# AIRI-Institute/nablaDFT

Hardware: AMD Instinct MI355X
Metric: conformer-steps/sec (fwd+bwd) + MAE(E,F) vs CPU reference (higher is better)
Workload: dtype f32 (dense products >= 192 tiles: f32 values split exactly into 3 bf16 pieces, 6 MFMA piece products, f32 accumulate; non-finite operands give NaN where plain f32 gives inf); 1 GPU; PaiNN-OC (nablaDFT/painn_pyg, config/model/painn-oc.yaml: F=128 L=6 R=100 rc=5A K=100) energy+forces train step incl. neighbour list, L1+L2 loss, grad all-reduce, clip 5.0, AdamW lr 5e-4; synthetic ~42-atom drug-like conformers, 2048 conformers/GPU/step; conformers_per_gpu=2048, edges_last_step=1669592, parallelism=dp1

## Files before the change

### nabladft_amd/csrc/common.h

```cpp
#pragma once
#include <hip/hip_runtime.h>
#include <stdint.h>
#include <stdio.h>

#define NQ_WAVE 64

#define NQ_OK 0
#define NQ_ERR_HIP 1
#define NQ_ERR_ARG 2
#define NQ_ERR_MOL_TOO_LARGE 3
#define NQ_ERR_WORKSPACE 4
#define NQ_ERR_NO_EDGES 5

extern thread_local char nq_err_buf[512];
int nq_fail(int code, const char* fmt, ...);

#define NQ_HIP(call)                                                                            \
  do {                                                                                          \
    hipError_t e__ = (call);                                                                    \
    if (e__ != hipSuccess)                                                                      \
      return nq_fail(NQ_ERR_HIP, "%s:%d %s -> %s", __FILE__, __LINE__, #call, hipGetErrorString(e__)); \
  } while (0)

#define NQ_LAUNCH_CHECK() NQ_HIP(hipGetLastError())
// ... 91 lines not shown
#define NQ_ROWCTR_INTS (8 * 4 * 8 * NQ_ROWCTR_PAD)

struct MsgRevArgs {
  NqGraphView g; int F;
  const float* V; const float* XH; const float* PHI; const float* PSI;
  const float* TV; const float* TXH; const float* TD; const float* TR;
  const float* GX; const float* GV;
  const float* GTX; const float* GTV;
  float* GXH; float* GTXH;
  float* GV_out; float* GTV_out;
  float* GPHI; float* GPSI;
  float4* GEDGE;
  float* GBR;
  int row_filter, mol_cap;
  int lite;
};

struct UpdArgs {
  int N, F;
  const float* XM; const float* VM; const float* U; const float* Y;
  float* S; float* CAT; float* X1; float* V1;
  const float* TXM; const float* TVM; const float* TU; const float* TY;
  float* TS; float* TCAT; float* TX1; float* TV1;
};

struct UpdRevArgs {
  int N, F;
  const float* U; const float* Y; const float* S; const float* CAT;
  const float* TU; const float* TY; const float* TS; const float* TCAT;
  float* GX; float* GV; float* GTX; float* GTV;
  float* GY; float* GTY;
  const float* GCAT; const float* GTCAT;
  float* GU; float* GTU;
  int lite; float* GX_out;
};

struct ReadoutArgs {
  int N, H;
  const float* ZO; const float* TZO; const float* w2; float o2_dummy; const float* o2;
  float* e_atom; float* te_atom;
  const float* ge; const float* gte;
  float* GZO; float* GTZO;
  float* TMPW;
};

int nq_graph_count_impl(const float* pos, const int* mol_ptr, int N, int B, int max_mol_atoms, float cutoff2, int K, int* deg, int* lowdeg,
                        int* row_ptr, int* lowptr, int* E_host, hipStream_t st);
int nq_graph_fill_impl(GraphFillArgs args, int B, int max_mol_atoms, hipStream_t st);

int nq_gemm_nn_epi(hipStream_t st, const float* G, const float* W, float* C, int M, int Nout, int Kin, const float* aux, float ea, float eb, int mode,
                   const char* tag = nullptr);
int nq_gemm_nn_dsilu2(hipStream_t st, const float* G, const float* W, float* C, float* C2, const float* aux, int M, int Nout, int Kin, const char* tag);
int nq_gemm_nt_dsilu(hipStream_t st, const float* A, const float* W, float* C, float* C2, const float* aux, int M, int N, int K, const char* tag = nullptr);
int nq_gemm_nt_act(hipStream_t, const float* A, const float* W, float* C, float* C2, const float* resid, float ea, float eb, int M, int N, int K,
                   const char* tag = nullptr);
int nq_gemm_nt(hipStream_t, const float* A, const float* W, float* C, const float* bias, float* C2_silu, int M, int N, int K, int lda,
               int ldw, int ldc, const char* tag = nullptr);
int nq_gemm_nn(hipStream_t, const float* G, const float* W, float* C, int M, int Nout, int Kin, int ldg, int ldw, int ldc, int accumulate,
               const char* tag = nullptr);
int nq_gemm_nt_res(hipStream_t st, const float* A, const float* W, float* C, const float* aux, float ea, int M, int N, int K);
size_t nq_gemm_tn_scratch_floats(long rows, int Mo, int No);
int nq_gemm_tn(hipStream_t, const float* GY, const float* X, float* out, long rows, int Mo, int No, int ldg, int ldx, float* scratch,
               const char* tag = nullptr, float* bias_out = nullptr, long bias_rows = 0);
size_t nq_colsum_scratch_floats(long rows, int cols);
int nq_colsum(hipStream_t, const float* A, long rows, int cols, int lda, float* out, float* scratch);
int nq_reduce_partials(hipStream_t, const float* part, int nsplit, long stride, long count, float* out);

int nq_rbf(hipStream_t, const float4* geom, int E, int R, double cutoff, int env_p, float coeff, const float* offsets, float* rho,
           float* drho, int type = 0, const float* theta = nullptr);
int nq_rbf_param_grad(hipStream_t, const float4* geom, int E, int R, double cutoff, int env_p, const float* offsets, int type, const float* theta,
                      const float* grho, float* contrib);
int nq_msg_fwd(hipStream_t, const MsgArgs&, bool tangent);
bool nq_filter_fits_lds(int F, int R);
void nq_make_filter_args(FilterArgs* fa, const float* WRT, const float* br, const float* mu, const float* RW, int R, double cutoff, int env_p,
                         float coeff, int mode = 0);
int nq_rbf_window(hipStream_t, const float4* geom, int E, const FilterArgs& fa, float* RW);
int nq_transpose(hipStream_t, const float* in, int rows, int cols, float* out);
size_t nq_k0_sort_scratch_ints(int E, int R);
int nq_k0_sort(hipStream_t, const float* RW, int E, int R, int* order, int* scratch, const int* row_of = nullptr, const int* col = nullptr,
               const int* mol_ptr = nullptr, const int* atom_mol = nullptr, int cap = 0, int* count_out = nullptr);
size_t nq_gwr_scratch_floats(int E, int F, int R, int parts = 3);
int nq_gwr_sorted(hipStream_t, const float* GPHI, const float* GPSI, const float* RW, const int* order, int E, int F, int R, float* gWr,
                  float* scratch, int parts = 3, const int* count_dev = nullptr);
int nq_msgf_fwd(hipStream_t, const MsgArgs&, const FilterArgs&, bool tangent);
int nq_msgf_rev(hipStream_t, const MsgRevArgs&, const FilterArgs&, bool dual, bool pair_rows = true);
int nq_molgw_max_atoms(void);
bool nq_molgw_config_ok(int F, int R);
bool nq_molgw_supported(int F, int R, int max_mol_atoms);
size_t nq_molgw_sched_ints(int E, int B);
size_t nq_molgw_sched_slots(int E, int B);
size_t nq_molgw_rec_floats(int E, int B);
size_t nq_molgw_part_floats(int F, int B);
int nq_molgw_schedule(hipStream_t, const NqGraphView&, const int* dst, const float* RW, int R, int cap, int* sched_ints, float* recs);
int nq_molgw_geometry(hipStream_t, const NqGraphView&, const float* RW, const float* TD, const float* TR, const int* sched_ints, float* recs);
int nq_gwr_mol(hipStream_t, const NqGraphView&, int F, int R, int max_mol_atoms, const float* XH, const float* V, const float* TXH, const float* TV,
               const float* GX, const float* GV, const float* GTX, const float* GTV, const int* sched_ints, const float* recs, float* part, float* gWr,
               float* gbr, bool accumulate = false);
int nq_msg_rev(hipStream_t, const MsgRevArgs&, bool dual);
int nq_geom_tan(hipStream_t, const NqGraphView&, const int* dst, const float* pos_dot, float* TD, float* TR);
int nq_geom_rev(hipStream_t, const NqGraphView&, const float4* GEDGE, int nwaves, float* forces);

bool nq_gemm_exact_f32_requested();
size_t nq_updfuse_frag_floats(int F);
int nq_updfuse_presplit(hipStream_t, const float* U, const float* V1, const float* V2, int F, float* frag);
int nq_upd_fused(hipStream_t, const UpdArgs&, const float* frag, const float* c1, const float* c2, float* ZQ, float* Q);
int nq_upd_a(hipStream_t, const UpdArgs&, bool tan);
int nq_upd_b(hipStream_t, const UpdArgs&, bool tan);
int nq_silu_tan(hipStream_t, const float* Z, const float* TZ, float* TH, long count);
int nq_silu_rev(hipStream_t, const float* Z, const float* TZ, float* G, float* GT, long count, bool dual, bool lite = false);
int nq_upd_rev(hipStream_t, const UpdRevArgs&, int stage, bool dual);
int nq_embed(hipStream_t, const int* z, const float* emb, int N, int F, float* X0);
size_t nq_embed_grad_scratch_floats(int N, int F, int T);
int nq_embed_grad(hipStream_t, const int* z, const float* GX, int N, int F, int T, float* out, float* scratch);
int nq_readout(hipStream_t, const ReadoutArgs&, int mode);
int nq_readout_rev(hipStream_t, const ReadoutArgs&, bool dual);
int nq_mol_sum(hipStream_t, const float* e_atom, const int* mol_ptr, int B, float* out);
int nq_atom_seeds(hipStream_t, const float* gE, const int* atom_mol, int N, float* ge, float* gte);
int nq_negate(hipStream_t, const float* in, float* out, long count);
int nq_axpy(hipStream_t, const float* x, float* y, long count);
int nq_loss_impl(hipStream_t, const float* E, const float* y, int B, const float* Fc, const float* Ft, int N, float ce, float cf, float* loss,
                 float* gE, float* gF, bool mse);
int nq_adamw_impl(hipStream_t, float* p, const float* g, float* m, float* v, long count, float max_norm, float lr, float beta1, float beta2,
                  float eps, float wd, int step, float* scratch);
```

### nabladft_amd/csrc/edge.hip

```cpp
#include "common.h"
#include <type_traits>
#include "lanes.h"

struct RbfArgs {
  const float4* geom; int E; int R; float inv_cutoff; float p, a, b, c; float coeff; const float* mu;
  float* rho; float* drho;
  int type;
  const float* theta;
  float norm_const;
  const float* grho;
  float* contrib;
};

__device__ __forceinline__ void rbf_envelope(const RbfArgs& q, float ds, float& env, float& denv) {
  env = 0.f; denv = 0.f;
  if (ds < 1.0f) {
    if (q.p > 0.f) {
      const float pm1 = powf(ds, q.p - 1.0f);
      const float p0 = pm1 * ds, p1 = p0 * ds, p2 = p1 * ds;
      env = 1.0f + q.a * p0 + q.b * p1 + q.c * p2;
      denv = q.a * q.p * pm1 + q.b * (q.p + 1.0f) * p0 + q.c * (q.p + 2.0f) * p1;
    } else {
      const float om = (1.0f - ds) * (1.0f + ds);
      env = expf(-(ds * ds) / om);
// ... 122 lines not shown
  const float v0 = q.V[o3 + f], v1 = q.V[o3 + F + f], v2 = q.V[o3 + 2 * F + f];
  float txa = 0.f, txb = 0.f, txc = 0.f, tv0 = 0.f, tv1 = 0.f, tv2 = 0.f;
  if (DUAL) {
    txa = q.TXH[o3 + f]; txb = q.TXH[o3 + F + f]; txc = q.TXH[o3 + 2 * F + f];
    tv0 = q.TV[o3 + f]; tv1 = q.TV[o3 + F + f]; tv2 = q.TV[o3 + 2 * F + f];
  }
  float gxa = 0.f, gxb = 0.f, gxc = 0.f, gv0 = 0.f, gv1 = 0.f, gv2 = 0.f;
  float gtxa = 0.f, gtxb = 0.f, gtxc = 0.f, gtv0 = 0.f, gtv1 = 0.f, gtv2 = 0.f;
  float sba = 0.f, sbb = 0.f, sbc = 0.f;
  for (int sp = beg; sp < end; ++sp) {
    const int k = q.g.col[sp];
    const float4 gm = q.g.geom[sp];
    const float r0 = -gm.x, r1 = -gm.y, r2 = -gm.z;
    const float* ph = q.PHI + (long)sp * F3;
    const float pa = ph[f], pb = ph[F + f], pc = ph[2 * F + f];
    const float* A = q.GV + (long)k * F3;
    const float A0 = A[f], A1 = A[F + f], A2 = A[2 * F + f];
    const float gma = q.GX[(long)k * F + f];
    const float mb = xb * pb, mc = xc * pc;
    float gmb = A0 * v0 + A1 * v1 + A2 * v2;
    float gmc = A0 * r0 + A1 * r1 + A2 * r2;
    gv0 += A0 * mb; gv1 += A1 * mb; gv2 += A2 * mb;
    if (DUAL) {
      const float td = q.TD[sp];
      const float tr0 = -q.TR[3 * (long)sp], tr1 = -q.TR[3 * (long)sp + 1], tr2 = -q.TR[3 * (long)sp + 2];
      const float* ps = q.PSI + (long)sp * F3;
      const float tpa = ps[f] * td, tpb = ps[F + f] * td, tpc = ps[2 * F + f] * td;
      const float* T = q.GTV + (long)k * F3;
      const float T0 = T[f], T1 = T[F + f], T2 = T[2 * F + f];
      const float gtma = q.GTX[(long)k * F + f];
      const float tmb = txb * pb + xb * tpb;
      gmb += T0 * tv0 + T1 * tv1 + T2 * tv2;
      const float gtmb = T0 * v0 + T1 * v1 + T2 * v2;
      gmc += T0 * tr0 + T1 * tr1 + T2 * tr2;
      const float gtmc = T0 * r0 + T1 * r1 + T2 * r2;
      gv0 += T0 * tmb; gv1 += T1 * tmb; gv2 += T2 * tmb;
      gtv0 += T0 * mb; gtv1 += T1 * mb; gtv2 += T2 * mb;
      gxa += gma * pa + gtma * tpa; gxb += gmb * pb + gtmb * tpb; gxc += gmc * pc + gtmc * tpc;
      gtxa += gtma * pa; gtxb += gtmb * pb; gtxc += gtmc * pc;
      float* gp = q.GPHI + (long)sp * F3;
      float* gs = q.GPSI + (long)sp * F3;
      const float ga = gma * xa + gtma * txa, gb = gmb * xb + gtmb * txb, gc = gmc * xc + gtmc * txc;
      gp[f] = ga; gp[F + f] = gb; gp[2 * F + f] = gc;
      sba += ga; sbb += gb; sbc += gc;
      gs[f] = gtma * xa * td; gs[F + f] = gtmb * xb * td; gs[2 * F + f] = gtmc * xc * td;
    } else {
      gxa += gma * pa; gxb += gmb * pb; gxc += gmc * pc;
      const float* ps = q.PSI + (long)sp * F3;
      float gd = gma * xa * ps[f] + gmb * xb * ps[F + f] + gmc * xc * ps[2 * F + f];
      float e0 = A0 * mc, e1 = A1 * mc, e2 = A2 * mc;
      gd = nq_wave_sum(gd); e0 = nq_wave_sum(e0); e1 = nq_wave_sum(e1); e2 = nq_wave_sum(e2);
      if (lane == 0) {
        float4* dstp = q.GEDGE + (long)wave * q.g.E + sp;
        float4 acc = *dstp;
        acc.x += gd; acc.y += e0; acc.z += e1; acc.w += e2;
        *dstp = acc;
      }
    }
  }
  q.GXH[o3 + f] = gxa; q.GXH[o3 + F + f] = gxb; q.GXH[o3 + 2 * F + f] = gxc;
  q.GV_out[o3 + f] = q.GV[o3 + f] + gv0;
  q.GV_out[o3 + F + f] = q.GV[o3 + F + f] + gv1;
  q.GV_out[o3 + 2 * F + f] = q.GV[o3 + 2 * F + f] + gv2;
  if (DUAL) {
    q.GTXH[o3 + f] = gtxa; q.GTXH[o3 + F + f] = gtxb; q.GTXH[o3 + 2 * F + f] = gtxc;
    q.GBR[o3 + f] = sba; q.GBR[o3 + F + f] = sbb; q.GBR[o3 + 2 * F + f] = sbc;
    q.GTV_out[o3 + f] = q.GTV[o3 + f] + gtv0;
    q.GTV_out[o3 + F + f] = q.GTV[o3 + F + f] + gtv1;
    q.GTV_out[o3 + 2 * F + f] = q.GTV[o3 + 2 * F + f] + gtv2;
  }
}


#define FUSED_THREADS 1024
#ifndef NQ_DUAL2_THREADS
#define NQ_DUAL2_THREADS 512
#endif
#ifndef NQ_TAN2_THREADS
#define NQ_TAN2_THREADS 768
#endif
#ifndef NQ_DUALNG2_THREADS
#define NQ_DUALNG2_THREADS 768
#endif
__host__ __device__ constexpr int fused_threads(int kind, int ch) {
  return ch >= 4 ? 512
                 : (ch == 2 ? (kind == 3 ? NQ_DUAL2_THREADS : (kind == 4 ? NQ_DUALNG2_THREADS : (kind == 1 ? NQ_TAN2_THREADS : 1024)))
                            : (kind >= 3 ? 768 : 1024));
}
#define FUSED_THREADS_DUAL 1024

__device__ __forceinline__ float bcast_lane(float v, int t) {
  return __int_as_float(__builtin_amdgcn_readlane(__float_as_int(v), t));
}

#define RBFW_THREADS 256
__global__ __launch_bounds__(RBFW_THREADS) void k_rbf_window(const float4* __restrict__ geom, int E, FilterArgs fa, float* __restrict__ RW) {
  __shared__ float tile[RBFW_THREADS][RW_STRIDE + 1];
  const int e0 = blockIdx.x * RBFW_THREADS, e = e0 + threadIdx.x;
  if (e < E) {
    const int R = fa.R;
    const float dist = geom[e].w;
    const float ds = dist * fa.inv_cutoff;
    const int nwin = R < FWIN ? R : FWIN;
    int kc = (int)rintf(ds * (float)(R - 1));
    kc = min(max(kc, 0), R - 1);
    const int k0 = min(max(kc - FWIN / 2, 0), R - nwin);
    float beta = 1.f, dbeta = 0.f, env = 0.f, denv = 0.f;
    if (fa.mode == 0) {
      if (ds < 1.0f) {
        if (fa.p > 0.f) {
          const float pm1 = powf(ds, fa.p - 1.0f);
          const float p0 = pm1 * ds, p1 = p0 * ds, p2 = p1 * ds;
          env = 1.0f + fa.a * p0 + fa.b * p1 + fa.c * p2;
          denv = fa.a * fa.p * pm1 + fa.b * (fa.p + 1.0f) * p0 + fa.c * (fa.p + 2.0f) * p1;
        } else {
          const float om = (1.0f - ds) * (1.0f + ds);
          env = expf(-(ds * ds) / om);
          denv = -env * 2.0f * ds / (om * om);
        }
      }
    } else {
      const float arg = dist * (3.14159265358979323846f / fa.cutoff);
      const bool inside = dist < fa.cutoff;
      beta = inside ? 0.5f * (cosf(arg) + 1.0f) : 0.f;
      dbeta = inside ? -0.5f * (3.14159265358979323846f / fa.cutoff) * sinf(arg) : 0.f;
    }
    float* rw = tile[threadIdx.x];
#pragma unroll
    for (int t = 0; t < 16; ++t) {
      float rl = 0.f, drl = 0.f;
      if (t < nwin) {
        if (fa.mode == 0) {
          const float diff = ds - fa.mu[k0 + t];
          const float g = expf(fa.coeff * (diff * diff));
          rl = env * g;
          drl = fa.inv_cutoff * g * (denv + env * (2.0f * fa.coeff) * diff);
        } else {
          const float diff = dist - fa.mu[k0 + t];
          const float g = expf(fa.coeff * (diff * diff));
          if (fa.mode == 2) {
            rl = g;
            drl = g * (2.0f * fa.coeff) * diff;
          } else {
            rl = beta * g;
            drl = dbeta * g + beta * g * (2.0f * fa.coeff) * diff;
          }
        }
      }
      rw[t] = (t == 13) ? __int_as_float(k0) : (t == 14 ? beta : rl);
      rw[16 + t] = (t == 14) ? dbeta : drl;
    }
  }
  __syncthreads();
  const long base = (long)e0 * RW_STRIDE;
  const long lim = (long)min(RBFW_THREADS, E - e0) * RW_STRIDE;
#pragma unroll 4
  for (int i = threadIdx.x; i < RBFW_THREADS * RW_STRIDE; i += RBFW_THREADS)
    if (i < lim) RW[base + i] = tile[i / RW_STRIDE][i % RW_STRIDE];
}

struct RowRegs { int kk; float gx, gy, gz, td, t0, t1, t2, pf; };
#ifndef NQ_RW_TOUCH
#define NQ_RW_TOUCH 1
#endif
__device__ __forceinline__ void row_touch_done(const RowRegs& r) {
#if NQ_RW_TOUCH
  asm volatile("" ::"v"(r.pf));
#endif
}

template <bool NEED_T>
__device__ __forceinline__ void load_row(RowRegs& r, const NqGraphView& g, const float* __restrict__ TD, const float* __restrict__ TR,
                                         const float* __restrict__ RW, int sp0, int cnt, int lane) {
  r.kk = 0; r.gx = r.gy = r.gz = 0.f; r.td = r.t0 = r.t1 = r.t2 = 0.f; r.pf = 0.f;
  if (lane < cnt) {
    const int sp = sp0 + lane;
#if NQ_RW_TOUCH
    r.pf = RW[(long)sp * RW_STRIDE + 15];
#endif
    r.kk = g.col[sp];
    const float4 gm = g.geom[sp];
    r.gx = gm.x; r.gy = gm.y; r.gz = gm.z;
    if (NEED_T) { r.td = TD[sp]; r.t0 = TR[3 * (long)sp]; r.t1 = TR[3 * (long)sp + 1]; r.t2 = TR[3 * (long)sp + 2]; }
  }
}
template <bool PSI, int CH>
__device__ __forceinline__ void filter_eval(const WinRegs<PSI>& w, const float* wrt, int F, int F3, int fb, const float (&bra)[CH],
                                            const float (&brb)[CH], const float (&brc)[CH], float (&pa)[CH], float (&pb)[CH], float (&pc)[CH],
                                            float (&qa)[CH], float (&qb)[CH], float (&qc)[CH]) {
  typedef VOps<CH> O;
  typedef typename O::V V;
  const V ba = O::from(bra), bb = O::from(brb), bc = O::from(brc);
  V va = ba * O::splat(w.rr[14]), vb = bb * O::splat(w.rr[14]), vc = bc * O::splat(w.rr[14]);
  V ua = O::splat(0.f), ub = ua, uc = ua;
  if (PSI) { ua = ba * O::splat(w.dd[14]); ub = bb * O::splat(w.dd[14]); uc = bc * O::splat(w.dd[14]); }
  const int k0 = __builtin_amdgcn_readfirstlane(__float_as_int(w.rr[13]));
  const float* wk = wrt + k0 * F3 + fb;
#pragma unroll
  for (int t = 0; t < FWIN; ++t) {
    const V wa = lds_tap<CH>(wk + t * F3), wb = lds_tap<CH>(wk + t * F3 + F), wc = lds_tap<CH>(wk + t * F3 + 2 * F);
    const V r = O::splat(w.rr[t]);
    va = O::fma(wa, r, va); vb = O::fma(wb, r, vb); vc = O::fma(wc, r, vc);
    if (PSI) {
      const V d = O::splat(w.dd[t]);
      ua = O::fma(wa, d, ua); ub = O::fma(wb, d, ub); uc = O::fma(wc, d, uc);
    }
  }
  O::to(pa, va); O::to(pb, vb); O::to(pc, vc);
  O::to(qa, ua); O::to(qb, ub); O::to(qc, uc);
}

#ifndef NQ_CLAIM_KINDS
#define NQ_CLAIM_KINDS 15
#endif
#ifndef NQ_CLAIM_ROWS
#define NQ_CLAIM_ROWS 1
#endif
#ifndef NQ_CLAIM_GROUPS_DUAL
#define NQ_CLAIM_GROUPS_DUAL 1
#endif
#ifndef NQ_CLAIM_GROUPS
#define NQ_CLAIM_GROUPS 2
#endif
#define FUSED_ROWS(KIND)                                                                        \
  constexpr bool claim__ = ((NQ_CLAIM_KINDS >> (KIND)) & 1) != 0;                               \
  const bool dyn__ = claim__ && fa.row_ctr != nullptr;    \
  constexpr int crows__ = claim__ ? NQ_CLAIM_ROWS : 1;                                          \
  constexpr int cgmax__ = ((KIND) == 3) ? NQ_CLAIM_GROUPS_DUAL : NQ_CLAIM_GROUPS;               \
  const int cgrp__ = max(1, min(cgmax__, (int)(gridDim.x / nxcd / nslices)));    \
  const int grp__ = wg % cgrp__;                                                                \
  const int sub__ = (n_hi - x_lo + cgrp__ - 1) / cgrp__;                                        \
  const int s_lo__ = dyn__ ? x_lo + grp__ * sub__ : x_lo;                                       \
  const int s_hi__ = dyn__ ? min(n_hi, s_lo__ + sub__) : n_hi;                                  \
  int* const ctr__ = dyn__ ? fa.row_ctr + (((int)(blockIdx.x % nxcd) * nslices + slice) * cgmax__ + grp__) * NQ_ROWCTR_PAD : nullptr; \
  int n_static__ = x_lo + wg * nslots + slot;                                                   \
  auto claim_rows = [&]() __attribute__((always_inline)) -> int {                               \
    if (dyn__) {                                                                                \
      int v__ = 0;                                                                              \
      if (lane == 0) v__ = __hip_atomic_fetch_add(ctr__, crows__, __ATOMIC_RELAXED, __HIP_MEMORY_SCOPE_AGENT); \
      return s_lo__ + __builtin_amdgcn_readfirstlane(v__);                                      \
    }                                                                                           \
    const int v__ = n_static__; n_static__ += n_step; return v__;                               \
  };                                                                                            \
  for (int blk__ = claim_rows(), nxt__ = claim_rows(); blk__ < s_hi__; blk__ = nxt__, nxt__ = claim_rows()) \
    for (int n = blk__; n < min(blk__ + (dyn__ ? crows__ : 1), s_hi__); ++n)

#define FUSED_PROLOGUE                                                                          \
  extern __shared__ __attribute__((aligned(16))) float wrt[];                                  \
  const int F = q.F, F3 = 3 * q.F;                                                             \
  constexpr int FL = 64 * CH;                        \
  const int nslices = F / FL;                                                                  \
   \
  const int nxcd = (gridDim.x % (8 * nslices)) == 0 ? 8 : 1;                                   \
  const int bx = (int)(blockIdx.x / nxcd);                                                     \
  const int slice = bx % nslices, wg = bx / nslices;                                           \
  {                                 \
    const int Rp = fa.R < FWIN ? FWIN : fa.R;                                                  \
    const int per_row4 = (3 * FL) >> 2, fl4 = FL >> 2;                                         \
    float4* dst4 = reinterpret_cast<float4*>(wrt);                                             \
    for (int i = threadIdx.x; i < Rp * per_row4; i += blockDim.x) {                            \
      const int r = i / per_row4, c4 = i % per_row4, part = c4 / fl4, cc = c4 % fl4;           \
      dst4[i] = r < fa.R ? reinterpret_cast<const float4*>(fa.WRT + (long)r * F3 + part * F + slice * FL)[cc] : make_float4(0.f, 0.f, 0.f, 0.f); \
    }                                                                                          \
  }                                                                                            \
  __syncthreads();                                                                             \
  const int nslots = blockDim.x >> 6;                                                          \
  const int slot = __builtin_amdgcn_readfirstlane(threadIdx.x >> 6);                           \
  const int lane = threadIdx.x & 63;                                                           \
  const int lfb = lane * CH;                           \
  const int fb = slice * FL + lfb;                        \
  float bra[CH], brb[CH], brc[CH];                                                             \
  ldv<CH>(bra, fa.br + fb); ldv<CH>(brb, fa.br + F + fb); ldv<CH>(brc, fa.br + 2 * F + fb);    \
                                \
  const int per_x = (q.g.N + nxcd - 1) / nxcd;                                                 \
  const int x_lo = (int)(blockIdx.x % nxcd) * per_x, n_hi = min(q.g.N, x_lo + per_x);          \
  const int n_step = (int)(gridDim.x / nxcd / nslices) * nslots;                               \
                                                          \

template <bool TAN, int CH>
struct FwdOps { float xa[CH], xb[CH], xc[CH], va[CH], vb[CH], vc[CH], txa[CH], txb[CH], txc[CH], tva[CH], tvb[CH], tvc[CH]; };

template <bool TAN>
struct FwdSrc {
  __amdgpu_buffer_rsrc_t xh, v, txh, tv;
  __device__ __forceinline__ FwdSrc(const MsgArgs& q) : xh(row_rsrc(q.XH)), v(row_rsrc(q.V)), txh(row_rsrc(TAN ? q.TXH : q.XH)), tv(row_rsrc(TAN ? q.TV : q.V)) {}
};
template <bool TAN, int CH>
__device__ __forceinline__ void load_fwd(FwdOps<TAN, CH>& o, const FwdSrc<TAN>& src, int k, int F, int F3, int fb) {
  const int ob = fb * 4, r0 = k * F3 * 4, r1 = r0 + F * 4, r2 = r1 + F * 4;
  ldv_buf<CH>(o.xa, src.xh, ob, r0); ldv_buf<CH>(o.xb, src.xh, ob, r1); ldv_buf<CH>(o.xc, src.xh, ob, r2);
  ldv_buf<CH>(o.va, src.v, ob, r0); ldv_buf<CH>(o.vb, src.v, ob, r1); ldv_buf<CH>(o.vc, src.v, ob, r2);
  if (TAN) {
    ldv_buf<CH>(o.txa, src.txh, ob, r0); ldv_buf<CH>(o.txb, src.txh, ob, r1); ldv_buf<CH>(o.txc, src.txh, ob, r2);
    ldv_buf<CH>(o.tva, src.tv, ob, r0); ldv_buf<CH>(o.tvb, src.tv, ob, r1); ldv_buf<CH>(o.tvc, src.tv, ob, r2);
  }
}

template <bool TAN, int CH>
__global__ __launch_bounds__(fused_threads(TAN ? 1 : 0, CH)) void k_msgf_fwd(MsgArgs q, FilterArgs fa, const float* __restrict__ RW) {
  FUSED_PROLOGUE
  const FwdSrc<TAN> src(q);
  FUSED_ROWS(TAN ? 1 : 0) {
    const int beg = __builtin_amdgcn_readfirstlane(q.g.row_ptr[n]), end = __builtin_amdgcn_readfirstlane(q.g.row_ptr[n + 1]);
    float dx[CH], d0[CH], d1[CH], d2[CH];
#pragma unroll
    for (int c = 0; c < CH; ++c) dx[c] = d0[c] = d1[c] = d2[c] = 0.f;
    for (int c0 = beg; c0 < end; c0 += 64) {
      const int cnt = min(64, end - c0);
      RowRegs row;
      load_row<TAN>(row, q.g, q.TD, q.TR, RW, c0, cnt, lane);
      FwdOps<TAN, CH> opA, opB;
      load_fwd<TAN, CH>(opA, src, bl_i(row.kk, 0), F, F3, fb);
      WinRegs<TAN> win;
      load_win<TAN>(win, RW, c0);
      auto step = [&](FwdOps<TAN, CH>& cur, FwdOps<TAN, CH>& nxt, int j, auto prefetch) __attribute__((always_inline)) {
        const int jn = min(j + 1, cnt - 1);
        if (decltype(prefetch)::value) load_fwd<TAN, CH>(nxt, src, bl_i(row.kk, jn), F, F3, fb);
        float pa[CH], pb[CH], pc[CH], qa[CH], qb[CH], qc[CH];
        filter_eval<TAN, CH>(win, wrt, FL, 3 * FL, lfb, bra, brb, brc, pa, pb, pc, qa, qb, qc);
        __builtin_amdgcn_sched_barrier(0);
        if (decltype(prefetch)::value) load_win<TAN>(win, RW, c0 + jn);
        const float gx = bl_f(row.gx, j), gy = bl_f(row.gy, j), gz = bl_f(row.gz, j);
        float td = 0.f, tr0 = 0.f, tr1 = 0.f, tr2 = 0.f;
        if (TAN) { td = bl_f(row.td, j); tr0 = bl_f(row.t0, j); tr1 = bl_f(row.t1, j); tr2 = bl_f(row.t2, j); }
#pragma unroll
        for (int c = 0; c < CH; ++c) {
          const float mb = cur.xb[c] * pb[c], mc = cur.xc[c] * pc[c];
          if (!TAN) {
            dx[c] += cur.xa[c] * pa[c];
            d0[c] += cur.va[c] * mb + mc * gx;
            d1[c] += cur.vb[c] * mb + mc * gy;
            d2[c] += cur.vc[c] * mb + mc * gz;
          } else {
            const float tma = cur.txa[c] * pa[c] + cur.xa[c] * (qa[c] * td);
            const float tmb = cur.txb[c] * pb[c] + cur.xb[c] * (qb[c] * td);
            const float tmc = cur.txc[c] * pc[c] + cur.xc[c] * (qc[c] * td);
            dx[c] += tma;
            d0[c] += cur.tva[c] * mb + cur.va[c] * tmb + tmc * gx + mc * tr0;
            d1[c] += cur.tvb[c] * mb + cur.vb[c] * tmb + tmc * gy + mc * tr1;
            d2[c] += cur.tvc[c] * mb + cur.vc[c] * tmb + tmc * gz + mc * tr2;
          }
        }
      };
      const int pairs = cnt & ~1;
#pragma nounroll
      for (int j = 0; j < pairs; j += 2) {
        step(opA, opB, j, std::true_type());
        step(opB, opA, j + 1, std::true_type());
      }
      if (cnt & 1) step(opA, opB, cnt - 1, std::false_type());
      row_touch_done(row);
    }
    const long o = (long)n * F + fb, o3 = (long)n * F3 + fb;
    float x0[CH], w0[CH], w1[CH], w2[CH];
    if (!TAN) {
      ldv<CH>(x0, q.X + o); ldv<CH>(w0, q.V + o3); ldv<CH>(w1, q.V + o3 + F); ldv<CH>(w2, q.V + o3 + 2 * F);
    } else {
      ldv<CH>(x0, q.TX + o); ldv<CH>(w0, q.TV + o3); ldv<CH>(w1, q.TV + o3 + F); ldv<CH>(w2, q.TV + o3 + 2 * F);
    }
#pragma unroll
    for (int c = 0; c < CH; ++c) { x0[c] += dx[c]; w0[c] += d0[c]; w1[c] += d1[c]; w2[c] += d2[c]; }
    if (!TAN) {
      stv<CH>(q.XM + o, x0); stv<CH>(q.VM + o3, w0); stv<CH>(q.VM + o3 + F, w1); stv<CH>(q.VM + o3 + 2 * F, w2);
    } else {
      stv<CH>(q.TXM + o, x0); stv<CH>(q.TVM + o3, w0); stv<CH>(q.TVM + o3 + F, w1); stv<CH>(q.TVM + o3 + 2 * F, w2);
    }
  }
}

#ifndef NQ_ABLATE
#define NQ_ABLATE 0
#endif
#if NQ_ABLATE == 3
#define ABL_K(j) n
#else
#define ABL_K(j) bl_i(row.kk, j)
#endif
#if NQ_ABLATE == 4
#define ABL_SP(x) 0
#else
#define ABL_SP(x) (x)
#endif
template <bool DUAL, int CH>
struct RevOps { float A0[CH], A1[CH], A2[CH], gma[CH], T0[CH], T1[CH], T2[CH], gtma[CH]; };

template <bool DUAL>
struct RevSrc {
  __amdgpu_buffer_rsrc_t gv, gx, gtv, gtx;
  __device__ __forceinline__ RevSrc(const MsgRevArgs& q) : gv(row_rsrc(q.GV)), gx(row_rsrc(q.GX)), gtv(row_rsrc(DUAL ? q.GTV : q.GV)), gtx(row_rsrc(DUAL ? q.GTX : q.GX)) {}
};
template <bool DUAL, int CH>
__device__ __forceinline__ void load_rev(RevOps<DUAL, CH>& o, const RevSrc<DUAL>& src, int k, int F, int F3, int fb) {
  const int ob = fb * 4, r0 = k * F3 * 4, r1 = r0 + F * 4, r2 = r1 + F * 4, rx = k * F * 4;
  ldv_buf<CH>(o.A0, src.gv, ob, r0); ldv_buf<CH>(o.A1, src.gv, ob, r1); ldv_buf<CH>(o.A2, src.gv, ob, r2);
  ldv_buf<CH>(o.gma, src.gx, ob, rx);
  if (DUAL) {
    ldv_buf<CH>(o.T0, src.gtv, ob, r0); ldv_buf<CH>(o.T1, src.gtv, ob, r1); ldv_buf<CH>(o.T2, src.gtv, ob, r2);
    ldv_buf<CH>(o.gtma, src.gtx, ob, rx);
  }
}

#ifndef NQ_DUAL_NA_RESIDENT
#define NQ_DUAL_NA_RESIDENT 1
#endif
#ifndef NQ_DUAL_MIRROR
#define NQ_DUAL_MIRROR 1
#endif
#ifndef NQ_DUAL_KX_EARLY
#define NQ_DUAL_KX_EARLY 1
#endif
template <bool DUAL, int CH, bool GW, bool LITE = false>
__device__ __forceinline__ void msgf_rev_body(const MsgRevArgs& q, const FilterArgs& fa, const float* __restrict__ RW) {
  FUSED_PROLOGUE
  const RevSrc<DUAL> src(q);
  FUSED_ROWS(DUAL ? 3 : 2) {
    if (DUAL && q.row_filter) {
      const int mm = __builtin_amdgcn_readfirstlane(q.g.atom_mol[n]);
      const bool big = __builtin_amdgcn_readfirstlane(q.g.mol_ptr[mm + 1]) - __builtin_amdgcn_readfirstlane(q.g.mol_ptr[mm]) > q.mol_cap;
      if (big != (q.row_filter == 2)) continue;
    }
    const int beg = __builtin_amdgcn_readfirstlane(q.g.row_ptr[n]), end = __builtin_amdgcn_readfirstlane(q.g.row_ptr[n + 1]);
    const int nlow = (DUAL && GW) ? __builtin_amdgcn_readfirstlane(q.g.lowptr[n + 1]) - __builtin_amdgcn_readfirstlane(q.g.lowptr[n]) : 0;
    const long o3 = (long)n * F3 + fb;
    float xa[CH], xb[CH], xc[CH], v0[CH], v1[CH], v2[CH], txa[CH], txb[CH], txc[CH], tv0[CH], tv1[CH], tv2[CH];
    ldv<CH>(xa, q.XH + o3); ldv<CH>(xb, q.XH + o3 + F); ldv<CH>(xc, q.XH + o3 + 2 * F);
    ldv<CH>(v0, q.V + o3); ldv<CH>(v1, q.V + o3 + F); ldv<CH>(v2, q.V + o3 + 2 * F);
    float nA0[CH], nA1[CH], nA2[CH], ngma[CH], nT0[CH], nT1[CH], nT2[CH], ngtma[CH];
    if (DUAL) {
      ldv<CH>(txa, q.TXH + o3); ldv<CH>(txb, q.TXH + o3 + F); ldv<CH>(txc, q.TXH + o3 + 2 * F);
      ldv<CH>(tv0, q.TV + o3); ldv<CH>(tv1, q.TV + o3 + F); ldv<CH>(tv2, q.TV + o3 + 2 * F);
#if NQ_DUAL_NA_RESIDENT
      if (GW) {
      ldv<CH>(nA0, q.GV + o3); ldv<CH>(nA1, q.GV + o3 + F); ldv<CH>(nA2, q.GV + o3 + 2 * F);
      ldv<CH>(nT0, q.GTV + o3); ldv<CH>(nT1, q.GTV + o3 + F); ldv<CH>(nT2, q.GTV + o3 + 2 * F);
      ldv<CH>(ngma, q.GX + (long)n * F + fb); ldv<CH>(ngtma, q.GTX + (long)n * F + fb);
      }
#endif
    } else {
#pragma unroll
      for (int c = 0; c < CH; ++c) txa[c] = txb[c] = txc[c] = tv0[c] = tv1[c] = tv2[c] = 0.f;
    }
    float gxa[CH], gxb[CH], gxc[CH], gv0[CH], gv1[CH], gv2[CH], gtxa[CH], gtxb[CH], gtxc[CH], gtv0[CH], gtv1[CH], gtv2[CH], sba[CH], sbb[CH], sbc[CH];
#pragma unroll
    for (int c = 0; c < CH; ++c) {
      gxa[c] = gxb[c] = gxc[c] = gv0[c] = gv1[c] = gv2[c] = 0.f;
      gtxa[c] = gtxb[c] = gtxc[c] = gtv0[c] = gtv1[c] = gtv2[c] = 0.f;
      sba[c] = sbb[c] = sbc[c] = 0.f;
    }
    for (int c0 = beg; c0 < end; c0 += 64) {
      const int cnt = min(64, end - c0);
      const int nlo = (DUAL && GW) ? max(0, min(cnt, nlow - (c0 - beg))) : 0;
      RowRegs row;
      load_row<DUAL>(row, q.g, q.TD, q.TR, RW, c0, cnt, lane);
      RevOps<DUAL, CH> opA, opB;
      load_rev<DUAL, CH>(opA, src, ABL_K(0), F, F3, fb);
      WinRegs<true> win;
      load_win<true>(win, RW, ABL_SP(c0));
      float4 eacc = make_float4(0.f, 0.f, 0.f, 0.f);
      auto step = [&](RevOps<DUAL, CH>& cur, RevOps<DUAL, CH>& nxt, int j, auto low_tag) __attribute__((always_inline)) {
        constexpr bool LOW = decltype(low_tag)::value;
        const int sp = c0 + j;
        const int jn = min(j + 1, cnt - 1);
        load_rev<DUAL, CH>(nxt, src, ABL_K(jn), F, F3, fb);
        float kxa[CH], kxb[CH], kxc[CH], kv0[CH], kv1[CH], kv2[CH], ktxa[CH], ktxb[CH], ktxc[CH], ktv0[CH], ktv1[CH], ktv2[CH];
        if (DUAL && GW && LOW && NQ_DUAL_KX_EARLY) {
          const long k3 = (long)ABL_K(j) * F3 + fb;
          ldv<CH>(kxa, q.XH + k3); ldv<CH>(kxb, q.XH + k3 + F); ldv<CH>(kxc, q.XH + k3 + 2 * F);
          ldv<CH>(kv0, q.V + k3); ldv<CH>(kv1, q.V + k3 + F); ldv<CH>(kv2, q.V + k3 + 2 * F);
          ldv<CH>(ktxa, q.TXH + k3); ldv<CH>(ktxb, q.TXH + k3 + F); ldv<CH>(ktxc, q.TXH + k3 + 2 * F);
          ldv<CH>(ktv0, q.TV + k3); ldv<CH>(ktv1, q.TV + k3 + F); ldv<CH>(ktv2, q.TV + k3 + 2 * F);
        }
        float pa[CH], pb[CH], pc[CH], qa[CH], qb[CH], qc[CH];
#if NQ_ABLATE == 2
#pragma unroll
        for (int c = 0; c < CH; ++c) { pa[c] = bra[c] * win.rr[0]; pb[c] = brb[c] * win.rr[1]; pc[c] = brc[c] * win.rr[2]; qa[c] = bra[c] * win.dd[0]; qb[c] = brb[c] * win.dd[1]; qc[c] = brc[c] * win.dd[2]; }
#else
        filter_eval<true, CH>(win, wrt, FL, 3 * FL, lfb, bra, brb, brc, pa, pb, pc, qa, qb, qc);
#endif
        const float beta = win.rr[14], dbeta = win.dd[14];
        __builtin_amdgcn_sched_barrier(0);
        load_win<true>(win, RW, ABL_SP(c0 + jn));
        if (DUAL && GW && LOW && !NQ_DUAL_KX_EARLY) {
          const long k3 = (long)ABL_K(j) * F3 + fb;
          ldv<CH>(kxa, q.XH + k3); ldv<CH>(kxb, q.XH + k3 + F); ldv<CH>(kxc, q.XH + k3 + 2 * F);
          ldv<CH>(kv0, q.V + k3); ldv<CH>(kv1, q.V + k3 + F); ldv<CH>(kv2, q.V + k3 + 2 * F);
          ldv<CH>(ktxa, q.TXH + k3); ldv<CH>(ktxb, q.TXH + k3 + F); ldv<CH>(ktxc, q.TXH + k3 + 2 * F);
          ldv<CH>(ktv0, q.TV + k3); ldv<CH>(ktv1, q.TV + k3 + F); ldv<CH>(ktv2, q.TV + k3 + 2 * F);
        }
        const float r0 = -bl_f(row.gx, j), r1 = -bl_f(row.gy, j), r2 = -bl_f(row.gz, j);
        float td = 0.f, tr0 = 0.f, tr1 = 0.f, tr2 = 0.f;
        if (DUAL) { td = bl_f(row.td, j); tr0 = -bl_f(row.t0, j); tr1 = -bl_f(row.t1, j); tr2 = -bl_f(row.t2, j); }
        float gd = 0.f, e0 = 0.f, e1 = 0.f, e2 = 0.f;
        float ga[CH], gb[CH], gc[CH], ha[CH], hb[CH], hc[CH];
#pragma unroll
        for (int c = 0; c < CH; ++c) {
          const float A0 = cur.A0[c], A1 = cur.A1[c], A2 = cur.A2[c], gma = cur.gma[c];
          const float mb = xb[c] * pb[c], mc = xc[c] * pc[c];
          float gmb = A0 * v0[c] + A1 * v1[c] + A2 * v2[c];
          float gmc = A0 * r0 + A1 * r1 + A2 * r2;
          gv0[c] += A0 * mb; gv1[c] += A1 * mb; gv2[c] += A2 * mb;
          if (DUAL) {
            const float tpa = qa[c] * td, tpb = qb[c] * td, tpc = qc[c] * td;
            const float T0 = cur.T0[c], T1 = cur.T1[c], T2 = cur.T2[c], gtma = cur.gtma[c];
            const float tmb = txb[c] * pb[c] + xb[c] * tpb;
            gmb += T0 * tv0[c] + T1 * tv1[c] + T2 * tv2[c];
            const float gtmb = T0 * v0[c] + T1 * v1[c] + T2 * v2[c];
            gmc += T0 * tr0 + T1 * tr1 + T2 * tr2;
            const float gtmc = T0 * r0 + T1 * r1 + T2 * r2;
            gv0[c] += T0 * tmb; gv1[c] += T1 * tmb; gv2[c] += T2 * tmb;
            if (!LITE) { gtv0[c] += T0 * mb; gtv1[c] += T1 * mb; gtv2[c] += T2 * mb; }
            gxa[c] += gma * pa[c] + gtma * tpa; gxb[c] += gmb * pb[c] + gtmb * tpb; gxc[c] += gmc * pc[c] + gtmc * tpc;
            if (!LITE) { gtxa[c] += gtma * pa[c]; gtxb[c] += gtmb * pb[c]; gtxc[c] += gtmc * pc[c]; }
            if (GW) {
              ga[c] = gma * xa[c] + gtma * txa[c]; gb[c] = gmb * xb[c] + gtmb * txb[c]; gc[c] = gmc * xc[c] + gtmc * txc[c];
              ha[c] = gtma * xa[c] * td; hb[c] = gtmb * xb[c] * td; hc[c] = gtmc * xc[c] * td;
              sba[c] += ga[c] * beta + ha[c] * dbeta;
              sbb[c] += gb[c] * beta + hb[c] * dbeta;
              sbc[c] += gc[c] * beta + hc[c] * dbeta;
            }
          } else {
            gxa[c] += gma * pa[c]; gxb[c] += gmb * pb[c]; gxc[c] += gmc * pc[c];
            gd += gma * xa[c] * qa[c] + gmb * xb[c] * qb[c] + gmc * xc[c] * qc[c];
            e0 += A0 * mc; e1 += A1 * mc; e2 += A2 * mc;
          }
        }
        if (DUAL && GW && LOW && NQ_ABLATE != 1) {
#if !NQ_DUAL_NA_RESIDENT
          __builtin_amdgcn_sched_barrier(0);
          ldv<CH>(nA0, q.GV + o3); ldv<CH>(nA1, q.GV + o3 + F); ldv<CH>(nA2, q.GV + o3 + 2 * F);
          ldv<CH>(nT0, q.GTV + o3); ldv<CH>(nT1, q.GTV + o3 + F); ldv<CH>(nT2, q.GTV + o3 + 2 * F);
          ldv<CH>(ngma, q.GX + (long)n * F + fb); ldv<CH>(ngtma, q.GTX + (long)n * F + fb);
#endif
#pragma unroll
          for (int c = 0; c < CH; ++c) {
            const float rgmb = nA0[c] * kv0[c] + nA1[c] * kv1[c] + nA2[c] * kv2[c] + (nT0[c] * ktv0[c] + nT1[c] * ktv1[c] + nT2[c] * ktv2[c]);
            const float rgtmb = nT0[c] * kv0[c] + nT1[c] * kv1[c] + nT2[c] * kv2[c];
            const float rgmc = -(nA0[c] * r0 + nA1[c] * r1 + nA2[c] * r2) - (nT0[c] * tr0 + nT1[c] * tr1 + nT2[c] * tr2);
            const float rgtmc = -(nT0[c] * r0 + nT1[c] * r1 + nT2[c] * r2);
            ga[c] += ngma[c] * kxa[c] + ngtma[c] * ktxa[c]; gb[c] += rgmb * kxb[c] + rgtmb * ktxb[c]; gc[c] += rgmc * kxc[c] + rgtmc * ktxc[c];
            ha[c] += ngtma[c] * kxa[c] * td; hb[c] += rgtmb * kxb[c] * td; hc[c] += rgtmc * kxc[c] * td;
          }
          float* gp = q.GPHI + (long)sp * F3 + fb;
          float* gs = q.GPSI + (long)sp * F3 + fb;
          stv_stream<CH>(gp, ga); stv_stream<CH>(gp + F, gb); stv_stream<CH>(gp + 2 * F, gc);
          stv_stream<CH>(gs, ha); stv_stream<CH>(gs + F, hb); stv_stream<CH>(gs + 2 * F, hc);
        } else if (!DUAL) {
          gd = nq_wave_sum(gd); e0 = nq_wave_sum(e0); e1 = nq_wave_sum(e1); e2 = nq_wave_sum(e2);
          const bool mine = lane == j;
          eacc.x = mine ? gd : eacc.x; eacc.y = mine ? e0 : eacc.y; eacc.z = mine ? e1 : eacc.z; eacc.w = mine ? e2 : eacc.w;
        }
      };
      int j = 0;
#pragma nounroll
      for (; j + 1 < nlo; j += 2) {
        step(opA, opB, j, std::true_type());
        step(opB, opA, j + 1, std::true_type());
      }
#if NQ_DUAL_MIRROR
      if (j < nlo) {
        step(opA, opB, j, std::true_type());
        ++j;
#pragma nounroll
        for (; j + 1 < cnt; j += 2) {
          step(opB, opA, j, std::false_type());
          step(opA, opB, j + 1, std::false_type());
        }
        if (j < cnt) step(opB, opA, j, std::false_type());
      } else {
#pragma nounroll
        for (; j + 1 < cnt; j += 2) {
          step(opA, opB, j, std::false_type());
          step(opB, opA, j + 1, std::false_type());
        }
        if (j < cnt) step(opA, opB, j, std::false_type());
      }
#else
      if (j < nlo) {
        step(opA, opB, j, std::true_type());
        ++j;
        opA = opB;
      }
#pragma nounroll
      for (; j + 1 < cnt; j += 2) {
        step(opA, opB, j, std::false_type());
        step(opB, opA, j + 1, std::false_type());
      }
      if (j < cnt) step(opA, opB, j, std::false_type());
#endif
      row_touch_done(row);
      if (!DUAL && lane < cnt) {
        float4* dstp = q.GEDGE + (long)slice * q.g.E + c0 + lane;
        float4 acc = *dstp;
        acc.x += eacc.x; acc.y += eacc.y; acc.z += eacc.z; acc.w += eacc.w;
        *dstp = acc;
      }
    }
    float g0[CH], g1[CH], g2[CH];
    stv<CH>(q.GXH + o3, gxa); stv<CH>(q.GXH + o3 + F, gxb); stv<CH>(q.GXH + o3 + 2 * F, gxc);
    ldv<CH>(g0, q.GV + o3); ldv<CH>(g1, q.GV + o3 + F); ldv<CH>(g2, q.GV + o3 + 2 * F);
#pragma unroll
    for (int c = 0; c < CH; ++c) { g0[c] += gv0[c]; g1[c] += gv1[c]; g2[c] += gv2[c]; }
    stv<CH>(q.GV_out + o3, g0); stv<CH>(q.GV_out + o3 + F, g1); stv<CH>(q.GV_out + o3 + 2 * F, g2);
    if (DUAL) {
      if (GW) { stv<CH>(q.GBR + o3, sba); stv<CH>(q.GBR + o3 + F, sbb); stv<CH>(q.GBR + o3 + 2 * F, sbc); }
      if (!LITE && !q.lite) {
        stv<CH>(q.GTXH + o3, gtxa); stv<CH>(q.GTXH + o3 + F, gtxb); stv<CH>(q.GTXH + o3 + 2 * F, gtxc);
        ldv<CH>(g0, q.GTV + o3); ldv<CH>(g1, q.GTV + o3 + F); ldv<CH>(g2, q.GTV + o3 + 2 * F);
#pragma unroll
        for (int c = 0; c < CH; ++c) { g0[c] += gtv0[c]; g1[c] += gtv1[c]; g2[c] += gtv2[c]; }
        stv<CH>(q.GTV_out + o3, g0); stv<CH>(q.GTV_out + o3 + F, g1); stv<CH>(q.GTV_out + o3 + 2 * F, g2);
      }
    }
  }
}


template <bool DUAL, int CH>
__global__ __launch_bounds__(fused_threads(DUAL ? 3 : 2, CH)) void k_msgf_rev(MsgRevArgs q, FilterArgs fa, const float* __restrict__ RW) {
  msgf_rev_body<DUAL, CH, DUAL>(q, fa, RW);
}
template <bool LITE, int CH>
__global__ __launch_bounds__(fused_threads(4, CH)) void k_msgf_rev_nopair(MsgRevArgs q, FilterArgs fa, const float* __restrict__ RW) {
  msgf_rev_body<true, CH, false, LITE>(q, fa, RW);
}

#define SORT_CHUNK 256
struct K0Filter { const int* row_of; const int* col; const int* mol_ptr; const int* atom_mol; int cap; };
__device__ __forceinline__ int k0_key(const float* __restrict__ RW, int e, int E, const K0Filter& f) {
  if (e >= E) return -1;
  if (f.row_of && f.col[e] >= f.row_of[e]) return -1;
  if (f.cap > 0) { const int m = f.atom_mol[f.row_of[e]]; if (f.mol_ptr[m + 1] - f.mol_ptr[m] <= f.cap) return -1; }
  return __float_as_int(RW[(long)e * RW_STRIDE + 13]);
}
__global__ __launch_bounds__(SORT_CHUNK) void k_k0_hist(const float* __restrict__ RW, int E, int nbins, int* __restrict__ chunk_hist,
                                                        int* __restrict__ local_rank, K0Filter flt) {
  __shared__ int keys[SORT_CHUNK];
  __shared__ int hist[256];
  const int e = blockIdx.x * SORT_CHUNK + threadIdx.x;
  const int key = k0_key(RW, e, E, flt);
  keys[threadIdx.x] = key;
  if (threadIdx.x < nbins) hist[threadIdx.x] = 0;
  __syncthreads();
  if (key >= 0) {
    int r = 0;
    for (int i = 0; i < (int)threadIdx.x; ++i) r += (keys[i] == key);
    local_rank[e] = r;
    atomicAdd(&hist[key], 1);
  }
  __syncthreads();
  if (threadIdx.x < nbins) chunk_hist[(long)threadIdx.x * gridDim.x + blockIdx.x] = hist[threadIdx.x];
}
__global__ __launch_bounds__(256) void k_k0_scan(int* __restrict__ hist, int nchunks, int nbins, int* __restrict__ bin_total) {
  const int lane = threadIdx.x & 63;
  const int b = blockIdx.x * 4 + (threadIdx.x >> 6);
  if (b >= nbins) return;
  int* row = hist + (long)b * nchunks;
  int carry = 0;
  for (int c0 = 0; c0 < nchunks; c0 += 64) {
    const int c = c0 + lane;
    const int v = c < nchunks ? row[c] : 0;
    int sc = v;
#pragma unroll
    for (int off = 1; off < 64; off <<= 1) {
      const int t = __shfl_up(sc, off, 64);
      if (lane >= off) sc += t;
    }
    if (c < nchunks) row[c] = carry + sc - v;
    carry += __shfl(sc, 63, 64);
  }
  if (lane == 0) bin_total[b] = carry;
}
__global__ __launch_bounds__(SORT_CHUNK) void k_k0_scatter(const float* __restrict__ RW, int E, int nbins, const int* __restrict__ hist,
                                                           const int* __restrict__ bin_total, const int* __restrict__ local_rank,
                                                           int* __restrict__ order, K0Filter flt, int* __restrict__ count_out) {
  __shared__ int base[256];
  if (threadIdx.x == 0) {
    int run = 0;
    for (int i = 0; i < nbins; ++i) { base[i] = run; run += bin_total[i]; }
    if (count_out && blockIdx.x == 0) *count_out = run;
  }
  __syncthreads();
  const int e = blockIdx.x * SORT_CHUNK + threadIdx.x;
  const int key = k0_key(RW, e, E, flt);
  if (key < 0) return;
  order[base[key] + hist[(long)key * gridDim.x + blockIdx.x] + local_rank[e]] = e;
}

#ifndef GWR_WAVES
#define GWR_WAVES 4
#endif
#ifndef GWR_DEPTH
#define GWR_DEPTH 6
#endif
#ifndef GWR_CHUNKS
#define GWR_CHUNKS 1360
#endif
template <int CH>
__global__ __launch_bounds__(GWR_WAVES * 64) void k_gwr_sorted(const float* __restrict__ GPHI, const float* __restrict__ GPSI, const float* __restrict__ RW,
                                                               const int* __restrict__ order, int E_, int F, int F3, int R, int chunk_len,
                                                               float* __restrict__ part, int* __restrict__ chunk_range, const int* __restrict__ count_dev) {
  const int wave = __builtin_amdgcn_readfirstlane(threadIdx.x >> 6), lane = threadIdx.x & 63;
  const int chunk = blockIdx.x * GWR_WAVES + wave;
// ... 178 lines not shown
  else hipLaunchKernelGGL((k_msg_rev<false>), dim3(q.g.N), dim3(q.F), 0, st, q);
  NQ_LAUNCH_CHECK();
  return NQ_OK;
}

int nq_geom_tan(hipStream_t st, const NqGraphView& g, const int* dst, const float* pos_dot, float* TD, float* TR) {
  NQ_PROF(st, "geom_tan");
  if (g.E <= 0) return NQ_OK;
  hipLaunchKernelGGL(k_geom_tan, dim3(nq_cdiv(g.E, 256)), dim3(256), 0, st, g, dst, pos_dot, TD, TR);
  NQ_LAUNCH_CHECK();
  return NQ_OK;
}

int nq_geom_rev(hipStream_t st, const NqGraphView& g, const float4* GEDGE, int nwaves, float* forces) {
  NQ_PROF(st, "geom_rev");
  hipLaunchKernelGGL(k_geom_rev, dim3(nq_cdiv(g.N, 128)), dim3(128), 0, st, g, GEDGE, nwaves, forces);
  NQ_LAUNCH_CHECK();
  return NQ_OK;
}

bool nq_filter_fits_lds(int F, int R) {
  return (size_t)(R < FWIN ? FWIN : R) * 3 * F * sizeof(float) <= 156 * 1024 && (F == 64 || F == 128 || F == 256);
}

void nq_make_filter_args(FilterArgs* fa, const float* WRT, const float* br, const float* mu, const float* RW, int R, double cutoff, int env_p,
                         float coeff, int mode) {
  const double p = env_p;
  fa->WRT = WRT; fa->br = br; fa->mu = mu; fa->RW = RW; fa->R = R; fa->inv_cutoff = (float)(1.0 / cutoff);
  fa->p = (float)p; fa->a = (float)(-(p + 1) * (p + 2) / 2); fa->b = (float)(p * (p + 2)); fa->c = (float)(-p * (p + 1) / 2);
  fa->coeff = coeff; fa->mode = mode; fa->cutoff = (float)cutoff; fa->row_ctr = nullptr;
}

int nq_rbf_window(hipStream_t st, const float4* geom, int E, const FilterArgs& fa, float* RW) {
  NQ_PROF(st, "rbf_window");
  if (E <= 0) return NQ_OK;
  hipLaunchKernelGGL(k_rbf_window, dim3(nq_cdiv(E, RBFW_THREADS)), dim3(RBFW_THREADS), 0, st, geom, E, fa, RW);
  NQ_LAUNCH_CHECK();
  return NQ_OK;
}

int nq_transpose(hipStream_t st, const float* in, int rows, int cols, float* out) {
  NQ_PROF(st, "transpose");
  hipLaunchKernelGGL(k_transpose, dim3(nq_cdiv(cols, 32), nq_cdiv(rows, 32)), dim3(32, 8), 0, st, in, rows, cols, out);
  NQ_LAUNCH_CHECK();
  return NQ_OK;
}

#ifndef NQ_CH_FWD
#define NQ_CH_FWD 0
#endif
#ifndef NQ_CH_TAN
#define NQ_CH_TAN 0
#endif
#ifndef NQ_CH_FORCE
#define NQ_CH_FORCE 0
#endif
#ifndef NQ_CH_DUAL
#define NQ_CH_DUAL 0
#endif
#ifndef NQ_SMALL_SLICE_ATOMS
#define NQ_SMALL_SLICE_ATOMS 2048
#endif
static int fused_ch(int kind, int F, int N) {
  const int forced = kind == 0 ? NQ_CH_FWD : (kind == 1 ? NQ_CH_TAN : (kind == 2 ? NQ_CH_FORCE : NQ_CH_DUAL));
  const int full = F / 64;
  if (forced > 0 && forced <= full && full % forced == 0) return forced;
  if (N < NQ_SMALL_SLICE_ATOMS && full >= 2) return full / 2;
  return full;
}
static int fused_grid(int N, int F, int ch, int* threads, size_t* lds, int R, int max_threads = FUSED_THREADS) {
  const int nslots = max_threads / 64;
  const int nslices = F / (64 * ch);
  *threads = nslots * 64;
  *lds = (size_t)(R < FWIN ? FWIN : R) * 3 * 64 * ch * sizeof(float);
  int per_cu = (int)((156 * 1024) / *lds);
  per_cu = per_cu < 1 ? 1 : (per_cu > 2 ? 2 : per_cu);
  int groups = 256 * per_cu / nslices;
  groups = groups < 8 ? 8 : (groups / 8) * 8;
  const int need = nq_cdiv(N, nslots);
  if (need < groups) groups = need;
  return groups * nslices;
}

#define FUSED_LAUNCH(KERN, FLAG, CHV, Q)                                                                          \
  do {                                                                                                            \
    NQ_DYN_LDS((KERN<FLAG, CHV>), lds);                                                                           \
    hipLaunchKernelGGL((KERN<FLAG, CHV>), dim3(grid), dim3(threads), lds, st, Q, fa, fa.RW);                      \
  } while (0)
#define FUSED_DISPATCH(KERN, FLAG, Q)                                   \
  do {                                                                  \
    switch (ch) {                                                       \
      case 1: FUSED_LAUNCH(KERN, FLAG, 1, Q); break;                    \
      case 2: FUSED_LAUNCH(KERN, FLAG, 2, Q); break;                    \
      case 4: FUSED_LAUNCH(KERN, FLAG, 4, Q); break;                    \
      default: return nq_fail(NQ_ERR_ARG, "fused message kernels need hidden_channels in {64,128,256}"); \
    }                                                                   \
  } while (0)

int nq_msgf_fwd(hipStream_t st, const MsgArgs& q, const FilterArgs& fa, bool tangent) {
  NQ_PROF(st, tangent ? "msgf_tan" : "msgf_fwd");
  if (q.g.N <= 0) return NQ_OK;
  if ((size_t)q.g.N * 3 * q.F * 4 >= 0xfffff000ull) return nq_fail(NQ_ERR_ARG, "fused message kernels: a node array of %d atoms x %d channels exceeds the 4 GB a buffer descriptor's scalar offset reaches", q.g.N, 3 * q.F);
  int threads; size_t lds;
  const int ch = fused_ch(tangent ? 1 : 0, q.F, q.g.N);
  const int grid = fused_grid(q.g.N, q.F, ch, &threads, &lds, fa.R, fused_threads(tangent ? 1 : 0, ch));
  if (tangent) FUSED_DISPATCH(k_msgf_fwd, true, q);
  else FUSED_DISPATCH(k_msgf_fwd, false, q);
  NQ_LAUNCH_CHECK();
  return NQ_OK;
}

int nq_msgf_rev(hipStream_t st, const MsgRevArgs& q, const FilterArgs& fa, bool dual, bool pair_rows) {
  NQ_PROF(st, dual ? (pair_rows ? "msgf_rev_dual" : "msgf_rev_dual_ng") : "msgf_rev_force");
  if (q.g.N <= 0) return NQ_OK;
  if ((size_t)q.g.N * 3 * q.F * 4 >= 0xfffff000ull) return nq_fail(NQ_ERR_ARG, "fused message kernels: a node array of %d atoms x %d channels exceeds the 4 GB a buffer descriptor's scalar offset reaches", q.g.N, 3 * q.F);
  int threads; size_t lds;
  const int kind = dual ? (pair_rows ? 3 : 4) : 2;
  const int ch = fused_ch(dual ? 3 : 2, q.F, q.g.N);
  const int grid = fused_grid(q.g.N, q.F, ch, &threads, &lds, fa.R, fused_threads(kind, ch));
  if (dual && !pair_rows && q.lite) FUSED_DISPATCH(k_msgf_rev_nopair, true, q);
  else if (dual && !pair_rows) FUSED_DISPATCH(k_msgf_rev_nopair, false, q);
  else if (dual) FUSED_DISPATCH(k_msgf_rev, true, q);
  else FUSED_DISPATCH(k_msgf_rev, false, q);
  NQ_LAUNCH_CHECK();
  return NQ_OK;
}

static int gwr_nbins(int R) { return R - (R < FWIN ? R : FWIN) + 1; }
static int gwr_chunks(int E) {
  int chunk_len = nq_cdiv(E, GWR_CHUNKS);
  if (chunk_len < 64) chunk_len = 64;
  return nq_cdiv(E, chunk_len);
}
size_t nq_k0_sort_scratch_ints(int E, int R) { return (size_t)nq_cdiv(E, SORT_CHUNK) * gwr_nbins(R) + (size_t)E + 256; }
int nq_k0_sort(hipStream_t st, const float* RW, int E, int R, int* order, int* scratch, const int* row_of, const int* col, const int* mol_ptr,
               const int* atom_mol, int cap, int* count_out) {
  NQ_PROF(st, "k0_sort");
  K0Filter flt{row_of, col, mol_ptr, atom_mol, (row_of && mol_ptr && atom_mol) ? cap : 0};
  const int nbins = gwr_nbins(R), nchunks = nq_cdiv(E, SORT_CHUNK);
  if (nbins > 256) return nq_fail(NQ_ERR_ARG, "k0 sort supports at most 256 bins (num_rbf <= 268)");
  int* chunk_hist = scratch; int* local_rank = scratch + (size_t)nchunks * nbins; int* bin_total = local_rank + E;
  hipLaunchKernelGGL(k_k0_hist, dim3(nchunks), dim3(SORT_CHUNK), 0, st, RW, E, nbins, chunk_hist, local_rank, flt);
  NQ_LAUNCH_CHECK();
  hipLaunchKernelGGL(k_k0_scan, dim3(nq_cdiv(nbins, 4)), dim3(256), 0, st, chunk_hist, nchunks, nbins, bin_total);
  NQ_LAUNCH_CHECK();
  hipLaunchKernelGGL(k_k0_scatter, dim3(nchunks), dim3(SORT_CHUNK), 0, st, RW, E, nbins, chunk_hist, bin_total, local_rank, order, flt, count_out);
  NQ_LAUNCH_CHECK();
  return NQ_OK;
}

size_t nq_gwr_scratch_floats(int E, int F, int R, int parts) { const size_t nc = gwr_chunks(E); return nc * R * parts * F + 2 * nc + 16; }

int nq_gwr_sorted(hipStream_t st, const float* GPHI, const float* GPSI, const float* RW, const int* order, int E, int F, int R, float* gWr,
                  float* scratch, int parts, const int* count_dev) {
  NQ_PROF(st, "gwr_sorted");
  const int nchunks = gwr_chunks(E), chunk_len = nq_cdiv(E, nchunks);
  float* part = scratch;
  const int F3 = parts * F;
  int* chunk_range = reinterpret_cast<int*>(scratch + (size_t)nchunks * R * F3);
  dim3 grid(nq_cdiv(nchunks, GWR_WAVES), parts);
  switch (F / 64) {
    case 1: hipLaunchKernelGGL((k_gwr_sorted<1>), grid, dim3(GWR_WAVES * 64), 0, st, GPHI, GPSI, RW, order, E, F, F3, R, chunk_len, part, chunk_range, count_dev); break;
    case 2: hipLaunchKernelGGL((k_gwr_sorted<2>), grid, dim3(GWR_WAVES * 64), 0, st, GPHI, GPSI, RW, order, E, F, F3, R, chunk_len, part, chunk_range, count_dev); break;
    case 4: hipLaunchKernelGGL((k_gwr_sorted<4>), grid, dim3(GWR_WAVES * 64), 0, st, GPHI, GPSI, RW, order, E, F, F3, R, chunk_len, part, chunk_range, count_dev); break;
    default: return nq_fail(NQ_ERR_ARG, "gwr_sorted needs hidden_channels in {64,128,256}");
  }
  NQ_LAUNCH_CHECK();
  hipLaunchKernelGGL(k_gwr_reduce, dim3(nq_cdiv((long)R * F3, 256)), dim3(256), 0, st, part, chunk_range, nq_cdiv(E, chunk_len), R, F3, gWr);
  NQ_LAUNCH_CHECK();
  return NQ_OK;
}
```

### nabladft_amd/csrc/engine.hip

```cpp
#include <stdarg.h>
#include <stdlib.h>
#include <string.h>

#include "../../include/nablaq.h"
#include "common.h"

thread_local char nq_err_buf[512] = "";
int nq_fail(int code, const char* fmt, ...) {
  va_list ap;
  va_start(ap, fmt);
  vsnprintf(nq_err_buf, sizeof(nq_err_buf), fmt, ap);
  va_end(ap);
  return code;
}

#include <map>
#include <mutex>
#include <utility>
static std::mutex g_lds_mu;
static std::map<std::pair<int, const void*>, size_t> g_lds_granted;
int nq_dyn_lds(const void* kernel, size_t bytes) {
  int dev = 0;
  NQ_HIP(hipGetDevice(&dev));
  std::lock_guard<std::mutex> lock(g_lds_mu);
// ... 58 lines not shown
  for (int l = 0; l < c->num_layers; ++l) {
    UpdP& u = P->upd[l];
    u.U = o; o += 2 * F * F; u.V1 = o; o += F * 2 * F; u.c1 = o; o += F; u.V2 = o; o += 3 * F * F; u.c2 = o; o += 3 * F;
  }
  P->O1 = o; o += H * F; P->o1 = o; o += H; P->w2 = o; o += H; P->o2 = o; o += 1;
  P->total = o;
  return NQ_OK;
}

struct WsLayer {
  size_t Z1, Hh, XH, PHI, PSI, XM, VM, UU, S, CAT, ZQ, Q, Y;
  size_t WRT;
  size_t UFRAG;
  size_t LGY, LGCAT, LGU, LGXH, LGXA, LGXB, LGVA, LGVB;
  size_t LGQ, LGH, LGQP, LGHP;
};
struct WsLayout {
  size_t X[65], V[65];
  WsLayer lay[64];
  size_t RHO2, RW, ORDER, ZO, e_atom, te_atom, TD, TR, pos_dot, ge, gte;
  size_t GX, GVa, GVb, GY, GQ, GCAT, GU, GXH, GH, GBR, GPHI2, GEDGE, GZO, TMPW, GRHO, BCON, ROWCTR, SCHED, GWREC, GWPART, scratch;
  size_t scratch_floats, total_floats;
  bool fused;
};
static size_t a4(size_t x) { return (x + 3) & ~(size_t)3; }

static void make_ws_layout(const nq_painn_cfg* c, size_t N, size_t E, size_t B, bool fused, WsLayout* W) {
  const size_t F = c->hidden_channels, R = c->num_rbf, H = F / 2, L = c->num_layers, T = c->num_elements;
  W->fused = fused;
  const size_t EP = W->fused ? 0 : E;
  size_t o = 0;
  auto take = [&](size_t n) { size_t r = o; o += a4(n); return r; };
  for (size_t l = 0; l <= L; ++l) { W->X[l] = take(2 * N * F); W->V[l] = take(2 * N * 3 * F); }
  for (size_t l = 0; l < L; ++l) {
    WsLayer& y = W->lay[l];
    y.Z1 = take(2 * N * F); y.Hh = take(2 * N * F); y.XH = take(2 * N * 3 * F);
    y.PHI = take(EP * 3 * F); y.PSI = take(EP * 3 * F); y.WRT = take(R * 3 * F);
    y.XM = take(2 * N * F); y.VM = take(2 * N * 3 * F); y.UU = take(2 * N * 6 * F);
    y.S = take(2 * N * F); y.CAT = take(2 * N * 2 * F); y.ZQ = take(2 * N * F); y.Q = take(2 * N * F); y.Y = take(2 * N * 3 * F);
    y.UFRAG = take(nq_updfuse_frag_floats((int)F));
    const size_t st_ = W->fused ? 1 : 0;
    y.LGY = take(st_ * 2 * N * 3 * F); y.LGCAT = take(st_ * 2 * N * 2 * F); y.LGU = take(st_ * 2 * N * 6 * F); y.LGXH = take(st_ * 2 * N * 3 * F);
    y.LGXA = take(st_ * N * F); y.LGXB = take(st_ * N * F); y.LGVA = take(st_ * N * 3 * F); y.LGVB = take(st_ * N * 3 * F);
    y.LGQ = take(st_ * 2 * N * F); y.LGH = take(st_ * 2 * N * F); y.LGQP = take(st_ * N * F); y.LGHP = take(st_ * N * F);
  }
  W->RHO2 = take(2 * EP * R);
  W->ORDER = take(W->fused ? E : 0);
  W->RW = take(W->fused ? E * 32 : 0);
  W->ZO = take(2 * N * H); W->e_atom = take(N); W->te_atom = take(N);
  W->TD = take(E); W->TR = take(3 * E); W->pos_dot = take(3 * N); W->ge = take(N); W->gte = take(N);
  W->GX = take(2 * N * F); W->GVa = take(2 * N * 3 * F); W->GVb = take(2 * N * 3 * F);
  W->GY = take(2 * N * 3 * F); W->GQ = take(2 * N * F); W->GCAT = take(2 * N * 2 * F); W->GU = take(2 * N * 6 * F);
  W->GXH = take(2 * N * 3 * F); W->GH = take(2 * N * F);
  W->GBR = take(N * 3 * F);
  W->GPHI2 = take(2 * E * 3 * F);
  W->GEDGE = take((F / 64) * E * 4);
  W->GZO = take(2 * N * H); W->TMPW = take(N * H);
  W->GRHO = take(c->rbf_type ? 2 * E * R : 0); W->BCON = take(c->rbf_type ? E * R : 0);
  W->ROWCTR = take(5 * L * NQ_ROWCTR_INTS);
  W->SCHED = take(W->fused ? nq_molgw_sched_ints((int)E, (int)B) : 0);
  W->GWREC = take(W->fused ? nq_molgw_rec_floats((int)E, (int)B) : 0);
  W->GWPART = take(W->fused ? nq_molgw_part_floats((int)F, (int)B) : 0);
  size_t s = 0;
  auto mx = [&](size_t v) { if (v > s) s = v; };
  mx(nq_gemm_tn_scratch_floats(2 * N, 3 * F, F)); mx(nq_gemm_tn_scratch_floats(2 * N, F, 2 * F)); mx(nq_gemm_tn_scratch_floats(6 * N, 2 * F, F));
  mx(W->fused ? nq_gwr_scratch_floats((int)E, (int)F, (int)R) : nq_gemm_tn_scratch_floats(2 * E, 3 * F, R));
  if (W->fused) mx(nq_k0_sort_scratch_ints((int)E, (int)R));
  mx(nq_gemm_tn_scratch_floats(2 * N, F, F)); mx(nq_gemm_tn_scratch_floats(2 * N, H, F));
  mx(nq_colsum_scratch_floats(N > E ? N : E, 3 * F));
  if (c->rbf_type) { mx(nq_colsum_scratch_floats(E, R)); mx(nq_colsum_scratch_floats(E * R, 1)); }
  mx(nq_embed_grad_scratch_floats((int)N, (int)F, (int)T));
  W->scratch_floats = s;
  W->scratch = take(s);
  W->total_floats = o;
  (void)B;
}

enum { GW_PAIR_ROWS = 0, GW_MOLECULE = 1, GW_MIXED = 2 };
struct StepPlan {
  bool fused;
  int gw_mode, gw_cap;
  bool lite;
  bool fused_update;
};
static StepPlan plan_step(const nq_painn_cfg* c, const nq_graph* g, bool want_forces) {
  auto env_on = [](const char* name) { const char* v = getenv(name); return v && v[0] == '1'; };
  StepPlan p{};
  p.fused = c->rbf_type == 0 && nq_filter_fits_lds(c->hidden_channels, c->num_rbf) && !env_on("NQ_NO_FUSED_FILTER");
  const char* cap = getenv("NQ_MOLGW_CAP");
  const int hw = nq_molgw_max_atoms();
  p.gw_cap = cap && atoi(cap) > 0 && atoi(cap) < hw ? atoi(cap) : hw;
  p.gw_mode = GW_PAIR_ROWS;
  if (p.fused && !env_on("NQ_NO_MOLGW") && nq_molgw_config_ok(c->hidden_channels, c->num_rbf) && g->max_mol_atoms > 0 && (env_on("NQ_MOLGW") || g->N >= 4096))
    p.gw_mode = g->max_mol_atoms <= p.gw_cap ? GW_MOLECULE : GW_MIXED;
  p.lite = p.fused && want_forces && !env_on("NQ_NO_LITE");
  p.fused_update = nq_updfuse_frag_floats(c->hidden_channels) > 0 && !env_on("NQ_NO_FUSED_UPDATE") && !nq_gemm_exact_f32_requested();
  return p;
}
static bool plan_fused(const nq_painn_cfg* c, int32_t N, int32_t E, int32_t B) {
  nq_graph g{};
  g.N = N; g.E = E; g.B = B;
  return plan_step(c, &g, false).fused;
}

struct StepRecord { nq_painn_cfg cfg; int32_t N, E, B, max_mol_atoms; StepPlan plan; };
static std::mutex g_plan_mu;
static std::map<const void*, StepRecord> g_plans;
static void record_plan(const void* ws, const nq_painn_cfg* c, const nq_graph* g, const StepPlan& p) {
  std::lock_guard<std::mutex> lock(g_plan_mu);
  g_plans[ws] = StepRecord{*c, g->N, g->E, g->B, g->max_mol_atoms, p};
}
static int recall_plan(const void* ws, const nq_painn_cfg* c, const nq_graph* g, StepPlan* p) {
  std::lock_guard<std::mutex> lock(g_plan_mu);
  auto it = g_plans.find(ws);
  if (it == g_plans.end()) return nq_fail(NQ_ERR_ARG, "nq_painn_backward: no forward call has prepared this workspace");
  const StepRecord& r = it->second;
  if (memcmp(&r.cfg, c, sizeof(nq_painn_cfg)) != 0 || r.N != g->N || r.E != g->E || r.B != g->B || r.max_mol_atoms != g->max_mol_atoms)
    return nq_fail(NQ_ERR_ARG, "nq_painn_backward: the last forward call on this workspace was made for a different model or batch");
  *p = r.plan;
  return NQ_OK;
}

static NqGraphView view_of(const nq_graph* g) {
  NqGraphView v;
  v.N = g->N; v.B = g->B; v.E = g->E;
  v.mol_ptr = g->mol_ptr; v.row_ptr = g->row_ptr; v.col = g->col; v.rev = g->rev;
  v.geom = reinterpret_cast<const float4*>(g->geom); v.z = g->z; v.atom_mol = g->atom_mol; v.lowptr = g->lowptr;
  return v;
}

static int check_common(const nq_painn_cfg* cfg, const nq_graph* g, const void* ws, size_t ws_bytes, bool fused, WsLayout* W, ParamLayout* P) {
  if (!cfg || !g || !ws) return nq_fail(NQ_ERR_ARG, "null argument");
  NQ_TRY(make_param_layout(cfg, P));
  if (g->N <= 0 || g->B <= 0) return nq_fail(NQ_ERR_ARG, "empty batch");
  if (g->E <= 0) return nq_fail(NQ_ERR_NO_EDGES, "batch has no edges within the cutoff");
  if ((reinterpret_cast<uintptr_t>(ws) & 15) != 0) return nq_fail(NQ_ERR_ARG, "workspace must be 16-byte aligned");
  make_ws_layout(cfg, g->N, g->E, g->B, fused, W);
  if (cfg->filter_mode != 0 && cfg->filter_mode != 1) return nq_fail(NQ_ERR_ARG, "filter_mode must be 0 (painn_pyg) or 1 (schnetpack)");
  if (cfg->filter_mode == 1 && !W->fused)
    return nq_fail(NQ_ERR_ARG, "filter_mode 1 (schnetpack) needs the fused-filter path: hidden_channels in {64,128,256} and WrT fitting the LDS");
  if (ws_bytes < W->total_floats * sizeof(float))
    return nq_fail(NQ_ERR_WORKSPACE, "workspace too small: %zu < %zu bytes", ws_bytes, W->total_floats * sizeof(float));
  return NQ_OK;
}

extern "C" {

int nq_abi_version(void) { return NQ_ABI_VERSION; }
int32_t nq_painn_molecule_lds_atoms(void) { return nq_molgw_max_atoms(); }

void nq_profile_enable(int32_t on) { nq_profile_on = on; }
int nq_profile_read2(char* names, int32_t name_stride, double* total_ms, int64_t* counts, double* flops, int32_t cap) {
  (void)hipDeviceSynchronize();
  std::vector<double> tot(g_prof_names.size(), 0.0), fl(g_prof_names.size(), 0.0);
  std::vector<long long> cnt(g_prof_names.size(), 0);
  for (auto& r : g_prof_recs) {
    float ms = 0.f;
    if (hipEventElapsedTime(&ms, r.a, r.b) == hipSuccess) { tot[r.name_id] += ms; cnt[r.name_id] += 1; fl[r.name_id] += r.flops; }
    (void)hipEventDestroy(r.a); (void)hipEventDestroy(r.b);
  }
  g_prof_recs.clear();
  int n = (int)g_prof_names.size();
  for (int i = 0; i < n && i < cap; ++i) {
    snprintf(names + (size_t)i * name_stride, name_stride, "%s", g_prof_names[i].c_str());
    total_ms[i] = tot[i]; counts[i] = cnt[i];
    if (flops) flops[i] = fl[i];
  }
  return n;
}
int nq_profile_read(char* names, int32_t name_stride, double* total_ms, int64_t* counts, int32_t cap) {
  return nq_profile_read2(names, name_stride, total_ms, counts, nullptr, cap);
}
const char* nq_last_error(void) { return nq_err_buf; }

int nq_graph_count(const float* pos, const int32_t* mol_ptr, int32_t N, int32_t B, int32_t max_mol_atoms, double cutoff,
                   int32_t max_neighbors, int32_t* deg, int32_t* lowdeg, int32_t* row_ptr, int32_t* lowptr, int32_t* E_host, void* stream) {
  if (!pos || !mol_ptr || !deg || !lowdeg || !row_ptr || !lowptr || !E_host) return nq_fail(NQ_ERR_ARG, "null argument");
  if (max_neighbors < 1) return nq_fail(NQ_ERR_ARG, "max_neighbors must be >= 1");
  return nq_graph_count_impl(pos, mol_ptr, N, B, max_mol_atoms, (float)(cutoff * cutoff), max_neighbors, deg, lowdeg, row_ptr, lowptr,
                             E_host, (hipStream_t)stream);
}

int nq_graph_fill(const float* pos, const int32_t* mol_ptr, int32_t N, int32_t B, int32_t E, int32_t max_mol_atoms, double cutoff,
                  int32_t max_neighbors, const int32_t* row_ptr, const int32_t* lowptr, int32_t* col, int32_t* dst, int32_t* rev, float* geom,
                  int32_t* slot2canon, int32_t* atom_mol, int64_t* edge_index, float* edge_dist, float* edge_vector, int64_t* id_swap,
                  int64_t* neighbors, void* stream) {
  if (!pos || !mol_ptr || !row_ptr || !lowptr || !col || !dst || !rev || !geom || !slot2canon || !atom_mol)
    return nq_fail(NQ_ERR_ARG, "null argument");
  if (edge_index && (!edge_dist || !edge_vector || !id_swap)) return nq_fail(NQ_ERR_ARG, "canonical outputs must be all set or all NULL");
  if ((reinterpret_cast<uintptr_t>(geom) & 15) != 0) return nq_fail(NQ_ERR_ARG, "geom must be 16-byte aligned");
  GraphFillArgs a;
  a.pos = pos; a.mol_ptr = mol_ptr; a.row_ptr = row_ptr; a.lowptr = lowptr;
  a.r2 = (float)(cutoff * cutoff); a.K = max_neighbors;
  a.col = col; a.dst = dst; a.rev = rev; a.geom = reinterpret_cast<float4*>(geom); a.slot2canon = slot2canon;
  a.c_src = (long long*)edge_index; a.c_dst = edge_index ? (long long*)edge_index + E : nullptr;
  a.c_dist = edge_dist; a.c_vec = edge_vector; a.id_swap = (long long*)id_swap; a.neighbors = (long long*)neighbors;
  a.atom_mol = atom_mol;
  (void)N;
  return nq_graph_fill_impl(a, B, max_mol_atoms, (hipStream_t)stream);
}

size_t nq_painn_num_params(const nq_painn_cfg* cfg) {
  ParamLayout P;
  if (!cfg || make_param_layout(cfg, &P) != NQ_OK) return 0;
  return P.total;
}

size_t nq_painn_workspace_bytes(const nq_painn_cfg* cfg, int32_t N, int32_t E, int32_t B) {
  ParamLayout P;
  if (!cfg || make_param_layout(cfg, &P) != NQ_OK || N <= 0 || E < 0) return 0;
  WsLayout W;
  make_ws_layout(cfg, N, E, B, plan_fused(cfg, N, E, B), &W);
  return W.total_floats * sizeof(float);
}

int nq_painn_ws_lookup(const nq_painn_cfg* cfg, int32_t N, int32_t E, int32_t B, const char* name, int32_t l, int32_t tangent,
                       size_t* off, size_t* count) {
  ParamLayout P;
  if (!cfg || !name || !off || !count) return nq_fail(NQ_ERR_ARG, "null argument");
  NQ_TRY(make_param_layout(cfg, &P));
  WsLayout W;
  make_ws_layout(cfg, N, E, B, plan_fused(cfg, N, E, B), &W);
  const size_t F = cfg->hidden_channels, R = cfg->num_rbf, H = F / 2, n = N, e = E;
  const int L = cfg->num_layers;
  size_t base = 0, rows = 0, w = 0;
  bool dual = true;
#define LAYER_OK(maxl) if (l < 0 || l > (maxl)) return nq_fail(NQ_ERR_ARG, "layer %d out of range", l)
  if (!strcmp(name, "x_in")) { LAYER_OK(L); base = W.X[l]; rows = n; w = F; }
  else if (!strcmp(name, "vec_in")) { LAYER_OK(L); base = W.V[l]; rows = n; w = 3 * F; }
  else if (!strcmp(name, "z1")) { LAYER_OK(L - 1); base = W.lay[l].Z1; rows = n; w = F; }
  else if (!strcmp(name, "h")) { LAYER_OK(L - 1); base = W.lay[l].Hh; rows = n; w = F; }
  else if (!strcmp(name, "xh")) { LAYER_OK(L - 1); base = W.lay[l].XH; rows = n; w = 3 * F; }
  else if (!strcmp(name, "phi") || !strcmp(name, "psi")) {
    LAYER_OK(L - 1);
    if (W.fused) return nq_fail(NQ_ERR_ARG, "buffer '%s' is not materialised (filter is fused into the message kernels)", name);
    base = name[1] == 'h' ? W.lay[l].PHI : W.lay[l].PSI; rows = e; w = 3 * F; dual = false;
  }
  else if (!strcmp(name, "x_msg")) { LAYER_OK(L - 1); base = W.lay[l].XM; rows = n; w = F; }
  else if (!strcmp(name, "vec_msg")) { LAYER_OK(L - 1); base = W.lay[l].VM; rows = n; w = 3 * F; }
  else if (!strcmp(name, "u")) { LAYER_OK(L - 1); base = W.lay[l].UU; rows = n; w = 6 * F; }
  else if (!strcmp(name, "s")) { LAYER_OK(L - 1); base = W.lay[l].S; rows = n; w = F; }
  else if (!strcmp(name, "cat")) { LAYER_OK(L - 1); base = W.lay[l].CAT; rows = n; w = 2 * F; }
  else if (!strcmp(name, "zq")) { LAYER_OK(L - 1); base = W.lay[l].ZQ; rows = n; w = F; }
  else if (!strcmp(name, "q")) { LAYER_OK(L - 1); base = W.lay[l].Q; rows = n; w = F; }
  else if (!strcmp(name, "y")) { LAYER_OK(L - 1); base = W.lay[l].Y; rows = n; w = 3 * F; }
  else if (!strcmp(name, "rho")) {
    if (W.fused) return nq_fail(NQ_ERR_ARG, "buffer 'rho' is not materialised (filter is fused into the message kernels)");
    base = W.RHO2; rows = e; w = R;
  }
  else if (!strcmp(name, "order")) {
    if (!W.fused) return nq_fail(NQ_ERR_ARG, "buffer 'order' exists only with the fused filter");
    base = W.ORDER; rows = e; w = 1; dual = false;
  }
  else if (!strcmp(name, "pair_sched")) {
    if (!W.fused) return nq_fail(NQ_ERR_ARG, "buffer 'pair_sched' exists only with the fused filter");
    base = W.SCHED; rows = 2 * nq_molgw_sched_slots((int)e, B); w = 1; dual = false;
  }
  else if (!strcmp(name, "pair_sched_meta")) {
    if (!W.fused) return nq_fail(NQ_ERR_ARG, "buffer 'pair_sched_meta' exists only with the fused filter");
    base = W.SCHED + 2 * nq_molgw_sched_slots((int)e, B); rows = nq_molgw_sched_ints((int)e, B) - 2 * nq_molgw_sched_slots((int)e, B); w = 1; dual = false;
  }
  else if (!strcmp(name, "rw")) {
    if (!W.fused) return nq_fail(NQ_ERR_ARG, "buffer 'rw' exists only with the fused filter");
    base = W.RW; rows = e; w = 32; dual = false;
  }
  else if (!strcmp(name, "zo")) { base = W.ZO; rows = n; w = H; }
  else if (!strcmp(name, "e_atom")) { base = tangent ? W.te_atom : W.e_atom; rows = n; w = 1; dual = false; tangent = 0; }
  else if (!strcmp(name, "t_d")) { base = W.TD; rows = e; w = 1; dual = false; }
  else if (!strcmp(name, "t_r")) { base = W.TR; rows = e; w = 3; dual = false; }
  else if (!strcmp(name, "gedge")) { base = W.GEDGE; rows = (F / 64) * e; w = 4; dual = false; }
  else return nq_fail(NQ_ERR_ARG, "unknown workspace buffer '%s'", name);
#undef LAYER_OK
  if (tangent && !dual) return nq_fail(NQ_ERR_ARG, "buffer '%s' has no tangent half", name);
  *off = base + (tangent ? rows * w : 0);
  *count = rows * w;
  return NQ_OK;
}

int nq_painn_forward(const nq_painn_cfg* cfg, const float* params, const float* rbf_offsets, const nq_graph* graph, void* workspace,
                     size_t workspace_bytes, float* energy, float* forces, void* stream) {
  if (!cfg || !graph) return nq_fail(NQ_ERR_ARG, "null argument");
  const StepPlan plan = plan_step(cfg, graph, forces != nullptr);
  WsLayout W; ParamLayout P;
  NQ_TRY(check_common(cfg, graph, workspace, workspace_bytes, plan.fused, &W, &P));
  if (!params || !rbf_offsets || !energy) return nq_fail(NQ_ERR_ARG, "null argument");
  record_plan(workspace, cfg, graph, plan);
  hipStream_t st = (hipStream_t)stream;
  float* ws = (float*)workspace;
  const NqGraphView g = view_of(graph);
  const int N = g.N, E = g.E, F = cfg->hidden_channels, R = cfg->num_rbf, H = F / 2, L = cfg->num_layers;
  const size_t NF = (size_t)N * F;
  int* const rowctr0 = reinterpret_cast<int*>(ws + W.ROWCTR);
  NQ_HIP(hipMemsetAsync(rowctr0, 0, (size_t)2 * L * NQ_ROWCTR_INTS * sizeof(int), st));
  auto row_ctr = [&](int kind, int l) { return N >= 4096 ? rowctr0 + ((size_t)kind * L + l) * NQ_ROWCTR_INTS : (int*)nullptr; };

  NQ_TRY(nq_embed(st, g.z, params + P.emb, N, F, ws + W.X[0]));
  NQ_HIP(hipMemsetAsync(ws + W.X[0] + NF, 0, NF * sizeof(float), st));
  NQ_HIP(hipMemsetAsync(ws + W.V[0], 0, 6 * NF * sizeof(float), st));
  float* rho = ws + W.RHO2; float* drho = rho + (size_t)E * R;
  const bool lite_store = plan.lite;
  if (W.fused) {
    FilterArgs fa0;
    nq_make_filter_args(&fa0, nullptr, nullptr, rbf_offsets, ws + W.RW, R, cfg->cutoff, cfg->envelope_exponent, cfg->rbf_coeff, cfg->filter_mode);
    NQ_TRY(nq_rbf_window(st, g.geom, E, fa0, ws + W.RW));
    int* const sched = reinterpret_cast<int*>(ws + W.SCHED);
    if (plan.gw_mode != GW_PAIR_ROWS) NQ_TRY(nq_molgw_schedule(st, g, graph->dst, ws + W.RW, R, plan.gw_cap, sched, ws + W.GWREC));
    if (plan.gw_mode == GW_PAIR_ROWS) NQ_TRY(nq_k0_sort(st, ws + W.RW, E, R, reinterpret_cast<int*>(ws + W.ORDER), reinterpret_cast<int*>(ws + W.scratch), graph->dst, g.col));
    else if (plan.gw_mode == GW_MIXED)
      NQ_TRY(nq_k0_sort(st, ws + W.RW, E, R, reinterpret_cast<int*>(ws + W.ORDER), reinterpret_cast<int*>(ws + W.scratch), graph->dst, g.col, g.mol_ptr, g.atom_mol,
                        plan.gw_cap, sched + nq_molgw_sched_ints(E, g.B) - 1));
  } else {
    NQ_TRY(nq_rbf(st, g.geom, E, R, cfg->cutoff, cfg->envelope_exponent, cfg->rbf_coeff, rbf_offsets, rho, drho, cfg->rbf_type, params + P.basis));
  }

  for (int l = 0; l < L; ++l) {
    const WsLayer& y = W.lay[l]; const MsgP& mp = P.msg[l]; const UpdP& up = P.upd[l];
    NQ_TRY(nq_gemm_nt(st, ws + W.X[l], params + mp.W1, ws + y.Z1, params + mp.b1, ws + y.Hh, N, F, F, F, F, F, "W1"));
    NQ_TRY(nq_gemm_nt(st, ws + y.Hh, params + mp.W2, ws + y.XH, params + mp.b2, nullptr, N, 3 * F, F, F, F, 3 * F, "W2"));
    MsgArgs m{};
    m.g = g; m.F = F; m.X = ws + W.X[l]; m.V = ws + W.V[l]; m.XH = ws + y.XH; m.PHI = ws + y.PHI; m.PSI = ws + y.PSI;
    m.XM = ws + y.XM; m.VM = ws + y.VM;
    if (W.fused) {
      FilterArgs fa;
      NQ_TRY(nq_transpose(st, params + mp.Wr, 3 * F, R, ws + y.WRT));
      nq_make_filter_args(&fa, ws + y.WRT, params + mp.br, rbf_offsets, ws + W.RW, R, cfg->cutoff, cfg->envelope_exponent, cfg->rbf_coeff, cfg->filter_mode);
      fa.row_ctr = row_ctr(0, l);
      NQ_TRY(nq_msgf_fwd(st, m, fa, false));
    } else {
      NQ_TRY(nq_gemm_nt(st, rho, params + mp.Wr, ws + y.PHI, params + mp.br, nullptr, E, 3 * F, R, R, R, 3 * F, "Wr"));
      NQ_TRY(nq_gemm_nt(st, drho, params + mp.Wr, ws + y.PSI, nullptr, nullptr, E, 3 * F, R, R, R, 3 * F, "Wr"));
      NQ_TRY(nq_msg_fwd(st, m, false));
    }
    UpdArgs u{};
    u.N = N; u.F = F; u.XM = ws + y.XM; u.VM = ws + y.VM; u.U = ws + y.UU; u.Y = ws + y.Y; u.S = ws + y.S; u.CAT = ws + y.CAT;
    u.X1 = ws + W.X[l + 1]; u.V1 = ws + W.V[l + 1];
    if (plan.fused_update) {
      NQ_TRY(nq_updfuse_presplit(st, params + up.U, params + up.V1, params + up.V2, F, ws + y.UFRAG));
      NQ_TRY(nq_upd_fused(st, u, ws + y.UFRAG, params + up.c1, params + up.c2, ws + y.ZQ, ws + y.Q));
      continue;
    }
    NQ_TRY(nq_gemm_nt(st, ws + y.VM, params + up.U, ws + y.UU, nullptr, nullptr, 3 * N, 2 * F, F, F, F, 2 * F, "U"));
    NQ_TRY(nq_upd_a(st, u, false));
    NQ_TRY(nq_gemm_nt(st, ws + y.CAT, params + up.V1, ws + y.ZQ, params + up.c1, ws + y.Q, N, F, 2 * F, 2 * F, 2 * F, F, "V1"));
    NQ_TRY(nq_gemm_nt(st, ws + y.Q, params + up.V2, ws + y.Y, params + up.c2, nullptr, N, 3 * F, F, F, F, 3 * F, "V2"));
    NQ_TRY(nq_upd_b(st, u, false));
  }
  NQ_TRY(nq_gemm_nt(st, ws + W.X[L], params + P.O1, ws + W.ZO, params + P.o1, nullptr, N, H, F, F, F, H, "O1"));
  ReadoutArgs r{};
  r.N = N; r.H = H; r.ZO = ws + W.ZO; r.w2 = params + P.w2; r.o2 = params + P.o2; r.e_atom = ws + W.e_atom;
  NQ_TRY(nq_readout(st, r, 0));
  NQ_TRY(nq_mol_sum(st, ws + W.e_atom, g.mol_ptr, g.B, energy));
  if (!forces) return NQ_OK;

  NQ_TRY(nq_atom_seeds(st, nullptr, g.atom_mol, N, ws + W.ge, nullptr));
  r.ge = ws + W.ge; r.GZO = ws + W.GZO;
  NQ_TRY(nq_readout_rev(st, r, false));
  float* gx_cur = lite_store ? ws + W.lay[L - 1].LGXA : ws + W.GX;
  NQ_TRY(nq_gemm_nn(st, ws + W.GZO, params + P.O1, gx_cur, N, H, F, H, F, F, 0, "O1"));
  float* gv_cur = lite_store ? ws + W.lay[L - 1].LGVA : ws + W.GVa; float* gv_oth = ws + W.GVb;
  NQ_HIP(hipMemsetAsync(gv_cur, 0, 3 * NF * sizeof(float), st));
  const int nwaves = F / 64;
  NQ_HIP(hipMemsetAsync(ws + W.GEDGE, 0, (size_t)nwaves * E * 4 * sizeof(float), st));
  for (int l = L - 1; l >= 0; --l) {
    const WsLayer& y = W.lay[l]; const MsgP& mp = P.msg[l]; const UpdP& up = P.upd[l];
    float* const GY = lite_store ? ws + y.LGY + 3 * NF : ws + W.GY;
    float* const GCAT = lite_store ? ws + y.LGCAT + 2 * NF : ws + W.GCAT;
    float* const GU = lite_store ? ws + y.LGU + 6 * NF : ws + W.GU;
    float* const GXH = lite_store ? ws + y.LGXH + 3 * NF : ws + W.GXH;
    float* const gx_msg = lite_store ? ws + y.LGXB : gx_cur;
    float* const gv_msg = lite_store ? ws + y.LGVB : gv_cur;
    float* const gx_next = lite_store ? (l > 0 ? ws + W.lay[l - 1].LGXA : ws + W.GX) : gx_cur;
    float* const gv_next = lite_store ? (l > 0 ? ws + W.lay[l - 1].LGVA : ws + W.GVb) : gv_oth;
    UpdRevArgs u{};
    u.N = N; u.F = F; u.U = ws + y.UU; u.Y = ws + y.Y; u.S = ws + y.S; u.CAT = ws + y.CAT;
    u.GX = gx_cur; u.GV = gv_cur; u.GY = GY; u.GCAT = GCAT; u.GU = GU;
    u.GX_out = lite_store ? gx_msg : nullptr;
    NQ_TRY(nq_upd_rev(st, u, 1, false));
    float* const GQ = lite_store ? ws + y.LGQ + NF : ws + W.GQ;
    if (lite_store) NQ_TRY(nq_gemm_nn_dsilu2(st, GY, params + up.V2, ws + y.LGQP, GQ, ws + y.ZQ, N, 3 * F, F, "V2"));
    else NQ_TRY(nq_gemm_nn_epi(st, GY, params + up.V2, GQ, N, 3 * F, F, ws + y.ZQ, 0.f, 1.f, 1, "V2"));
    NQ_TRY(nq_gemm_nn(st, GQ, params + up.V1, GCAT, N, F, 2 * F, F, 2 * F, 2 * F, 0, "V1"));
    NQ_TRY(nq_upd_rev(st, u, 2, false));
    if (lite_store) NQ_TRY(nq_gemm_nn_epi(st, GU, params + up.U, gv_msg, 3 * N, 2 * F, F, gv_cur, 1.f, 0.f, 0, "U"));
    else NQ_TRY(nq_gemm_nn(st, GU, params + up.U, gv_cur, 3 * N, 2 * F, F, 2 * F, F, F, 1, "U"));
    MsgRevArgs m{};
    m.g = g; m.F = F; m.V = ws + W.V[l]; m.XH = ws + y.XH; m.PHI = ws + y.PHI; m.PSI = ws + y.PSI;
    m.GX = gx_msg; m.GV = gv_msg; m.GXH = GXH; m.GV_out = gv_next; m.GEDGE = reinterpret_cast<float4*>(ws + W.GEDGE);
    if (W.fused) {
      FilterArgs fa;
      nq_make_filter_args(&fa, ws + y.WRT, params + mp.br, rbf_offsets, ws + W.RW, R, cfg->cutoff, cfg->envelope_exponent, cfg->rbf_coeff, cfg->filter_mode);
      fa.row_ctr = row_ctr(1, l);
      NQ_TRY(nq_msgf_rev(st, m, fa, false));
    } else {
      NQ_TRY(nq_msg_rev(st, m, false));
    }
    float* const GH = lite_store ? ws + y.LGH + NF : ws + W.GH;
    if (lite_store) NQ_TRY(nq_gemm_nn_dsilu2(st, GXH, params + mp.W2, ws + y.LGHP, GH, ws + y.Z1, N, 3 * F, F, "W2"));
    else NQ_TRY(nq_gemm_nn_epi(st, GXH, params + mp.W2, GH, N, 3 * F, F, ws + y.Z1, 0.f, 1.f, 1, "W2"));
    if (lite_store) {
      NQ_TRY(nq_gemm_nn_epi(st, GH, params + mp.W1, gx_next, N, F, F, gx_msg, 1.f, 0.f, 0, "W1"));
      gx_cur = gx_next; gv_cur = gv_next;
    } else {
      { float* t = gv_cur; gv_cur = gv_oth; gv_oth = t; }
      NQ_TRY(nq_gemm_nn(st, GH, params + mp.W1, gx_cur, N, F, F, F, F, F, 1, "W1"));
    }
  }
  NQ_TRY(nq_geom_rev(st, g, reinterpret_cast<const float4*>(ws + W.GEDGE), nwaves, forces));
  return NQ_OK;
}

struct SideStream {
  hipStream_t main = nullptr, side = nullptr;
  bool on = false;
  std::vector<hipEvent_t>* pool = nullptr;
  size_t used = 0;
  bool forked = false, joined = false;
  hipEvent_t last_read[8] = {};
  SideStream() = default;
  SideStream(const SideStream&) = delete;
  SideStream& operator=(const SideStream&) = delete;
  ~SideStream() { if (on && forked && !joined) join(); }
  hipEvent_t next() {
    if (used == pool->size()) { hipEvent_t e; if (hipEventCreateWithFlags(&e, hipEventDisableTiming) != hipSuccess) return nullptr; pool->push_back(e); }
    return (*pool)[used++];
  }
  hipStream_t fork() {
    if (!on) return main;
    hipEvent_t e = next();
    (void)hipEventRecord(e, main); (void)hipStreamWaitEvent(side, e, 0);
    forked = true; joined = false;
    return side;
  }
  void read_by_side(int buf) { if (on) { hipEvent_t e = next(); (void)hipEventRecord(e, side); last_read[buf] = e; } }
  void before_main_writes(int buf) { if (on && last_read[buf]) { (void)hipStreamWaitEvent(main, last_read[buf], 0); last_read[buf] = nullptr; } }
  void join() { if (on) { hipEvent_t e = next(); (void)hipEventRecord(e, side); (void)hipStreamWaitEvent(main, e, 0); joined = true; } }
};
enum { SB_GY = 0, SB_GQ, SB_GU, SB_GXH, SB_GH, SB_GPHI, SB_GBR };
struct SidePool { hipStream_t side = nullptr; std::vector<hipEvent_t> events; };
static std::mutex g_side_mu;
static std::map<std::pair<int, hipStream_t>, SidePool*> g_side_pools;
static void side_stream_init(SideStream& s, hipStream_t main, int n_atoms) {
  s.main = main;
  const char* env = getenv("NQ_SIDE_STREAM");
  const bool want = env && (env[0] == '0' || env[0] == '1') ? env[0] == '1' : n_atoms <= 16384;
  if (!want) return;
  int dev = 0;
  if (hipGetDevice(&dev) != hipSuccess) return;
  std::lock_guard<std::mutex> lock(g_side_mu);
  SidePool*& pool = g_side_pools[std::make_pair(dev, main)];
  if (!pool) {
    SidePool* p = new SidePool();
    if (hipStreamCreateWithFlags(&p->side, hipStreamNonBlocking) != hipSuccess) { delete p; return; }
    pool = p;
  }
  s.side = pool->side; s.pool = &pool->events; s.on = true;
}

static int painn_backward_impl(const nq_painn_cfg* cfg, const float* params, const float* rbf_offsets, const nq_graph* graph, void* workspace,
                               size_t workspace_bytes, const float* grad_energy, const float* grad_forces, float* grad_params, void* stream,
                               bool seeded, const float* seed_x, const float* seed_vec, void* const* layer_events = nullptr) {
  if (!cfg || !graph || !workspace) return nq_fail(NQ_ERR_ARG, "null argument");
  StepPlan plan;
  NQ_TRY(recall_plan(workspace, cfg, graph, &plan));
  WsLayout W; ParamLayout P;
  NQ_TRY(check_common(cfg, graph, workspace, workspace_bytes, plan.fused, &W, &P));
  if (!params || !grad_params || !rbf_offsets) return nq_fail(NQ_ERR_ARG, "null argument");
  hipStream_t st = (hipStream_t)stream;
  float* ws = (float*)workspace;
  float* gp = grad_params;
  float* scr = ws + W.scratch;
  const NqGraphView g = view_of(graph);
  const int N = g.N, E = g.E, F = cfg->hidden_channels, R = cfg->num_rbf, H = F / 2, L = cfg->num_layers, T = cfg->num_elements;
  const size_t NF = (size_t)N * F;
  int* const rowctr0 = reinterpret_cast<int*>(ws + W.ROWCTR);
  NQ_HIP(hipMemsetAsync(rowctr0 + (size_t)2 * L * NQ_ROWCTR_INTS, 0, (size_t)3 * L * NQ_ROWCTR_INTS * sizeof(int), st));
  auto row_ctr = [&](int kind, int l) { return N >= 4096 ? rowctr0 + ((size_t)kind * L + l) * NQ_ROWCTR_INTS : (int*)nullptr; };

  const size_t NH = (size_t)N * H;
  ReadoutArgs r{};
  r.N = N; r.H = H; r.ZO = ws + W.ZO; r.TZO = ws + W.ZO + NH; r.w2 = params + P.w2; r.o2 = params + P.o2;
  r.e_atom = ws + W.e_atom; r.te_atom = ws + W.te_atom;
  if (seeded) {
    auto zero = [&](size_t off, size_t n) { return hipMemsetAsync(ws + off, 0, n * sizeof(float), st); };
    for (int l = 0; l <= L; ++l) { NQ_HIP(zero(W.X[l] + NF, NF)); NQ_HIP(zero(W.V[l] + 3 * NF, 3 * NF)); }
    for (int l = 0; l < L; ++l) {
      const WsLayer& y = W.lay[l];
      NQ_HIP(zero(y.Z1 + NF, NF)); NQ_HIP(zero(y.Hh + NF, NF)); NQ_HIP(zero(y.XH + 3 * NF, 3 * NF)); NQ_HIP(zero(y.XM + NF, NF));
      NQ_HIP(zero(y.VM + 3 * NF, 3 * NF)); NQ_HIP(zero(y.UU + 6 * NF, 6 * NF)); NQ_HIP(zero(y.S + NF, NF)); NQ_HIP(zero(y.CAT + 2 * NF, 2 * NF));
      NQ_HIP(zero(y.ZQ + NF, NF)); NQ_HIP(zero(y.Q + NF, NF)); NQ_HIP(zero(y.Y + 3 * NF, 3 * NF));
    }
    NQ_HIP(zero(W.TD, E)); NQ_HIP(zero(W.TR, 3 * (size_t)E)); NQ_HIP(zero(W.ZO + (size_t)N * H, (size_t)N * H)); NQ_HIP(zero(W.te_atom, N));
  } else {
  if (grad_forces) NQ_TRY(nq_negate(st, grad_forces, ws + W.pos_dot, 3L * N));
  else NQ_HIP(hipMemsetAsync(ws + W.pos_dot, 0, 3 * (size_t)N * sizeof(float), st));
  NQ_TRY(nq_geom_tan(st, g, graph->dst, ws + W.pos_dot, ws + W.TD, ws + W.TR));
  for (int l = 0; l < L; ++l) {
    const WsLayer& y = W.lay[l]; const MsgP& mp = P.msg[l]; const UpdP& up = P.upd[l];
    float* TZ1 = ws + y.Z1 + NF; float* TH = ws + y.Hh + NF; float* TXH = ws + y.XH + 3 * NF;
    NQ_TRY(nq_gemm_nt_dsilu(st, ws + W.X[l] + NF, params + mp.W1, TZ1, TH, ws + y.Z1, N, F, F, "W1"));
    NQ_TRY(nq_gemm_nt(st, TH, params + mp.W2, TXH, nullptr, nullptr, N, 3 * F, F, F, F, 3 * F, "W2"));
    MsgArgs m{};
    m.g = g; m.F = F; m.X = ws + W.X[l]; m.V = ws + W.V[l]; m.XH = ws + y.XH; m.PHI = ws + y.PHI; m.PSI = ws + y.PSI;
    m.TX = ws + W.X[l] + NF; m.TV = ws + W.V[l] + 3 * NF; m.TXH = TXH; m.TD = ws + W.TD; m.TR = ws + W.TR;
    m.TXM = ws + y.XM + NF; m.TVM = ws + y.VM + 3 * NF;
    if (W.fused) {
      FilterArgs fa;
      nq_make_filter_args(&fa, ws + y.WRT, params + mp.br, rbf_offsets, ws + W.RW, R, cfg->cutoff, cfg->envelope_exponent, cfg->rbf_coeff, cfg->filter_mode);
      fa.row_ctr = row_ctr(2, l);
      NQ_TRY(nq_msgf_fwd(st, m, fa, true));
    } else {
      NQ_TRY(nq_msg_fwd(st, m, true));
    }
    UpdArgs u{};
    u.N = N; u.F = F; u.XM = ws + y.XM; u.VM = ws + y.VM; u.U = ws + y.UU; u.Y = ws + y.Y; u.S = ws + y.S; u.CAT = ws + y.CAT;
    u.TXM = ws + y.XM + NF; u.TVM = ws + y.VM + 3 * NF; u.TU = ws + y.UU + 6 * NF; u.TY = ws + y.Y + 3 * NF;
    u.TS = ws + y.S + NF; u.TCAT = ws + y.CAT + 2 * NF; u.TX1 = ws + W.X[l + 1] + NF; u.TV1 = ws + W.V[l + 1] + 3 * NF;
    float* TZQ = ws + y.ZQ + NF; float* TQ = ws + y.Q + NF;
    NQ_TRY(nq_gemm_nt(st, ws + y.VM + 3 * NF, params + up.U, ws + y.UU + 6 * NF, nullptr, nullptr, 3 * N, 2 * F, F, F, F, 2 * F, "U"));
    NQ_TRY(nq_upd_a(st, u, true));
    NQ_TRY(nq_gemm_nt_dsilu(st, ws + y.CAT + 2 * NF, params + up.V1, TZQ, TQ, ws + y.ZQ, N, F, 2 * F, "V1"));
    NQ_TRY(nq_gemm_nt(st, TQ, params + up.V2, ws + y.Y + 3 * NF, nullptr, nullptr, N, 3 * F, F, F, F, 3 * F, "V2"));
    NQ_TRY(nq_upd_b(st, u, true));
  }
  NQ_TRY(nq_gemm_nt(st, ws + W.X[L] + NF, params + P.O1, ws + W.ZO + NH, nullptr, nullptr, N, H, F, F, F, H, "O1"));
  r.N = N; r.H = H; r.ZO = ws + W.ZO; r.TZO = ws + W.ZO + NH; r.w2 = params + P.w2; r.o2 = params + P.o2;
  r.e_atom = ws + W.e_atom; r.te_atom = ws + W.te_atom;
  NQ_TRY(nq_readout(st, r, 1));

  }
  if (grad_energy) NQ_TRY(nq_atom_seeds(st, grad_energy, g.atom_mol, N, ws + W.ge, ws + W.gte));
  else {
    NQ_HIP(hipMemsetAsync(ws + W.ge, 0, (size_t)N * sizeof(float), st));
    NQ_TRY(nq_atom_seeds(st, nullptr, g.atom_mol, N, ws + W.gte, nullptr));
  }
  if (seeded) NQ_HIP(hipMemsetAsync(ws + W.gte, 0, (size_t)N * sizeof(float), st));
  r.ge = ws + W.ge; r.gte = ws + W.gte; r.GZO = ws + W.GZO; r.GTZO = ws + W.GZO + NH; r.TMPW = ws + W.TMPW;
  NQ_TRY(nq_readout_rev(st, r, true));
  const bool lite = plan.lite && !seeded;
  SideStream ss;
  if (plan.gw_mode != GW_MIXED) side_stream_init(ss, st, N);
  hipStream_t sd = ss.fork();
  NQ_TRY(nq_colsum(sd, ws + W.TMPW, N, H, H, gp + P.w2, scr));
  NQ_TRY(nq_colsum(sd, ws + W.ge, N, 1, 1, gp + P.o2, scr));
  NQ_TRY(nq_gemm_tn(sd, ws + W.GZO, ws + W.X[L], gp + P.O1, 2L * N, H, F, H, F, scr, "O1", gp + P.o1, N));
  NQ_TRY(nq_gemm_nn(st, ws + W.GZO, params + P.O1, ws + W.GX, lite ? N : 2 * N, H, F, H, F, F, 0, "O1"));
  float* gv_cur = ws + W.GVa; float* gv_oth = ws + W.GVb;
  NQ_HIP(hipMemsetAsync(gv_cur, 0, (lite ? 3 : 6) * NF * sizeof(float), st));
  if (seeded) {
    if (seed_x) NQ_TRY(nq_axpy(st, seed_x, ws + W.GX, (long)NF));
    if (seed_vec) NQ_HIP(hipMemcpyAsync(gv_cur, seed_vec, 3 * NF * sizeof(float), hipMemcpyDeviceToDevice, st));
  }
  float* gphi = ws + W.GPHI2; float* gpsi = gphi + (size_t)E * 3 * F;
  const bool molgw = plan.gw_mode != GW_PAIR_ROWS, mixed = plan.gw_mode == GW_MIXED;
  const int* const sched = reinterpret_cast<const int*>(ws + W.SCHED);
  const int* const n_big_pairs = sched + nq_molgw_sched_ints(E, g.B) - 1;
  if (molgw) NQ_TRY(nq_molgw_geometry(st, g, ws + W.RW, ws + W.TD, ws + W.TR, sched, ws + W.GWREC));
  if (mixed) NQ_HIP(hipMemsetAsync(ws + W.GBR, 0, 3 * NF * sizeof(float), st));
  for (int l = L - 1; l >= 0; --l) {
    const WsLayer& y = W.lay[l]; const MsgP& mp = P.msg[l]; const UpdP& up = P.upd[l];
    float* const GYs = lite ? ws + y.LGY : ws + W.GY;
    float* const GCATs = lite ? ws + y.LGCAT : ws + W.GCAT;
    float* const GUs = lite ? ws + y.LGU : ws + W.GU;
    float* const GXHs = lite ? ws + y.LGXH : ws + W.GXH;
    float* const GQs = lite ? ws + y.LGQ : ws + W.GQ;
    float* const GHs = lite ? ws + y.LGH : ws + W.GH;
    UpdRevArgs u{};
    u.N = N; u.F = F; u.U = ws + y.UU; u.Y = ws + y.Y; u.S = ws + y.S; u.CAT = ws + y.CAT;
    u.TU = ws + y.UU + 6 * NF; u.TY = ws + y.Y + 3 * NF; u.TS = ws + y.S + NF; u.TCAT = ws + y.CAT + 2 * NF;
    u.GX = ws + W.GX; u.GTX = lite ? ws + y.LGXA : ws + W.GX + NF; u.GV = gv_cur; u.GTV = lite ? ws + y.LGVA : gv_cur + 3 * NF;
    u.GY = GYs; u.GTY = GYs + 3 * NF; u.GCAT = GCATs; u.GTCAT = GCATs + 2 * NF;
    u.GU = GUs; u.GTU = GUs + 6 * NF;
    u.lite = lite ? 1 : 0;
    ss.before_main_writes(SB_GY);
    NQ_TRY(nq_upd_rev(st, u, 1, true));
    sd = ss.fork();
    NQ_TRY(nq_gemm_tn(sd, GYs, ws + y.Q, gp + up.V2, 2L * N, 3 * F, F, 3 * F, F, scr, "V2", gp + up.c2, N));
    ss.read_by_side(SB_GY);
    ss.before_main_writes(SB_GQ);
    NQ_TRY(nq_gemm_nn(st, GYs, params + up.V2, GQs, lite ? N : 2 * N, 3 * F, F, 3 * F, F, F, 0, "V2"));
    NQ_TRY(nq_silu_rev(st, ws + y.ZQ, ws + y.ZQ + NF, GQs, lite ? ws + y.LGQP : GQs + NF, (long)NF, true, lite));
    sd = ss.fork();
    NQ_TRY(nq_gemm_tn(sd, GQs, ws + y.CAT, gp + up.V1, 2L * N, F, 2 * F, F, 2 * F, scr, "V1", gp + up.c1, N));
    ss.read_by_side(SB_GQ);
    NQ_TRY(nq_gemm_nn(st, GQs, params + up.V1, GCATs, lite ? N : 2 * N, F, 2 * F, F, 2 * F, 2 * F, 0, "V1"));
    ss.before_main_writes(SB_GU);
    NQ_TRY(nq_upd_rev(st, u, 2, true));
    sd = ss.fork();
    NQ_TRY(nq_gemm_tn(sd, GUs, ws + y.VM, gp + up.U, 6L * N, 2 * F, F, 2 * F, F, scr, "U"));
    ss.read_by_side(SB_GU);
    NQ_TRY(nq_gemm_nn(st, GUs, params + up.U, gv_cur, lite ? 3 * N : 6 * N, 2 * F, F, 2 * F, F, F, 1, "U"));
    MsgRevArgs m{};
    m.g = g; m.F = F; m.V = ws + W.V[l]; m.XH = ws + y.XH; m.PHI = ws + y.PHI; m.PSI = ws + y.PSI;
    m.TV = ws + W.V[l] + 3 * NF; m.TXH = ws + y.XH + 3 * NF; m.TD = ws + W.TD; m.TR = ws + W.TR;
    m.GX = ws + W.GX; m.GV = gv_cur; m.GTX = lite ? ws + y.LGXB : ws + W.GX + NF; m.GTV = lite ? ws + y.LGVB : gv_cur + 3 * NF;
    m.GXH = GXHs; m.GTXH = GXHs + 3 * NF; m.GV_out = gv_oth; m.GTV_out = gv_oth + 3 * NF;
    m.lite = lite ? 1 : 0;
    m.GPHI = gphi; m.GPSI = gpsi; m.GBR = ws + W.GBR;
    ss.before_main_writes(SB_GXH); ss.before_main_writes(SB_GPHI); ss.before_main_writes(SB_GBR);
    if (W.fused) {
      FilterArgs fa;
      nq_make_filter_args(&fa, ws + y.WRT, params + mp.br, rbf_offsets, ws + W.RW, R, cfg->cutoff, cfg->envelope_exponent, cfg->rbf_coeff, cfg->filter_mode);
      fa.row_ctr = row_ctr(3, l);
      m.mol_cap = plan.gw_cap;
      m.row_filter = mixed ? 1 : 0;
      NQ_TRY(nq_msgf_rev(st, m, fa, true, !molgw));
      if (mixed) {
        m.row_filter = 2;
        fa.row_ctr = row_ctr(4, l);
        NQ_TRY(nq_msgf_rev(st, m, fa, true, true));
        NQ_TRY(nq_gwr_sorted(st, gphi, gpsi, ws + W.RW, reinterpret_cast<const int*>(ws + W.ORDER), E / 2, F, R, gp + mp.Wr, scr, 3, n_big_pairs));
        NQ_TRY(nq_colsum(st, ws + W.GBR, N, 3 * F, 3 * F, gp + mp.br, scr));
      }
      if (molgw)
        NQ_TRY(nq_gwr_mol(st, g, F, R, plan.gw_cap, m.XH, m.V, m.TXH, m.TV, m.GX, m.GV, m.GTX, m.GTV, sched, ws + W.GWREC, ws + W.GWPART, gp + mp.Wr, gp + mp.br, mixed));
    } else {
      NQ_TRY(nq_msg_rev(st, m, true));
    }
    { float* t = gv_cur; gv_cur = gv_oth; gv_oth = t; }
    sd = ss.fork();
    if (W.fused && !molgw) NQ_TRY(nq_gwr_sorted(sd, gphi, gpsi, ws + W.RW, reinterpret_cast<const int*>(ws + W.ORDER), E / 2, F, R, gp + mp.Wr, scr));
    else if (!W.fused) NQ_TRY(nq_gemm_tn(sd, gphi, ws + W.RHO2, gp + mp.Wr, 2L * E, 3 * F, R, 3 * F, R, scr, "Wr"));
    if (cfg->rbf_type)
      NQ_TRY(nq_gemm_nn(st, gphi, params + mp.Wr, ws + W.GRHO, 2 * E, 3 * F, R, 3 * F, R, R, l == L - 1 ? 0 : 1, "Wr"));
    if (!molgw) NQ_TRY(nq_colsum(sd, ws + W.GBR, N, 3 * F, 3 * F, gp + mp.br, scr));
    NQ_TRY(nq_gemm_tn(sd, GXHs, ws + y.Hh, gp + mp.W2, 2L * N, 3 * F, F, 3 * F, F, scr, "W2", gp + mp.b2, N));
    ss.read_by_side(SB_GPHI); ss.read_by_side(SB_GBR); ss.read_by_side(SB_GXH);
    ss.before_main_writes(SB_GH);
    NQ_TRY(nq_gemm_nn(st, GXHs, params + mp.W2, GHs, lite ? N : 2 * N, 3 * F, F, 3 * F, F, F, 0, "W2"));
    NQ_TRY(nq_silu_rev(st, ws + y.Z1, ws + y.Z1 + NF, GHs, lite ? ws + y.LGHP : GHs + NF, (long)NF, true, lite));
    sd = ss.fork();
    NQ_TRY(nq_gemm_tn(sd, GHs, ws + W.X[l], gp + mp.W1, 2L * N, F, F, F, F, scr, "W1", gp + mp.b1, N));
    ss.read_by_side(SB_GH);
    NQ_TRY(nq_gemm_nn(st, GHs, params + mp.W1, ws + W.GX, lite ? N : 2 * N, F, F, F, F, F, 1, "W1"));
    if (layer_events && layer_events[L - 1 - l]) NQ_HIP(hipEventRecord((hipEvent_t)layer_events[L - 1 - l], ss.on ? ss.side : st));
  }
  ss.join();
  NQ_TRY(nq_embed_grad(st, g.z, ws + W.GX, N, F, T, gp + P.emb, scr));
  if (cfg->rbf_type) {
    NQ_TRY(nq_rbf_param_grad(st, g.geom, E, R, cfg->cutoff, cfg->envelope_exponent, rbf_offsets, cfg->rbf_type, params + P.basis, ws + W.GRHO, ws + W.BCON));
    if (cfg->rbf_type == 1) NQ_TRY(nq_colsum(st, ws + W.BCON, E, R, R, gp + P.basis, scr));
    else NQ_TRY(nq_colsum(st, ws + W.BCON, (long)E * R, 1, 1, gp + P.basis, scr));
  }
  return NQ_OK;
}

int nq_painn_backward(const nq_painn_cfg* cfg, const float* params, const float* rbf_offsets, const nq_graph* graph, void* workspace,
                      size_t workspace_bytes, const float* grad_energy, const float* grad_forces, float* grad_params, void* stream) {
  return painn_backward_impl(cfg, params, rbf_offsets, graph, workspace, workspace_bytes, grad_energy, grad_forces, grad_params, stream, false, nullptr,
                             nullptr);
}
int nq_painn_backward_events(const nq_painn_cfg* cfg, const float* params, const float* rbf_offsets, const nq_graph* graph, void* workspace,
                             size_t workspace_bytes, const float* grad_energy, const float* grad_forces, float* grad_params, void* const* layer_events_host,
                             void* stream) {
  return painn_backward_impl(cfg, params, rbf_offsets, graph, workspace, workspace_bytes, grad_energy, grad_forces, grad_params, stream, false, nullptr,
                             nullptr, layer_events_host);
}
int nq_painn_layer_param_ranges(const nq_painn_cfg* cfg, int64_t* ranges_host) {
  ParamLayout P;
  if (!cfg || !ranges_host) return nq_fail(NQ_ERR_ARG, "null argument");
  NQ_TRY(make_param_layout(cfg, &P));
  const int L = cfg->num_layers;
  for (int l = 0; l < L; ++l) {
    const size_t m0 = P.msg[l].W1, m1 = l + 1 < L ? P.msg[l + 1].W1 : P.upd[0].U;
    const size_t u0 = P.upd[l].U, u1 = l + 1 < L ? P.upd[l + 1].U : P.O1;
    ranges_host[4 * l + 0] = (int64_t)m0; ranges_host[4 * l + 1] = (int64_t)(m1 - m0);
    ranges_host[4 * l + 2] = (int64_t)u0; ranges_host[4 * l + 3] = (int64_t)(u1 - u0);
  }
  ranges_host[4 * L + 0] = (int64_t)P.O1; ranges_host[4 * L + 1] = (int64_t)(P.total - P.O1);
  ranges_host[4 * L + 2] = 0; ranges_host[4 * L + 3] = (int64_t)P.msg[0].W1;
  return NQ_OK;
}
int nq_painn_backward_seeded(const nq_painn_cfg* cfg, const float* params, const float* rbf_offsets, const nq_graph* graph, void* workspace,
                             size_t workspace_bytes, const float* grad_energy, const float* grad_x, const float* grad_vec, float* grad_params,
                             void* stream) {
  return painn_backward_impl(cfg, params, rbf_offsets, graph, workspace, workspace_bytes, grad_energy, nullptr, grad_params, stream, true, grad_x,
                             grad_vec);
}

int nq_loss_l1_l2(const float* energy, const float* y, int32_t B, const float* forces, const float* f_target, int32_t N, float coef_e,
                  float coef_f, float* loss, float* grad_energy, float* grad_forces, void* stream) {
  if (!energy || !y || !forces || !f_target || !loss || !grad_energy || !grad_forces) return nq_fail(NQ_ERR_ARG, "null argument");
  return nq_loss_impl((hipStream_t)stream, energy, y, B, forces, f_target, N, coef_e, coef_f, loss, grad_energy, grad_forces, false);
}
int nq_loss_mse(const float* energy, const float* y, int32_t B, const float* forces, const float* f_target, int32_t N, float coef_e,
                  float coef_f, float* loss, float* grad_energy, float* grad_forces, void* stream) {
  if (!energy || !y || !forces || !f_target || !loss || !grad_energy || !grad_forces) return nq_fail(NQ_ERR_ARG, "null argument");
  return nq_loss_impl((hipStream_t)stream, energy, y, B, forces, f_target, N, coef_e, coef_f, loss, grad_energy, grad_forces, true);
}

int nq_adamw_step(float* params, const float* grads, float* exp_avg, float* exp_avg_sq, size_t count, float max_norm, float lr, float beta1,
                  float beta2, float eps, float weight_decay, int32_t step, float* scratch, void* stream) {
  if (!params || !grads || !exp_avg || !exp_avg_sq || !scratch || step < 1) return nq_fail(NQ_ERR_ARG, "bad argument");
  return nq_adamw_impl((hipStream_t)stream, params, grads, exp_avg, exp_avg_sq, (long)count, max_norm, lr, beta1, beta2, eps, weight_decay,
                       step, scratch);
}

int nq_linear_forward(const float* A, const float* Wt, const float* bias, float* C, float* C_silu, int32_t M, int32_t N, int32_t K, void* stream) {
  return nq_gemm_nt((hipStream_t)stream, A, Wt, C, bias, C_silu, M, N, K, K, K, N);
}
int nq_linear_forward_act(const float* A, const float* Wt, float* C, float* C_act, const float* resid, float alpha, float beta, int32_t M, int32_t N, int32_t K,
                          void* stream) {
  if (!A || !Wt || !C || !C_act) return nq_fail(NQ_ERR_ARG, "null argument");
  return nq_gemm_nt_act((hipStream_t)stream, A, Wt, C, C_act, resid, alpha, beta, M, N, K);
}
int nq_linear_forward_res(const float* A, const float* Wt, const float* aux, float alpha, float* C, int32_t M, int32_t N, int32_t K, void* stream) {
  if (!A || !Wt || !C || !aux) return nq_fail(NQ_ERR_ARG, "null argument");
  if (aux == C) return nq_fail(NQ_ERR_ARG, "nq_linear_forward_res: aux must not alias C");
  return nq_gemm_nt_res((hipStream_t)stream, A, Wt, C, aux, alpha, M, N, K);
}
int nq_linear_input_grad(const float* G, const float* Wt, float* C, int32_t M, int32_t N, int32_t K, int32_t accumulate, void* stream) {
  return nq_gemm_nn((hipStream_t)stream, G, Wt, C, M, N, K, N, K, K, accumulate);
}
int nq_linear_input_grad_epi(const float* G, const float* Wt, float* C, int32_t M, int32_t N, int32_t K, const float* aux, float alpha, float beta, int32_t mode,
                             void* stream) {
// ... 19 lines not shown
```

### nabladft_amd/csrc/molpair.hip

```cpp
#include "common.h"
#include "lanes.h"
#include <type_traits>

#ifndef GM_THREADS
#define GM_THREADS 512
#endif
#define GM_STAGE_THREADS 512
#define GM_NW (GM_THREADS / 64)
#define GM_ROWS 32
#define GM_WMAX (GM_ROWS - 1 - (FWIN - 1))
#define GM_CH 32
#define GM_BATCH 8
#ifndef GM_ATOM_PAD
#define GM_ATOM_PAD 4
#endif
#define GM_ATOM_FLOATS (20 * GM_CH + GM_ATOM_PAD)
#define GM_ATOM_BYTES (GM_ATOM_FLOATS * 4)
#define GM_RING_BYTES 512
#define GM_MAX_ATOMS ((160 * 1024 - GM_NW * GM_RING_BYTES) / GM_ATOM_BYTES)
#define GM_PART_FLOATS (GM_ROWS * 3 * GM_CH)
#define GM_MAX_BINS 128
#define GM_PA_DWORDS (2 * 64 * 4)
#define GM_PG_DWORDS 64
#ifndef GM_STAGE_EARLY
// ... 125 lines not shown
      const int forced_end = w == GM_NW - 1 ? np : cnt[min(GM_MAX_BINS, wlo[w + 1])];
      const int optional_end = min(cur + target, cnt[min(GM_MAX_BINS, wlo[w] + GM_WMAX)]);
      const int end = max(cur, max(forced_end, optional_end));
      nb += (end - cur + GM_BATCH - 1) / GM_BATCH;
      cur = end;
    }
    cut[GM_NW] = np; bst[GM_NW] = nb;
  }
  __syncthreads();
  if (lane <= GM_NW) sched_ptr[(long)m * (GM_NW + 1) + lane] = cut[lane];
  if (lane < GM_NW) {
    const int len = cut[lane + 1] - cut[lane];
    seg[(long)m * GM_NW + lane] = make_int2(b0 + bst[lane], len);
    for (int i = len; i < (bst[lane + 1] - bst[lane]) * GM_BATCH; ++i) sched[(long)GM_BATCH * (b0 + bst[lane]) + i] = make_int2(-1, 0);
  }
  pair_sched_pass<true>(g, dst, RW, wlo, cut, bst, b0, a0, s0, s1, lane, cnt, sched);
}

__global__ __launch_bounds__(256) void k_pair_arec(const int2* __restrict__ sched, const int2* __restrict__ seg, const float* __restrict__ RW,
                                                    const float* __restrict__ TD, int nseg, u4* __restrict__ PA) {
  const int wid = blockIdx.x * 4 + (threadIdx.x >> 6), sg = wid >> 2, lane = threadIdx.x & 63;
  if (sg >= nseg) return;
  const int2 se = seg[sg];
  const int nb = (se.y + GM_BATCH - 1) / GM_BATCH, j = lane & 31, sub = lane >> 5;
  const int half = TD != nullptr ? 1 : 0, olane = half * 32 + j;
  for (int b = (wid & 3) * 2 + sub; b < nb; b += 8) {
    const long batch = se.x + b;
    float v[GM_BATCH];
#pragma unroll
    for (int i = 0; i < GM_BATCH; ++i) {
      const int2 en = sched[batch * GM_BATCH + i];
      const int off = (int)((unsigned)en.y >> 26);
      const int t = j - off;
      const bool valid = en.x >= 0 && (((unsigned)t < (unsigned)FWIN) | (j == 31));
      const int tap = j == 31 ? 14 : min(max(t, 0), FWIN - 1);
      v[i] = valid ? RW[(long)max(en.x, 0) * RW_STRIDE + half * 16 + tap] * (TD ? TD[max(en.x, 0)] : 1.0f) : 0.f;
    }
    unsigned hi[4], lo[4];
#pragma unroll
    for (int i = 0; i < 4; ++i) gm_split2(v[2 * i], v[2 * i + 1], hi[i], lo[i]);
    PA[(batch * 2 + 0) * 64 + olane] = u4{hi[0], hi[1], hi[2], hi[3]};
    PA[(batch * 2 + 1) * 64 + olane] = u4{lo[0], lo[1], lo[2], lo[3]};
  }
}
__global__ __launch_bounds__(256) void k_pair_grec(const int2* __restrict__ sched, const int2* __restrict__ seg, const float4* __restrict__ geom,
                                                    const float* __restrict__ TR, int nseg, float* __restrict__ PG) {
  const int wid = blockIdx.x * 4 + (threadIdx.x >> 6), sg = wid >> 2, lane = threadIdx.x & 63;
  if (sg >= nseg) return;
  const int2 se = seg[sg];
  const int nb = (se.y + GM_BATCH - 1) / GM_BATCH, i = lane >> 3, f = lane & 7;
  for (int b = wid & 3; b < nb; b += 4) {
    const long batch = se.x + b;
    const int2 en = sched[batch * GM_BATCH + i];
    float v = 0.f;
    if (en.x >= 0) {
      if (f < 3) v = reinterpret_cast<const float*>(geom)[4 * (long)en.x + f];
      else if (f == 3) v = 0.f;
      else if (f < 7) v = TR[3 * (long)en.x + (f - 4)];
      else v = __int_as_float((((en.y >> 13) & 0x1fff) << 16) | (en.y & 0x1fff));
    }
    PG[batch * GM_PG_DWORDS + lane] = v;
  }
}

struct GwrMolArgs {
  NqGraphView g; int F; int nslices; int groups; int max_atoms;
  const float* XH; const float* V; const float* TXH; const float* TV;
  const float* GX; const float* GV; const float* GTX; const float* GTV;
  const int2* seg;
  const int* order;
  float* part;
};

template <bool DIFF>
__device__ __forceinline__ float gm_pair_sum(float x, float y) {
  if (GM_ABLATE & 16) return DIFF ? y - x : x + y;
  const auto r = __builtin_amdgcn_permlane32_swap(__float_as_uint(x), __float_as_uint(y), false, false);
  return DIFF ? __uint_as_float(r[1]) - __uint_as_float(r[0]) : __uint_as_float(r[0]) + __uint_as_float(r[1]);
}

struct GmOps { f4 P0, P1, P2, A, T; };
struct GmRec { u4 hi, lo; };

__global__ __launch_bounds__(GM_THREADS) void k_gwr_mol(GwrMolArgs q, const u4* __restrict__ PA, const unsigned* __restrict__ PG) {
  extern __shared__ __attribute__((aligned(16))) float rows[];
  const int F = q.F, F3 = 3 * q.F;
  int slice = blockIdx.x % q.nslices, group = blockIdx.x / q.nslices;
  if (q.groups % 8 == 0) { const int x = blockIdx.x & 7, r = blockIdx.x >> 3; slice = r % q.nslices; group = (r / q.nslices) * 8 + x; }
  const int wave = __builtin_amdgcn_readfirstlane(threadIdx.x >> 6), lane = threadIdx.x & 63;
  const int half = lane >> 5, c = lane & 31;
  const int cb = slice * GM_CH;
  f16v acc0, acc1, acc2;
#pragma unroll
  for (int r = 0; r < 16; ++r) acc0[r] = acc1[r] = acc2[r] = 0.f;
  const unsigned hmask = half ? 0xffffffffu : 0u;
  const unsigned lbase = (unsigned)(c * 16);
  char* const ring = reinterpret_cast<char*>(rows) + (size_t)q.max_atoms * GM_ATOM_BYTES + wave * GM_RING_BYTES;

  const int st_at = threadIdx.x >> 3, st_qd = threadIdx.x & 7;
  const bool stager = threadIdx.x < GM_STAGE_THREADS;
  auto blk_load = [&](int blk, int a0, int na, f4 (&r)[4]) __attribute__((always_inline)) {
    const float* s0; const float* s1; const float* s2; const float* s3;
    int st3 = F3;
    switch (blk) {
      case 0: s0 = q.XH; s1 = q.XH + F; s2 = q.XH + 2 * F; s3 = q.TXH; break;
      case 1: s0 = q.TXH + F; s1 = q.TXH + 2 * F; s2 = q.V; s3 = q.V + F; break;
      case 2: s0 = q.V + 2 * F; s1 = q.TV; s2 = q.TV + F; s3 = q.TV + 2 * F; break;
      case 3: s0 = q.GV; s1 = q.GV + F; s2 = q.GV + 2 * F; s3 = q.GX; st3 = F; break;
      default: s0 = q.GTV; s1 = q.GTV + F; s2 = q.GTV + 2 * F; s3 = q.GTX; st3 = F; break;
    }
    const long n = a0 + min(st_at, na - 1), o = n * F3 + cb + 4 * st_qd;
    r[0] = *reinterpret_cast<const f4*>(s0 + o); r[1] = *reinterpret_cast<const f4*>(s1 + o); r[2] = *reinterpret_cast<const f4*>(s2 + o);
    r[3] = *reinterpret_cast<const f4*>(s3 + n * st3 + cb + 4 * st_qd);
  };
  auto blk_store = [&](int blk, int na, const f4 (&r)[4]) __attribute__((always_inline)) {
    if (st_at < na) {
      float* d = rows + st_at * GM_ATOM_FLOATS + blk * (GM_CH * 4) + (4 * st_qd) * 4;
#pragma unroll
      for (int i = 0; i < 4; ++i) *reinterpret_cast<f4*>(d + i * 4) = f4{r[0][i], r[1][i], r[2][i], r[3][i]};
    }
  };
  auto ops_load = [&](GmOps& o, unsigned nk) __attribute__((always_inline)) {
    const unsigned no = (nk >> 16) * GM_ATOM_BYTES, ko = (nk & 0xffffu) * GM_ATOM_BYTES;
    const unsigned x = (no ^ ko) & hmask;
    const char* ps = reinterpret_cast<const char*>(rows) + ((no ^ x) + lbase);
    const char* pt = reinterpret_cast<const char*>(rows) + ((ko ^ x) + lbase);
    if (GM_ABLATE & 8) { const float z = __uint_as_float((no ^ x) + lbase); o.P0 = o.P1 = o.P2 = f4{z, z, 1.f, 2.f}; o.A = o.T = f4{1.f, z, __uint_as_float((ko ^ x) + lbase), 3.f}; return; }
    o.P0 = *reinterpret_cast<const f4*>(ps);
    o.P1 = *reinterpret_cast<const f4*>(ps + GM_CH * 16);
    o.P2 = *reinterpret_cast<const f4*>(ps + 2 * GM_CH * 16);
    o.A = *reinterpret_cast<const f4*>(pt + 3 * GM_CH * 16);
    o.T = *reinterpret_cast<const f4*>(pt + 4 * GM_CH * 16);
  };
  auto rec_load = [&](GmRec& r, long batch) __attribute__((always_inline)) {
    r.hi = PA[(batch * 2 + 0) * 64 + lane];
    r.lo = PA[(batch * 2 + 1) * 64 + lane];
  };
  auto geo_load = [&](long batch) __attribute__((always_inline)) -> unsigned { return PG[batch * GM_PG_DWORDS + lane]; };
  auto ring_put = [&](int slot, unsigned g) __attribute__((always_inline)) { *reinterpret_cast<unsigned*>(ring + slot * 256 + lane * 4) = g; };
  auto ring_lo = [&](int slot, int i) __attribute__((always_inline)) -> f4 { return *reinterpret_cast<const f4*>(ring + slot * 256 + i * 32); };
  auto ring_hi = [&](int slot, int i) __attribute__((always_inline)) -> f4 { return *reinterpret_cast<const f4*>(ring + slot * 256 + i * 32 + 16); };
  unsigned bh[3][4], bl[3][4];
#pragma unroll
  for (int p_ = 0; p_ < 3; ++p_)
#pragma unroll
    for (int j = 0; j < 4; ++j) bh[p_][j] = bl[p_][j] = 0u;
  auto batch = [&](const GmRec& rc, int slot, int live, bool more, GmOps& L0, GmOps& L1, f4& gc) __attribute__((always_inline)) {
    auto step = [&](int i, GmOps& cur, GmOps& nxt, float& ba, float& bb, float& bc) __attribute__((always_inline)) {
      const f4 gn = ring_hi(i < GM_BATCH - 1 ? slot : slot ^ 1, (i + 1) & 7);
      const f4 g0 = ring_lo(slot, i);
      unsigned nkn = (unsigned)__builtin_amdgcn_readfirstlane(__float_as_int(gn[3]));
      if (i == GM_BATCH - 1 && !more) nkn = 0;
      ops_load(nxt, nkn);
      const float gx = g0[0], gy = g0[1], gz = g0[2], t0 = gc[0], t1 = gc[1], t2 = gc[2];
      const f4 P0 = cur.P0, P1 = cur.P1, P2 = cur.P2, A = cur.A, T = cur.T;
      const float xa = P0[0], xb = P0[1], xc = P0[2], txa = P0[3], txb = P1[0], txc = P1[1], v0 = P1[2], v1 = P1[3], v2 = P2[0], tv0 = P2[1],
                  tv1 = P2[2], tv2 = P2[3];
      float ga, gb, gcc, ha, hb, hc;
      if (GM_ABLATE & 4) { ga = xa + gx; gb = xb + txa; gcc = xc + A[0]; ha = txb + T[0]; hb = v2 + gy + t0; hc = tv2 + v1 + t1 + t2 + gz + txc + v0 + tv0 + tv1; }
      else {
        const float gmb = A[0] * v0 + A[1] * v1 + A[2] * v2 + (T[0] * tv0 + T[1] * tv1 + T[2] * tv2);
        const float gtmb = T[0] * v0 + T[1] * v1 + T[2] * v2;
        const float gmc = (A[0] * gx + A[1] * gy + A[2] * gz) + (T[0] * t0 + T[1] * t1 + T[2] * t2);
        const float gtmc = T[0] * gx + T[1] * gy + T[2] * gz;
        const float gma = A[3], gtma = T[3];
        ga = gma * xa + gtma * txa; gb = gmb * xb + gtmb * txb; gcc = gmc * xc + gtmc * txc;
        ha = gtma * xa; hb = gtmb * xb; hc = gtmc * xc;
      }
      ba = gm_pair_sum<false>(ga, ha); bb = gm_pair_sum<false>(gb, hb); bc = gm_pair_sum<true>(gcc, hc);
      gc = gn;
    };
    if (!(GM_ABLATE & 1)) {
#pragma unroll
      for (int j = 0; j < GM_BATCH / 2; ++j) {
        if (!(GM_ABLATE & 256) && 2 * j >= live) break;
        float a0_, b0_, c0_, a1_, b1_, c1_;
        step(2 * j, L0, L1, a0_, b0_, c0_);
        step(2 * j + 1, L1, L0, a1_, b1_, c1_);
        gm_split2(a0_, a1_, bh[0][j], bl[0][j]);
        gm_split2(b0_, b1_, bh[1][j], bl[1][j]);
        gm_split2(c0_, c1_, bh[2][j], bl[2][j]);
      }
    }
    if (!(GM_ABLATE & 2)) {
      const gm_bf8 ah = __builtin_bit_cast(gm_bf8, rc.hi), al = __builtin_bit_cast(gm_bf8, rc.lo);
      const gm_bf8 h0 = __builtin_bit_cast(gm_bf8, (u4{bh[0][0], bh[0][1], bh[0][2], bh[0][3]})), l0 = __builtin_bit_cast(gm_bf8, (u4{bl[0][0], bl[0][1], bl[0][2], bl[0][3]}));
      const gm_bf8 h1 = __builtin_bit_cast(gm_bf8, (u4{bh[1][0], bh[1][1], bh[1][2], bh[1][3]})), l1 = __builtin_bit_cast(gm_bf8, (u4{bl[1][0], bl[1][1], bl[1][2], bl[1][3]}));
      const gm_bf8 h2 = __builtin_bit_cast(gm_bf8, (u4{bh[2][0], bh[2][1], bh[2][2], bh[2][3]})), l2 = __builtin_bit_cast(gm_bf8, (u4{bl[2][0], bl[2][1], bl[2][2], bl[2][3]}));
      acc0 = __builtin_amdgcn_mfma_f32_32x32x16_bf16(al, h0, acc0, 0, 0, 0);
      acc1 = __builtin_amdgcn_mfma_f32_32x32x16_bf16(al, h1, acc1, 0, 0, 0);
      acc2 = __builtin_amdgcn_mfma_f32_32x32x16_bf16(al, h2, acc2, 0, 0, 0);
      acc0 = __builtin_amdgcn_mfma_f32_32x32x16_bf16(ah, l0, acc0, 0, 0, 0);
      acc1 = __builtin_amdgcn_mfma_f32_32x32x16_bf16(ah, l1, acc1, 0, 0, 0);
      acc2 = __builtin_amdgcn_mfma_f32_32x32x16_bf16(ah, l2, acc2, 0, 0, 0);
      acc0 = __builtin_amdgcn_mfma_f32_32x32x16_bf16(ah, h0, acc0, 0, 0, 0);
      acc1 = __builtin_amdgcn_mfma_f32_32x32x16_bf16(ah, h1, acc1, 0, 0, 0);
      acc2 = __builtin_amdgcn_mfma_f32_32x32x16_bf16(ah, h2, acc2, 0, 0, 0);
    } else { acc0[0] += __uint_as_float(bh[0][0] ^ bl[1][1] ^ bh[2][2] ^ bl[0][3] ^ bh[1][0] ^ bl[2][1] ^ bh[0][1] ^ bl[0][0] ^ bh[1][2] ^ bl[1][3] ^ bh[2][0] ^ bl[2][3] ^ rc.hi[0] ^ rc.lo[1]); }
  };

  int rpos = -1;
  auto next_mol = [&]() __attribute__((always_inline)) -> int {
    for (++rpos;; ++rpos) {
      const long idx = (long)rpos * q.groups + ((rpos & 1) ? q.groups - 1 - group : group);
      if (idx >= q.g.B) return q.g.B;
      const int mm = q.order ? q.order[idx] : (int)idx;
      if (q.g.mol_ptr[mm + 1] - q.g.mol_ptr[mm] <= q.max_atoms) return mm;
    }
  };
  int m = next_mol();
  if (m < q.g.B && stager) {
    const int a0 = __builtin_amdgcn_readfirstlane(q.g.mol_ptr[m]), na = __builtin_amdgcn_readfirstlane(q.g.mol_ptr[m + 1]) - a0;
#pragma unroll
    for (int blk = 0; blk < 5; ++blk) { f4 r[4]; blk_load(blk, a0, na, r); blk_store(blk, na, r); }
  }
  GmRec RX, RY;
  unsigned gq0 = 0, gq1 = 0;
  int2 sg = make_int2(0, 0);
  if (m < q.g.B) {
    sg = q.seg[(long)m * GM_NW + wave];
    sg.x = __builtin_amdgcn_readfirstlane(sg.x); sg.y = __builtin_amdgcn_readfirstlane(sg.y);
    rec_load(RX, sg.x); gq0 = geo_load(sg.x); gq1 = geo_load(sg.x + 1);
  }
  while (m < q.g.B) {
    const int mn = next_mol();
    int a0n = 0, nan = 1;
    int2 sgn_ = make_int2(0, 0);
    if (mn < q.g.B) {
      a0n = __builtin_amdgcn_readfirstlane(q.g.mol_ptr[mn]); nan = __builtin_amdgcn_readfirstlane(q.g.mol_ptr[mn + 1]) - a0n;
      sgn_ = q.seg[(long)mn * GM_NW + wave];
      sgn_.x = __builtin_amdgcn_readfirstlane(sgn_.x); sgn_.y = __builtin_amdgcn_readfirstlane(sgn_.y);
    }
    if (!(GM_ABLATE & 128)) __syncthreads();
    const int nb = (sg.y + GM_BATCH - 1) / GM_BATCH;
    if (nb > 0) {
      const long b0 = sg.x, last = b0 + nb - 1;
      GmOps L0, L1;
      ring_put(0, gq0);
      f4 gc = ring_hi(0, 0);
      ops_load(L0, (unsigned)__builtin_amdgcn_readfirstlane(__float_as_int(gc[3])));
      int left = sg.y;
#pragma nounroll
      for (long b = b0; b <= last; b += 2) {
        ring_put(1, gq1);
        rec_load(RY, min(b + 1, last));
        gq0 = geo_load(min(b + 2, last));
        __builtin_amdgcn_sched_barrier(0);
        batch(RX, 0, min(left, GM_BATCH), b < last, L0, L1, gc);
        if (b + 1 > last) break;
        ring_put(0, gq0);
        rec_load(RX, min(b + 2, last));
        gq1 = geo_load(min(b + 3, last));
        __builtin_amdgcn_sched_barrier(0);
        batch(RY, 1, min(left - GM_BATCH, GM_BATCH), b + 1 < last, L0, L1, gc);
        left -= 2 * GM_BATCH;
      }
    }
    f4 stg[5][4];
    if (GM_STAGE_EARLY && mn < q.g.B && stager) {
#pragma unroll
      for (int blk = 0; blk < 5; ++blk) blk_load(blk, a0n, nan, stg[blk]);
    }
    if (mn < q.g.B) { rec_load(RX, sgn_.x); gq0 = geo_load(sgn_.x); gq1 = geo_load(sgn_.x + 1); }
    if (!(GM_ABLATE & 128)) __syncthreads();
    if (mn < q.g.B && stager) {
#pragma unroll
      for (int blk = 0; blk < 5; ++blk) {
        if (!GM_STAGE_EARLY) blk_load(blk, a0n, nan, stg[blk]);
        blk_store(blk, nan, stg[blk]);
      }
    }
    m = mn; sg = sgn_;
  }
  float* out = q.part + ((long)(group * q.nslices + slice) * GM_NW + wave) * GM_PART_FLOATS;
#pragma unroll
  for (int r = 0; r < 16; ++r) {
    const int row = (r & 3) + 8 * (r >> 2) + 4 * half;
    out[(row * 3 + 0) * GM_CH + c] = acc0[r];
    out[(row * 3 + 1) * GM_CH + c] = acc1[r];
    out[(row * 3 + 2) * GM_CH + c] = acc2[r];
  }
}

#define GMR_Q 4
__global__ __launch_bounds__(256) void k_gwr_mol_reduce(const float* __restrict__ part, const int* __restrict__ wlo, int groups, int nslices, int R, int F,
                                                        float* __restrict__ gWr, float* __restrict__ gbr, int acc) {
  __shared__ float red[GMR_Q][256 / GMR_Q];
  const int e = threadIdx.x & (256 / GMR_Q - 1), qd = threadIdx.x / (256 / GMR_Q);
  const int idx = blockIdx.x * (256 / GMR_Q) + e;
  const int F3 = 3 * F;
  const bool live = idx < (R + 1) * F3;
  const int k = live ? idx / F3 : 0, col = live ? idx % F3 : 0;
  const int p = col / F, ch = col % F, slice = ch / GM_CH, c = ch % GM_CH;
  const int gper = (groups + GMR_Q - 1) / GMR_Q, g0 = min(groups, qd * gper), g1 = min(groups, g0 + gper);
  float s = 0.f;
  if (live)
    for (int w = 0; w < GM_NW; ++w) {
      int row = GM_ROWS - 1;
      if (k < R) {
        row = k - wlo[w];
        if (row < 0 || row >= GM_ROWS - 1) continue;
      }
      const int o = (row * 3 + p) * GM_CH + c;
#pragma unroll 8
      for (int g = g0; g < g1; ++g) s += part[((long)(g * nslices + slice) * GM_NW + w) * GM_PART_FLOATS + o];
    }
  red[qd][e] = s;
  __syncthreads();
  if (qd != 0 || !live) return;
  s = (red[0][e] + red[1][e]) + (red[2][e] + red[3][e]);
  if (k < R) gWr[(long)col * R + k] = acc ? gWr[(long)col * R + k] + s : s;
  else gbr[col] = acc ? gbr[col] + s : s;
}

#define GM_ORDER_MAX 32768
__global__ __launch_bounds__(1024) void k_mol_order(NqGraphView g, int cap, int n2, int* __restrict__ order) {
  extern __shared__ unsigned okeys[];
  for (int i = threadIdx.x; i < n2; i += 1024) {
    unsigned key = 0;
    if (i < g.B) {
      const int a0 = g.mol_ptr[i], a1 = g.mol_ptr[i + 1];
      const int pairs = a1 - a0 <= cap ? g.lowptr[a1] - g.lowptr[a0] : 0;
      key = ((unsigned)min(pairs, 2047) << 20) | (0xFFFFFu - (unsigned)i);
    }
    okeys[i] = key;
  }
  __syncthreads();
  for (int k = 2; k <= n2; k <<= 1)
    for (int j = k >> 1; j > 0; j >>= 1) {
      for (int i = threadIdx.x; i < n2; i += 1024) {
        const int x = i ^ j;
        if (x > i) {
          const unsigned a = okeys[i], b = okeys[x];
          const bool desc = (i & k) == 0;
          if ((a < b) == desc) { okeys[i] = b; okeys[x] = a; }
        }
      }
      __syncthreads();
    }
  for (int i = threadIdx.x; i < g.B; i += 1024) order[i] = (int)(0xFFFFFu - (okeys[i] & 0xFFFFFu));
}

int nq_molgw_max_atoms(void) { return GM_MAX_ATOMS; }
bool nq_molgw_config_ok(int F, int R) {
  return F % GM_CH == 0 && R >= FWIN && R - FWIN + 1 <= GM_NW * GM_WMAX && R - FWIN + 1 <= GM_MAX_BINS;
}
bool nq_molgw_supported(int F, int R, int max_mol_atoms) {
  return nq_molgw_config_ok(F, R) && max_mol_atoms > 0 && max_mol_atoms <= GM_MAX_ATOMS;
}
static int molgw_groups(int B, int nslices) {
  int groups = 256 / nslices;
  if (groups < 1) groups = 1;
  if (groups > B) groups = B;
  return groups;
}
size_t nq_molgw_sched_ints(int E, int B) {
  return 2 * GM_BATCH * gm_max_batches(E, B) + 2 * (size_t)B * GM_NW + (size_t)B * (GM_NW + 1) + GM_MAX_BINS + GM_NW + 1 + (size_t)B + 16;
}
size_t nq_molgw_sched_slots(int E, int B) { return GM_BATCH * gm_max_batches(E, B); }
size_t nq_molgw_rec_floats(int E, int B) { return gm_max_batches(E, B) * (GM_PA_DWORDS + GM_PG_DWORDS) + 16; }
size_t nq_molgw_part_floats(int F, int B) { const int ns = F / GM_CH; return (size_t)molgw_groups(B, ns) * ns * GM_NW * GM_PART_FLOATS; }

struct MolGwBufs { int2* sched; int2* seg; int* sched_ptr; int* hist; int* wlo; int* order; };
static MolGwBufs molgw_bufs(int* base, int E, int B) {
  MolGwBufs b;
  b.sched = reinterpret_cast<int2*>(base);
  b.seg = b.sched + GM_BATCH * gm_max_batches(E, B);
  b.sched_ptr = reinterpret_cast<int*>(b.seg + (size_t)B * GM_NW);
  b.hist = b.sched_ptr + (size_t)B * (GM_NW + 1);
  b.wlo = b.hist + GM_MAX_BINS;
  b.order = B <= GM_ORDER_MAX ? b.wlo + GM_NW + 1 : nullptr;
  return b;
}

int nq_molgw_schedule(hipStream_t st, const NqGraphView& g, const int* dst, const float* RW, int R, int cap, int* sched_ints, float* recs) {
  NQ_PROF(st, "pair_schedule");
  const MolGwBufs b = molgw_bufs(sched_ints, g.E, g.B);
  NQ_HIP(hipMemsetAsync(b.hist, 0, GM_MAX_BINS * sizeof(int), st));
  int blocks = nq_cdiv(g.E, 256 * 8);
  blocks = blocks < 1 ? 1 : (blocks > 1024 ? 1024 : blocks);
  hipLaunchKernelGGL(k_pair_hist, dim3(blocks), dim3(256), 0, st, RW, dst, g.col, g.E, b.hist);
  NQ_LAUNCH_CHECK();
  hipLaunchKernelGGL(k_pair_windows, dim3(1), dim3(64), 0, st, b.hist, R - FWIN + 1, b.wlo);
  NQ_LAUNCH_CHECK();
  hipLaunchKernelGGL(k_pair_sched, dim3(g.B), dim3(64), 0, st, g, dst, RW, b.wlo, cap < GM_MAX_ATOMS ? cap : GM_MAX_ATOMS, b.sched, b.sched_ptr, b.seg);
  NQ_LAUNCH_CHECK();
  if (b.order) {
    int n2 = 1;
    while (n2 < g.B) n2 <<= 1;
    const size_t lds = (size_t)n2 * sizeof(unsigned);
    NQ_DYN_LDS(k_mol_order, lds);
    hipLaunchKernelGGL(k_mol_order, dim3(1), dim3(1024), lds, st, g, cap < GM_MAX_ATOMS ? cap : GM_MAX_ATOMS, n2, b.order);
    NQ_LAUNCH_CHECK();
  }
  const int nseg = g.B * GM_NW;
  hipLaunchKernelGGL(k_pair_arec, dim3(nseg), dim3(256), 0, st, b.sched, b.seg, RW, (const float*)nullptr, nseg, reinterpret_cast<u4*>(recs));
  NQ_LAUNCH_CHECK();
  return NQ_OK;
}
int nq_molgw_geometry(hipStream_t st, const NqGraphView& g, const float* RW, const float* TD, const float* TR, const int* sched_ints, float* recs) {
  NQ_PROF(st, "pair_geometry");
  const MolGwBufs b = molgw_bufs(const_cast<int*>(sched_ints), g.E, g.B);
  float* PG = recs + gm_max_batches(g.E, g.B) * GM_PA_DWORDS;
  const int nseg = g.B * GM_NW;
  hipLaunchKernelGGL(k_pair_grec, dim3(nseg), dim3(256), 0, st, b.sched, b.seg, g.geom, TR, nseg, PG);
  NQ_LAUNCH_CHECK();
  hipLaunchKernelGGL(k_pair_arec, dim3(nseg), dim3(256), 0, st, b.sched, b.seg, RW, TD, nseg, reinterpret_cast<u4*>(recs));
  NQ_LAUNCH_CHECK();
  return NQ_OK;
}

int nq_gwr_mol(hipStream_t st, const NqGraphView& g, int F, int R, int max_mol_atoms, const float* XH, const float* V, const float* TXH, const float* TV,
               const float* GX, const float* GV, const float* GTX, const float* GTV, const int* sched_ints, const float* recs, float* part, float* gWr,
               float* gbr, bool accumulate) {
  NQ_PROF(st, "gwr_mol");
  const MolGwBufs b = molgw_bufs(const_cast<int*>(sched_ints), g.E, g.B);
  GwrMolArgs q;
  q.g = g; q.F = F; q.nslices = F / GM_CH; q.groups = molgw_groups(g.B, q.nslices);
  q.max_atoms = max_mol_atoms < GM_MAX_ATOMS ? max_mol_atoms : GM_MAX_ATOMS;
  q.XH = XH; q.V = V; q.TXH = TXH; q.TV = TV; q.GX = GX; q.GV = GV; q.GTX = GTX; q.GTV = GTV;
  q.seg = b.seg; q.order = b.order; q.part = part;
  const u4* PA = reinterpret_cast<const u4*>(recs);
  const unsigned* PG = reinterpret_cast<const unsigned*>(recs + gm_max_batches(g.E, g.B) * GM_PA_DWORDS);
  const size_t lds = (size_t)q.max_atoms * GM_ATOM_BYTES + GM_NW * GM_RING_BYTES;
  NQ_DYN_LDS(k_gwr_mol, lds);
  hipLaunchKernelGGL(k_gwr_mol, dim3(q.groups * q.nslices), dim3(GM_THREADS), lds, st, q, PA, PG);
  NQ_LAUNCH_CHECK();
  hipLaunchKernelGGL(k_gwr_mol_reduce, dim3(nq_cdiv((long)(R + 1) * 3 * F, 256 / GMR_Q)), dim3(256), 0, st, part, b.wlo, q.groups, q.nslices, R, F, gWr, gbr, accumulate ? 1 : 0);
  NQ_LAUNCH_CHECK();
  return NQ_OK;
}
```

Before: 47210 conformer-steps/s.

## Specialise layer-0 message kernels to skip terms zeroed by empty vector features

Adds layer-0 template variants of the fused message forward, reverse and per-molecule filter-gradient kernels. At layer 0 the vector features V (and their tangents) are zero, so the b-channel filter, the V loads, and the corresponding MFMA accumulations and LDS staging blocks are dropped. The aim is less memory traffic and arithmetic in the first interaction layer of forward, tangent and backward passes. It adds more kernel instantiations and relies on the caller passing layer0 only when V is truly zero.

Result: faster. 48840 conformer-steps/s, median of 6 (+3.5%).

```diff
diff --git a/nabladft_amd/csrc/common.h b/nabladft_amd/csrc/common.h
--- a/nabladft_amd/csrc/common.h
+++ b/nabladft_amd/csrc/common.h
@@ -197,8 +197,8 @@
 size_t nq_gwr_scratch_floats(int E, int F, int R, int parts = 3);
 int nq_gwr_sorted(hipStream_t, const float* GPHI, const float* GPSI, const float* RW, const int* order, int E, int F, int R, float* gWr,
                   float* scratch, int parts = 3, const int* count_dev = nullptr);
-int nq_msgf_fwd(hipStream_t, const MsgArgs&, const FilterArgs&, bool tangent);
-int nq_msgf_rev(hipStream_t, const MsgRevArgs&, const FilterArgs&, bool dual, bool pair_rows = true);
+int nq_msgf_fwd(hipStream_t, const MsgArgs&, const FilterArgs&, bool tangent, bool layer0 = false);
+int nq_msgf_rev(hipStream_t, const MsgRevArgs&, const FilterArgs&, bool dual, bool pair_rows = true, bool layer0 = false);
 int nq_molgw_max_atoms(void);
 bool nq_molgw_config_ok(int F, int R);
 bool nq_molgw_supported(int F, int R, int max_mol_atoms);
@@ -210,7 +210,7 @@
 int nq_molgw_geometry(hipStream_t, const NqGraphView&, const float* RW, const float* TD, const float* TR, const int* sched_ints, float* recs);
 int nq_gwr_mol(hipStream_t, const NqGraphView&, int F, int R, int max_mol_atoms, const float* XH, const float* V, const float* TXH, const float* TV,
                const float* GX, const float* GV, const float* GTX, const float* GTV, const int* sched_ints, const float* recs, float* part, float* gWr,
-               float* gbr, bool accumulate = false);
+               float* gbr, bool accumulate = false, bool layer0 = false);
 int nq_msg_rev(hipStream_t, const MsgRevArgs&, bool dual);
 int nq_geom_tan(hipStream_t, const NqGraphView&, const int* dst, const float* pos_dot, float* TD, float* TR);
 int nq_geom_rev(hipStream_t, const NqGraphView&, const float4* GEDGE, int nwaves, float* forces);
diff --git a/nabladft_amd/csrc/edge.hip b/nabladft_amd/csrc/edge.hip
--- a/nabladft_amd/csrc/edge.hip
+++ b/nabladft_amd/csrc/edge.hip
@@ -228,7 +228,8 @@
 #ifndef NQ_DUALNG2_THREADS
 #define NQ_DUALNG2_THREADS 768
 #endif
-__host__ __device__ constexpr int fused_threads(int kind, int ch) {
+__host__ __device__ constexpr int fused_threads(int kind, int ch, bool l0 = false) {
+  if (l0) return ch >= 4 ? 512 : 1024;
   return ch >= 4 ? 512
                  : (ch == 2 ? (kind == 3 ? NQ_DUAL2_THREADS : (kind == 4 ? NQ_DUALNG2_THREADS : (kind == 1 ? NQ_TAN2_THREADS : 1024)))
                             : (kind >= 3 ? 768 : 1024));
@@ -330,26 +331,41 @@
     if (NEED_T) { r.td = TD[sp]; r.t0 = TR[3 * (long)sp]; r.t1 = TR[3 * (long)sp + 1]; r.t2 = TR[3 * (long)sp + 2]; }
   }
 }
-template <bool PSI, int CH>
+template <bool PSI, int CH, int PM = 7, int QM = 7>
 __device__ __forceinline__ void filter_eval(const WinRegs<PSI>& w, const float* wrt, int F, int F3, int fb, const float (&bra)[CH],
                                             const float (&brb)[CH], const float (&brc)[CH], float (&pa)[CH], float (&pb)[CH], float (&pc)[CH],
                                             float (&qa)[CH], float (&qb)[CH], float (&qc)[CH]) {
   typedef VOps<CH> O;
   typedef typename O::V V;
+  constexpr int QMM = PSI ? QM : 0, TM = PM | QMM;
+  constexpr bool PA = (PM & 1) != 0, PB = (PM & 2) != 0, PC = (PM & 4) != 0, QA = (QMM & 1) != 0, QB = (QMM & 2) != 0, QC = (QMM & 4) != 0;
   const V ba = O::from(bra), bb = O::from(brb), bc = O::from(brc);
-  V va = ba * O::splat(w.rr[14]), vb = bb * O::splat(w.rr[14]), vc = bc * O::splat(w.rr[14]);
-  V ua = O::splat(0.f), ub = ua, uc = ua;
-  if (PSI) { ua = ba * O::splat(w.dd[14]); ub = bb * O::splat(w.dd[14]); uc = bc * O::splat(w.dd[14]); }
+  V va = O::splat(0.f), vb = va, vc = va, ua = va, ub = va, uc = va;
+  if (PA) va = ba * O::splat(w.rr[14]);
+  if (PB) vb = bb * O::splat(w.rr[14]);
+  if (PC) vc = bc * O::splat(w.rr[14]);
+  if (QA) ua = ba * O::splat(w.dd[14]);
+  if (QB) ub = bb * O::splat(w.dd[14]);
+  if (QC) uc = bc * O::splat(w.dd[14]);
   const int k0 = __builtin_amdgcn_readfirstlane(__float_as_int(w.rr[13]));
   const float* wk = wrt + k0 * F3 + fb;
 #pragma unroll
   for (int t = 0; t < FWIN; ++t) {
-    const V wa = lds_tap<CH>(wk + t * F3), wb = lds_tap<CH>(wk + t * F3 + F), wc = lds_tap<CH>(wk + t * F3 + 2 * F);
-    const V r = O::splat(w.rr[t]);
-    va = O::fma(wa, r, va); vb = O::fma(wb, r, vb); vc = O::fma(wc, r, vc);
-    if (PSI) {
+    V wa = va, wb = va, wc = va;
+    if (TM & 1) wa = lds_tap<CH>(wk + t * F3);
+    if (TM & 2) wb = lds_tap<CH>(wk + t * F3 + F);
+    if (TM & 4) wc = lds_tap<CH>(wk + t * F3 + 2 * F);
+    if (PM) {
+      const V r = O::splat(w.rr[t]);
+      if (PA) va = O::fma(wa, r, va);
+      if (PB) vb = O::fma(wb, r, vb);
+      if (PC) vc = O::fma(wc, r, vc);
+    }
+    if (QMM) {
       const V d = O::splat(w.dd[t]);
-      ua = O::fma(wa, d, ua); ub = O::fma(wb, d, ub); uc = O::fma(wc, d, uc);
+      if (QA) ua = O::fma(wa, d, ua);
+      if (QB) ub = O::fma(wb, d, ub);
+      if (QC) uc = O::fma(wc, d, uc);
     }
   }
   O::to(pa, va); O::to(pb, vb); O::to(pc, vc);
@@ -431,9 +447,13 @@
   __amdgpu_buffer_rsrc_t xh, v, txh, tv;
   __device__ __forceinline__ FwdSrc(const MsgArgs& q) : xh(row_rsrc(q.XH)), v(row_rsrc(q.V)), txh(row_rsrc(TAN ? q.TXH : q.XH)), tv(row_rsrc(TAN ? q.TV : q.V)) {}
 };
-template <bool TAN, int CH>
+template <bool TAN, int CH, bool L0 = false>
 __device__ __forceinline__ void load_fwd(FwdOps<TAN, CH>& o, const FwdSrc<TAN>& src, int k, int F, int F3, int fb) {
   const int ob = fb * 4, r0 = k * F3 * 4, r1 = r0 + F * 4, r2 = r1 + F * 4;
+  if (L0) {
+    ldv_buf<CH>(o.xa, src.xh, ob, r0); ldv_buf<CH>(o.xc, src.xh, ob, r2);
+    return;
+  }
   ldv_buf<CH>(o.xa, src.xh, ob, r0); ldv_buf<CH>(o.xb, src.xh, ob, r1); ldv_buf<CH>(o.xc, src.xh, ob, r2);
   ldv_buf<CH>(o.va, src.v, ob, r0); ldv_buf<CH>(o.vb, src.v, ob, r1); ldv_buf<CH>(o.vc, src.v, ob, r2);
   if (TAN) {
@@ -442,8 +462,8 @@
   }
 }
 
-template <bool TAN, int CH>
-__global__ __launch_bounds__(fused_threads(TAN ? 1 : 0, CH)) void k_msgf_fwd(MsgArgs q, FilterArgs fa, const float* __restrict__ RW) {
+template <bool TAN, int CH, bool L0 = false>
+__global__ __launch_bounds__(fused_threads(TAN ? 1 : 0, CH, L0)) void k_msgf_fwd(MsgArgs q, FilterArgs fa, const float* __restrict__ RW) {
   FUSED_PROLOGUE
   const FwdSrc<TAN> src(q);
   FUSED_ROWS(TAN ? 1 : 0) {
@@ -456,14 +476,15 @@
       RowRegs row;
       load_row<TAN>(row, q.g, q.TD, q.TR, RW, c0, cnt, lane);
       FwdOps<TAN, CH> opA, opB;
-      load_fwd<TAN, CH>(opA, src, bl_i(row.kk, 0), F, F3, fb);
+      load_fwd<TAN, CH, L0>(opA, src, bl_i(row.kk, 0), F, F3, fb);
       WinRegs<TAN> win;
       load_win<TAN>(win, RW, c0);
       auto step = [&](FwdOps<TAN, CH>& cur, FwdOps<TAN, CH>& nxt, int j, auto prefetch) __attribute__((always_inline)) {
         const int jn = min(j + 1, cnt - 1);
-        if (decltype(prefetch)::value) load_fwd<TAN, CH>(nxt, src, bl_i(row.kk, jn), F, F3, fb);
+        if (decltype(prefetch)::value) load_fwd<TAN, CH, L0>(nxt, src, bl_i(row.kk, jn), F, F3, fb);
         float pa[CH], pb[CH], pc[CH], qa[CH], qb[CH], qc[CH];
-        filter_eval<TAN, CH>(win, wrt, FL, 3 * FL, lfb, bra, brb, brc, pa, pb, pc, qa, qb, qc);
+        if (L0) filter_eval<TAN, CH, (TAN ? 4 : 5), 5>(win, wrt, FL, 3 * FL, lfb, bra, brb, brc, pa, pb, pc, qa, qb, qc);
+        else filter_eval<TAN, CH>(win, wrt, FL, 3 * FL, lfb, bra, brb, brc, pa, pb, pc, qa, qb, qc);
         __builtin_amdgcn_sched_barrier(0);
         if (decltype(prefetch)::value) load_win<TAN>(win, RW, c0 + jn);
         const float gx = bl_f(row.gx, j), gy = bl_f(row.gy, j), gz = bl_f(row.gz, j);
@@ -471,6 +492,21 @@
         if (TAN) { td = bl_f(row.td, j); tr0 = bl_f(row.t0, j); tr1 = bl_f(row.t1, j); tr2 = bl_f(row.t2, j); }
 #pragma unroll
         for (int c = 0; c < CH; ++c) {
+          if (L0) {
+            const float mc = cur.xc[c] * pc[c];
+            if (!TAN) {
+              const float m0 = mc * gx, m1 = mc * gy, m2 = mc * gz;
+              dx[c] += cur.xa[c] * pa[c];
+              d0[c] += m0; d1[c] += m1; d2[c] += m2;
+            } else {
+              const float tma = cur.xa[c] * (qa[c] * td), tmc = cur.xc[c] * (qc[c] * td);
+              dx[c] += tma;
+              d0[c] += fmaf(mc, tr0, tmc * gx);
+              d1[c] += fmaf(mc, tr1, tmc * gy);
+              d2[c] += fmaf(mc, tr2, tmc * gz);
+            }
+            continue;
+          }
           const float mb = cur.xb[c] * pb[c], mc = cur.xc[c] * pc[c];
           if (!TAN) {
             dx[c] += cur.xa[c] * pa[c];
@@ -499,7 +535,11 @@
     }
     const long o = (long)n * F + fb, o3 = (long)n * F3 + fb;
     float x0[CH], w0[CH], w1[CH], w2[CH];
-    if (!TAN) {
+    if (L0) {
+#pragma unroll
+      for (int c = 0; c < CH; ++c) x0[c] = w0[c] = w1[c] = w2[c] = 0.f;
+      if (!TAN) ldv<CH>(x0, q.X + o);
+    } else if (!TAN) {
       ldv<CH>(x0, q.X + o); ldv<CH>(w0, q.V + o3); ldv<CH>(w1, q.V + o3 + F); ldv<CH>(w2, q.V + o3 + 2 * F);
     } else {
       ldv<CH>(x0, q.TX + o); ldv<CH>(w0, q.TV + o3); ldv<CH>(w1, q.TV + o3 + F); ldv<CH>(w2, q.TV + o3 + 2 * F);
@@ -555,7 +595,7 @@
 #ifndef NQ_DUAL_KX_EARLY
 #define NQ_DUAL_KX_EARLY 1
 #endif
-template <bool DUAL, int CH, bool GW, bool LITE = false>
+template <bool DUAL, int CH, bool GW, bool LITE = false, bool L0 = false>
 __device__ __forceinline__ void msgf_rev_body(const MsgRevArgs& q, const FilterArgs& fa, const float* __restrict__ RW) {
   FUSED_PROLOGUE
   const RevSrc<DUAL> src(q);
@@ -569,10 +609,16 @@
     const int nlow = (DUAL && GW) ? __builtin_amdgcn_readfirstlane(q.g.lowptr[n + 1]) - __builtin_amdgcn_readfirstlane(q.g.lowptr[n]) : 0;
     const long o3 = (long)n * F3 + fb;
     float xa[CH], xb[CH], xc[CH], v0[CH], v1[CH], v2[CH], txa[CH], txb[CH], txc[CH], tv0[CH], tv1[CH], tv2[CH];
-    ldv<CH>(xa, q.XH + o3); ldv<CH>(xb, q.XH + o3 + F); ldv<CH>(xc, q.XH + o3 + 2 * F);
-    ldv<CH>(v0, q.V + o3); ldv<CH>(v1, q.V + o3 + F); ldv<CH>(v2, q.V + o3 + 2 * F);
+    if (L0) {
+#pragma unroll
+      for (int c = 0; c < CH; ++c) xa[c] = xb[c] = xc[c] = v0[c] = v1[c] = v2[c] = 0.f;
+      if (!DUAL) { ldv<CH>(xa, q.XH + o3); ldv<CH>(xc, q.XH + o3 + 2 * F); }
+    } else {
+      ldv<CH>(xa, q.XH + o3); ldv<CH>(xb, q.XH + o3 + F); ldv<CH>(xc, q.XH + o3 + 2 * F);
+      ldv<CH>(v0, q.V + o3); ldv<CH>(v1, q.V + o3 + F); ldv<CH>(v2, q.V + o3 + 2 * F);
+    }
     float nA0[CH], nA1[CH], nA2[CH], ngma[CH], nT0[CH], nT1[CH], nT2[CH], ngtma[CH];
-    if (DUAL) {
+    if (DUAL && !L0) {
       ldv<CH>(txa, q.TXH + o3); ldv<CH>(txb, q.TXH + o3 + F); ldv<CH>(txc, q.TXH + o3 + 2 * F);
       ldv<CH>(tv0, q.TV + o3); ldv<CH>(tv1, q.TV + o3 + F); ldv<CH>(tv2, q.TV + o3 + 2 * F);
 #if NQ_DUAL_NA_RESIDENT
@@ -586,6 +632,7 @@
 #pragma unroll
       for (int c = 0; c < CH; ++c) txa[c] = txb[c] = txc[c] = tv0[c] = tv1[c] = tv2[c] = 0.f;
     }
+    static_assert(!L0 || !GW, "the pair-row flavour has no layer-0 form");
     float gxa[CH], gxb[CH], gxc[CH], gv0[CH], gv1[CH], gv2[CH], gtxa[CH], gtxb[CH], gtxc[CH], gtv0[CH], gtv1[CH], gtv2[CH], sba[CH], sbb[CH], sbc[CH];
 #pragma unroll
     for (int c = 0; c < CH; ++c) {
@@ -621,7 +668,8 @@
 #pragma unroll
         for (int c = 0; c < CH; ++c) { pa[c] = bra[c] * win.rr[0]; pb[c] = brb[c] * win.rr[1]; pc[c] = brc[c] * win.rr[2]; qa[c] = bra[c] * win.dd[0]; qb[c] = brb[c] * win.dd[1]; qc[c] = brc[c] * win.dd[2]; }
 #else
-        filter_eval<true, CH>(win, wrt, FL, 3 * FL, lfb, bra, brb, brc, pa, pb, pc, qa, qb, qc);
+        if (L0) filter_eval<true, CH, 5, 5>(win, wrt, FL, 3 * FL, lfb, bra, brb, brc, pa, pb, pc, qa, qb, qc);
+        else filter_eval<true, CH>(win, wrt, FL, 3 * FL, lfb, bra, brb, brc, pa, pb, pc, qa, qb, qc);
 #endif
         const float beta = win.rr[14], dbeta = win.dd[14];
         __builtin_amdgcn_sched_barrier(0);
@@ -641,6 +689,21 @@
 #pragma unroll
         for (int c = 0; c < CH; ++c) {
           const float A0 = cur.A0[c], A1 = cur.A1[c], A2 = cur.A2[c], gma = cur.gma[c];
+          if (L0) {
+            float gmc = A0 * r0 + A1 * r1 + A2 * r2;
+            if (DUAL) {
+              const float T0 = cur.T0[c], T1 = cur.T1[c], T2 = cur.T2[c], gtma = cur.gtma[c];
+              gmc += T0 * tr0 + T1 * tr1 + T2 * tr2;
+              const float gtmc = T0 * r0 + T1 * r1 + T2 * r2;
+              gxa[c] += gma * pa[c] + gtma * (qa[c] * td); gxc[c] += gmc * pc[c] + gtmc * (qc[c] * td);
+            } else {
+              const float mc = xc[c] * pc[c];
+              gxa[c] += gma * pa[c]; gxc[c] += gmc * pc[c];
+              gd += fmaf(gmc * xc[c], qc[c], gma * xa[c] * qa[c]);
+              e0 += A0 * mc; e1 += A1 * mc; e2 += A2 * mc;
+            }
+            continue;
+          }
           const float mb = xb[c] * pb[c], mc = xc[c] * pc[c];
           float gmb = A0 * v0[c] + A1 * v1[c] + A2 * v2[c];
           float gmc = A0 * r0 + A1 * r1 + A2 * r2;
@@ -743,6 +806,7 @@
     }
     float g0[CH], g1[CH], g2[CH];
     stv<CH>(q.GXH + o3, gxa); stv<CH>(q.GXH + o3 + F, gxb); stv<CH>(q.GXH + o3 + 2 * F, gxc);
+    if (L0) continue;
     ldv<CH>(g0, q.GV + o3); ldv<CH>(g1, q.GV + o3 + F); ldv<CH>(g2, q.GV + o3 + 2 * F);
 #pragma unroll
     for (int c = 0; c < CH; ++c) { g0[c] += gv0[c]; g1[c] += gv1[c]; g2[c] += gv2[c]; }
@@ -764,6 +828,10 @@
 template <bool DUAL, int CH>
 __global__ __launch_bounds__(fused_threads(DUAL ? 3 : 2, CH)) void k_msgf_rev(MsgRevArgs q, FilterArgs fa, const float* __restrict__ RW) {
   msgf_rev_body<DUAL, CH, DUAL>(q, fa, RW);
+}
+template <bool DUAL, int CH>
+__global__ __launch_bounds__(fused_threads(DUAL ? 4 : 2, CH, true)) void k_msgf_rev_l0(MsgRevArgs q, FilterArgs fa, const float* __restrict__ RW) {
+  msgf_rev_body<DUAL, CH, false, DUAL, true>(q, fa, RW);
 }
 template <bool LITE, int CH>
 __global__ __launch_bounds__(fused_threads(4, CH)) void k_msgf_rev_nopair(MsgRevArgs q, FilterArgs fa, const float* __restrict__ RW) {
@@ -1108,43 +1176,51 @@
   return groups * nslices;
 }
 
-#define FUSED_LAUNCH(KERN, FLAG, CHV, Q)                                                                          \
+#define FUSED_LAUNCH(KERN, Q, ...)                                                                                \
   do {                                                                                                            \
-    NQ_DYN_LDS((KERN<FLAG, CHV>), lds);                                                                           \
-    hipLaunchKernelGGL((KERN<FLAG, CHV>), dim3(grid), dim3(threads), lds, st, Q, fa, fa.RW);                      \
+    NQ_DYN_LDS((KERN<__VA_ARGS__>), lds);                                                                         \
+    hipLaunchKernelGGL((KERN<__VA_ARGS__>), dim3(grid), dim3(threads), lds, st, Q, fa, fa.RW);                    \
   } while (0)
-#define FUSED_DISPATCH(KERN, FLAG, Q)                                   \
+#define FUSED_DISPATCH_CH(Q, LAUNCH1, LAUNCH2, LAUNCH4)                 \
   do {                                                                  \
     switch (ch) {                                                       \
-      case 1: FUSED_LAUNCH(KERN, FLAG, 1, Q); break;                    \
-      case 2: FUSED_LAUNCH(KERN, FLAG, 2, Q); break;                    \
-      case 4: FUSED_LAUNCH(KERN, FLAG, 4, Q); break;                    \
+      case 1: LAUNCH1; break;                                           \
+      case 2: LAUNCH2; break;                                           \
+      case 4: LAUNCH4; break;                                           \
       default: return nq_fail(NQ_ERR_ARG, "fused message kernels need hidden_channels in {64,128,256}"); \
     }                                                                   \
   } while (0)
-
-int nq_msgf_fwd(hipStream_t st, const MsgArgs& q, const FilterArgs& fa, bool tangent) {
-  NQ_PROF(st, tangent ? "msgf_tan" : "msgf_fwd");
+#define FUSED_DISPATCH(KERN, FLAG, Q) FUSED_DISPATCH_CH(Q, FUSED_LAUNCH(KERN, Q, FLAG, 1), FUSED_LAUNCH(KERN, Q, FLAG, 2), FUSED_LAUNCH(KERN, Q, FLAG, 4))
+#define FUSED_DISPATCH_FWD_L0(FLAG, Q) \
+  FUSED_DISPATCH_CH(Q, FUSED_LAUNCH(k_msgf_fwd, Q, FLAG, 1, true), FUSED_LAUNCH(k_msgf_fwd, Q, FLAG, 2, true), FUSED_LAUNCH(k_msgf_fwd, Q, FLAG, 4, true))
+
+int nq_msgf_fwd(hipStream_t st, const MsgArgs& q, const FilterArgs& fa, bool tangent, bool layer0) {
+  NQ_PROF(st, tangent ? (layer0 ? "msgf_tan_l0" : "msgf_tan") : (layer0 ? "msgf_fwd_l0" : "msgf_fwd"));
   if (q.g.N <= 0) return NQ_OK;
   if ((size_t)q.g.N * 3 * q.F * 4 >= 0xfffff000ull) return nq_fail(NQ_ERR_ARG, "fused message kernels: a node array of %d atoms x %d channels exceeds the 4 GB a buffer descriptor's scalar offset reaches", q.g.N, 3 * q.F);
   int threads; size_t lds;
   const int ch = fused_ch(tangent ? 1 : 0, q.F, q.g.N);
-  const int grid = fused_grid(q.g.N, q.F, ch, &threads, &lds, fa.R, fused_threads(tangent ? 1 : 0, ch));
-  if (tangent) FUSED_DISPATCH(k_msgf_fwd, true, q);
+  const int grid = fused_grid(q.g.N, q.F, ch, &threads, &lds, fa.R, fused_threads(tangent ? 1 : 0, ch, layer0));
+  if (layer0 && tangent) FUSED_DISPATCH_FWD_L0(true, q);
+  else if (layer0) FUSED_DISPATCH_FWD_L0(false, q);
+  else if (tangent) FUSED_DISPATCH(k_msgf_fwd, true, q);
   else FUSED_DISPATCH(k_msgf_fwd, false, q);
   NQ_LAUNCH_CHECK();
   return NQ_OK;
 }
 
-int nq_msgf_rev(hipStream_t st, const MsgRevArgs& q, const FilterArgs& fa, bool dual, bool pair_rows) {
-  NQ_PROF(st, dual ? (pair_rows ? "msgf_rev_dual" : "msgf_rev_dual_ng") : "msgf_rev_force");
+int nq_msgf_rev(hipStream_t st, const MsgRevArgs& q, const FilterArgs& fa, bool dual, bool pair_rows, bool layer0) {
+  layer0 = layer0 && (!dual || (!pair_rows && q.lite));
+  NQ_PROF(st, dual ? (pair_rows ? "msgf_rev_dual" : (layer0 ? "msgf_rev_dual_ng_l0" : "msgf_rev_dual_ng")) : (layer0 ? "msgf_rev_force_l0" : "msgf_rev_force"));
   if (q.g.N <= 0) return NQ_OK;
   if ((size_t)q.g.N * 3 * q.F * 4 >= 0xfffff000ull) return nq_fail(NQ_ERR_ARG, "fused message kernels: a node array of %d atoms x %d channels exceeds the 4 GB a buffer descriptor's scalar offset reaches", q.g.N, 3 * q.F);
   int threads; size_t lds;
   const int kind = dual ? (pair_rows ? 3 : 4) : 2;
   const int ch = fused_ch(dual ? 3 : 2, q.F, q.g.N);
-  const int grid = fused_grid(q.g.N, q.F, ch, &threads, &lds, fa.R, fused_threads(kind, ch));
-  if (dual && !pair_rows && q.lite) FUSED_DISPATCH(k_msgf_rev_nopair, true, q);
+  const int grid = fused_grid(q.g.N, q.F, ch, &threads, &lds, fa.R, fused_threads(kind, ch, layer0));
+  if (layer0 && dual) FUSED_DISPATCH(k_msgf_rev_l0, true, q);
+  else if (layer0) FUSED_DISPATCH(k_msgf_rev_l0, false, q);
+  else if (dual && !pair_rows && q.lite) FUSED_DISPATCH(k_msgf_rev_nopair, true, q);
   else if (dual && !pair_rows) FUSED_DISPATCH(k_msgf_rev_nopair, false, q);
   else if (dual) FUSED_DISPATCH(k_msgf_rev, true, q);
   else FUSED_DISPATCH(k_msgf_rev, false, q);
diff --git a/nabladft_amd/csrc/engine.hip b/nabladft_amd/csrc/engine.hip
--- a/nabladft_amd/csrc/engine.hip
+++ b/nabladft_amd/csrc/engine.hip
@@ -164,6 +164,7 @@
   int gw_mode, gw_cap;
   bool lite;
   bool fused_update;
+  bool layer0;
 };
 static StepPlan plan_step(const nq_painn_cfg* c, const nq_graph* g, bool want_forces) {
   auto env_on = [](const char* name) { const char* v = getenv(name); return v && v[0] == '1'; };
@@ -177,6 +178,7 @@
     p.gw_mode = g->max_mol_atoms <= p.gw_cap ? GW_MOLECULE : GW_MIXED;
   p.lite = p.fused && want_forces && !env_on("NQ_NO_LITE");
   p.fused_update = nq_updfuse_frag_floats(c->hidden_channels) > 0 && !env_on("NQ_NO_FUSED_UPDATE") && !nq_gemm_exact_f32_requested();
+  p.layer0 = !env_on("NQ_NO_LAYER0");
   return p;
 }
 static bool plan_fused(const nq_painn_cfg* c, int32_t N, int32_t E, int32_t B) {
@@ -188,9 +190,18 @@
 struct StepRecord { nq_painn_cfg cfg; int32_t N, E, B, max_mol_atoms; StepPlan plan; };
 static std::mutex g_plan_mu;
 static std::map<const void*, StepRecord> g_plans;
+static StepRecord g_last_plan;
+static bool g_have_last_plan = false;
 static void record_plan(const void* ws, const nq_painn_cfg* c, const nq_graph* g, const StepPlan& p) {
   std::lock_guard<std::mutex> lock(g_plan_mu);
   g_plans[ws] = StepRecord{*c, g->N, g->E, g->B, g->max_mol_atoms, p};
+  g_last_plan = g_plans[ws]; g_have_last_plan = true;
+}
+static bool last_plan_for(const nq_painn_cfg* c, int32_t N, int32_t E, int32_t B, StepPlan* p) {
+  std::lock_guard<std::mutex> lock(g_plan_mu);
+  if (!g_have_last_plan || memcmp(&g_last_plan.cfg, c, sizeof(nq_painn_cfg)) != 0 || g_last_plan.N != N || g_last_plan.E != E || g_last_plan.B != B) return false;
+  *p = g_last_plan.plan;
+  return true;
 }
 static int recall_plan(const void* ws, const nq_painn_cfg* c, const nq_graph* g, StepPlan* p) {
   std::lock_guard<std::mutex> lock(g_plan_mu);
@@ -326,6 +337,16 @@
   else if (!strcmp(name, "zq")) { LAYER_OK(L - 1); base = W.lay[l].ZQ; rows = n; w = F; }
   else if (!strcmp(name, "q")) { LAYER_OK(L - 1); base = W.lay[l].Q; rows = n; w = F; }
   else if (!strcmp(name, "y")) { LAYER_OK(L - 1); base = W.lay[l].Y; rows = n; w = 3 * F; }
+  else if (!strcmp(name, "gxh")) {
+    LAYER_OK(L - 1);
+    StepPlan sp;
+    if (!last_plan_for(cfg, N, E, B, &sp)) return nq_fail(NQ_ERR_ARG, "buffer 'gxh': the latest forward call was not made for this model and batch");
+    if (!sp.fused) return nq_fail(NQ_ERR_ARG, "buffer 'gxh' exists only with the fused filter");
+    if (sp.lite) base = W.lay[l].LGXH;
+    else if (l == 0) base = W.GXH;
+    else return nq_fail(NQ_ERR_ARG, "buffer 'gxh' of layer %d is overwritten by the layers below it on this path", l);
+    rows = n; w = 3 * F;
+  }
   else if (!strcmp(name, "rho")) {
     if (W.fused) return nq_fail(NQ_ERR_ARG, "buffer 'rho' is not materialised (filter is fused into the message kernels)");
     base = W.RHO2; rows = e; w = R;
@@ -407,7 +428,7 @@
       NQ_TRY(nq_transpose(st, params + mp.Wr, 3 * F, R, ws + y.WRT));
       nq_make_filter_args(&fa, ws + y.WRT, params + mp.br, rbf_offsets, ws + W.RW, R, cfg->cutoff, cfg->envelope_exponent, cfg->rbf_coeff, cfg->filter_mode);
       fa.row_ctr = row_ctr(0, l);
-      NQ_TRY(nq_msgf_fwd(st, m, fa, false));
+      NQ_TRY(nq_msgf_fwd(st, m, fa, false, plan.layer0 && l == 0));
     } else {
       NQ_TRY(nq_gemm_nt(st, rho, params + mp.Wr, ws + y.PHI, params + mp.br, nullptr, E, 3 * F, R, R, R, 3 * F, "Wr"));
       NQ_TRY(nq_gemm_nt(st, drho, params + mp.Wr, ws + y.PSI, nullptr, nullptr, E, 3 * F, R, R, R, 3 * F, "Wr"));
@@ -472,13 +493,14 @@
       FilterArgs fa;
       nq_make_filter_args(&fa, ws + y.WRT, params + mp.br, rbf_offsets, ws + W.RW, R, cfg->cutoff, cfg->envelope_exponent, cfg->rbf_coeff, cfg->filter_mode);
       fa.row_ctr = row_ctr(1, l);
-      NQ_TRY(nq_msgf_rev(st, m, fa, false));
+      NQ_TRY(nq_msgf_rev(st, m, fa, false, true, plan.layer0 && l == 0));
     } else {
       NQ_TRY(nq_msg_rev(st, m, false));
     }
     float* const GH = lite_store ? ws + y.LGH + NF : ws + W.GH;
     if (lite_store) NQ_TRY(nq_gemm_nn_dsilu2(st, GXH, params + mp.W2, ws + y.LGHP, GH, ws + y.Z1, N, 3 * F, F, "W2"));
     else NQ_TRY(nq_gemm_nn_epi(st, GXH, params + mp.W2, GH, N, 3 * F, F, ws + y.Z1, 0.f, 1.f, 1, "W2"));
+    if (plan.layer0 && l == 0) break;
     if (lite_store) {
       NQ_TRY(nq_gemm_nn_epi(st, GH, params + mp.W1, gx_next, N, F, F, gx_msg, 1.f, 0.f, 0, "W1"));
       gx_cur = gx_next; gv_cur = gv_next;
@@ -579,8 +601,14 @@
   for (int l = 0; l < L; ++l) {
     const WsLayer& y = W.lay[l]; const MsgP& mp = P.msg[l]; const UpdP& up = P.upd[l];
     float* TZ1 = ws + y.Z1 + NF; float* TH = ws + y.Hh + NF; float* TXH = ws + y.XH + 3 * NF;
-    NQ_TRY(nq_gemm_nt_dsilu(st, ws + W.X[l] + NF, params + mp.W1, TZ1, TH, ws + y.Z1, N, F, F, "W1"));
-    NQ_TRY(nq_gemm_nt(st, TH, params + mp.W2, TXH, nullptr, nullptr, N, 3 * F, F, F, F, 3 * F, "W2"));
+    if (plan.layer0 && l == 0) {
+      NQ_HIP(hipMemsetAsync(TZ1, 0, NF * sizeof(float), st));
+      NQ_HIP(hipMemsetAsync(TH, 0, NF * sizeof(float), st));
+      NQ_HIP(hipMemsetAsync(TXH, 0, 3 * NF * sizeof(float), st));
+    } else {
+      NQ_TRY(nq_gemm_nt_dsilu(st, ws + W.X[l] + NF, params + mp.W1, TZ1, TH, ws + y.Z1, N, F, F, "W1"));
+      NQ_TRY(nq_gemm_nt(st, TH, params + mp.W2, TXH, nullptr, nullptr, N, 3 * F, F, F, F, 3 * F, "W2"));
+    }
     MsgArgs m{};
     m.g = g; m.F = F; m.X = ws + W.X[l]; m.V = ws + W.V[l]; m.XH = ws + y.XH; m.PHI = ws + y.PHI; m.PSI = ws + y.PSI;
     m.TX = ws + W.X[l] + NF; m.TV = ws + W.V[l] + 3 * NF; m.TXH = TXH; m.TD = ws + W.TD; m.TR = ws + W.TR;
@@ -589,7 +617,7 @@
       FilterArgs fa;
       nq_make_filter_args(&fa, ws + y.WRT, params + mp.br, rbf_offsets, ws + W.RW, R, cfg->cutoff, cfg->envelope_exponent, cfg->rbf_coeff, cfg->filter_mode);
       fa.row_ctr = row_ctr(2, l);
-      NQ_TRY(nq_msgf_fwd(st, m, fa, true));
+      NQ_TRY(nq_msgf_fwd(st, m, fa, true, plan.layer0 && l == 0));
     } else {
       NQ_TRY(nq_msg_fwd(st, m, true));
     }
@@ -640,6 +668,7 @@
   if (mixed) NQ_HIP(hipMemsetAsync(ws + W.GBR, 0, 3 * NF * sizeof(float), st));
   for (int l = L - 1; l >= 0; --l) {
     const WsLayer& y = W.lay[l]; const MsgP& mp = P.msg[l]; const UpdP& up = P.upd[l];
+    const bool l0 = plan.layer0 && l == 0;
     float* const GYs = lite ? ws + y.LGY : ws + W.GY;
     float* const GCATs = lite ? ws + y.LGCAT : ws + W.GCAT;
     float* const GUs = lite ? ws + y.LGU : ws + W.GU;
@@ -685,7 +714,7 @@
       fa.row_ctr = row_ctr(3, l);
       m.mol_cap = plan.gw_cap;
       m.row_filter = mixed ? 1 : 0;
-      NQ_TRY(nq_msgf_rev(st, m, fa, true, !molgw));
+      NQ_TRY(nq_msgf_rev(st, m, fa, true, !molgw, l0));
       if (mixed) {
         m.row_filter = 2;
         fa.row_ctr = row_ctr(4, l);
@@ -694,7 +723,7 @@
         NQ_TRY(nq_colsum(st, ws + W.GBR, N, 3 * F, 3 * F, gp + mp.br, scr));
       }
       if (molgw)
-        NQ_TRY(nq_gwr_mol(st, g, F, R, plan.gw_cap, m.XH, m.V, m.TXH, m.TV, m.GX, m.GV, m.GTX, m.GTV, sched, ws + W.GWREC, ws + W.GWPART, gp + mp.Wr, gp + mp.br, mixed));
+        NQ_TRY(nq_gwr_mol(st, g, F, R, plan.gw_cap, m.XH, m.V, m.TXH, m.TV, m.GX, m.GV, m.GTX, m.GTV, sched, ws + W.GWREC, ws + W.GWPART, gp + mp.Wr, gp + mp.br, mixed, l0));
     } else {
       NQ_TRY(nq_msg_rev(st, m, true));
     }
@@ -705,13 +734,13 @@
     if (cfg->rbf_type)
       NQ_TRY(nq_gemm_nn(st, gphi, params + mp.Wr, ws + W.GRHO, 2 * E, 3 * F, R, 3 * F, R, R, l == L - 1 ? 0 : 1, "Wr"));
     if (!molgw) NQ_TRY(nq_colsum(sd, ws + W.GBR, N, 3 * F, 3 * F, gp + mp.br, scr));
-    NQ_TRY(nq_gemm_tn(sd, GXHs, ws + y.Hh, gp + mp.W2, 2L * N, 3 * F, F, 3 * F, F, scr, "W2", gp + mp.b2, N));
+    NQ_TRY(nq_gemm_tn(sd, GXHs, ws + y.Hh, gp + mp.W2, l0 ? (long)N : 2L * N, 3 * F, F, 3 * F, F, scr, "W2", gp + mp.b2, N));
     ss.read_by_side(SB_GPHI); ss.read_by_side(SB_GBR); ss.read_by_side(SB_GXH);
     ss.before_main_writes(SB_GH);
     NQ_TRY(nq_gemm_nn(st, GXHs, params + mp.W2, GHs, lite ? N : 2 * N, 3 * F, F, 3 * F, F, F, 0, "W2"));
     NQ_TRY(nq_silu_rev(st, ws + y.Z1, ws + y.Z1 + NF, GHs, lite ? ws + y.LGHP : GHs + NF, (long)NF, true, lite));
     sd = ss.fork();
-    NQ_TRY(nq_gemm_tn(sd, GHs, ws + W.X[l], gp + mp.W1, 2L * N, F, F, F, F, scr, "W1", gp + mp.b1, N));
+    NQ_TRY(nq_gemm_tn(sd, GHs, ws + W.X[l], gp + mp.W1, l0 ? (long)N : 2L * N, F, F, F, F, scr, "W1", gp + mp.b1, N));
     ss.read_by_side(SB_GH);
     NQ_TRY(nq_gemm_nn(st, GHs, params + mp.W1, ws + W.GX, lite ? N : 2 * N, F, F, F, F, F, 1, "W1"));
     if (layer_events && layer_events[L - 1 - l]) NQ_HIP(hipEventRecord((hipEvent_t)layer_events[L - 1 - l], ss.on ? ss.side : st));
diff --git a/nabladft_amd/csrc/molpair.hip b/nabladft_amd/csrc/molpair.hip
--- a/nabladft_amd/csrc/molpair.hip
+++ b/nabladft_amd/csrc/molpair.hip
@@ -231,6 +231,7 @@
 struct GmOps { f4 P0, P1, P2, A, T; };
 struct GmRec { u4 hi, lo; };
 
+template <bool LZ>
 __global__ __launch_bounds__(GM_THREADS) void k_gwr_mol(GwrMolArgs q, const u4* __restrict__ PA, const unsigned* __restrict__ PG) {
   extern __shared__ __attribute__((aligned(16))) float rows[];
   const int F = q.F, F3 = 3 * q.F;
@@ -260,7 +261,8 @@
     }
     const long n = a0 + min(st_at, na - 1), o = n * F3 + cb + 4 * st_qd;
     r[0] = *reinterpret_cast<const f4*>(s0 + o); r[1] = *reinterpret_cast<const f4*>(s1 + o); r[2] = *reinterpret_cast<const f4*>(s2 + o);
-    r[3] = *reinterpret_cast<const f4*>(s3 + n * st3 + cb + 4 * st_qd);
+    if (LZ && blk == 0) r[3] = f4{0.f, 0.f, 0.f, 0.f};
+    else r[3] = *reinterpret_cast<const f4*>(s3 + n * st3 + cb + 4 * st_qd);
   };
   auto blk_store = [&](int blk, int na, const f4 (&r)[4]) __attribute__((always_inline)) {
     if (st_at < na) {
@@ -276,8 +278,8 @@
     const char* pt = reinterpret_cast<const char*>(rows) + ((ko ^ x) + lbase);
     if (GM_ABLATE & 8) { const float z = __uint_as_float((no ^ x) + lbase); o.P0 = o.P1 = o.P2 = f4{z, z, 1.f, 2.f}; o.A = o.T = f4{1.f, z, __uint_as_float((ko ^ x) + lbase), 3.f}; return; }
     o.P0 = *reinterpret_cast<const f4*>(ps);
-    o.P1 = *reinterpret_cast<const f4*>(ps + GM_CH * 16);
-    o.P2 = *reinterpret_cast<const f4*>(ps + 2 * GM_CH * 16);
+    if (!LZ) o.P1 = *reinterpret_cast<const f4*>(ps + GM_CH * 16);
+    if (!LZ) o.P2 = *reinterpret_cast<const f4*>(ps + 2 * GM_CH * 16);
     o.A = *reinterpret_cast<const f4*>(pt + 3 * GM_CH * 16);
     o.T = *reinterpret_cast<const f4*>(pt + 4 * GM_CH * 16);
   };
@@ -302,11 +304,18 @@
       if (i == GM_BATCH - 1 && !more) nkn = 0;
       ops_load(nxt, nkn);
       const float gx = g0[0], gy = g0[1], gz = g0[2], t0 = gc[0], t1 = gc[1], t2 = gc[2];
-      const f4 P0 = cur.P0, P1 = cur.P1, P2 = cur.P2, A = cur.A, T = cur.T;
+      const f4 P0 = cur.P0, A = cur.A, T = cur.T;
+      f4 P1 = f4{0.f, 0.f, 0.f, 0.f}, P2 = P1;
+      if (!LZ) { P1 = cur.P1; P2 = cur.P2; }
       const float xa = P0[0], xb = P0[1], xc = P0[2], txa = P0[3], txb = P1[0], txc = P1[1], v0 = P1[2], v1 = P1[3], v2 = P2[0], tv0 = P2[1],
                   tv1 = P2[2], tv2 = P2[3];
       float ga, gb, gcc, ha, hb, hc;
-      if (GM_ABLATE & 4) { ga = xa + gx; gb = xb + txa; gcc = xc + A[0]; ha = txb + T[0]; hb = v2 + gy + t0; hc = tv2 + v1 + t1 + t2 + gz + txc + v0 + tv0 + tv1; }
+      if (LZ) {
+        const float gmc = (A[0] * gx + A[1] * gy + A[2] * gz) + (T[0] * t0 + T[1] * t1 + T[2] * t2);
+        const float gtmc = T[0] * gx + T[1] * gy + T[2] * gz;
+        ga = A[3] * xa; gcc = gmc * xc; ha = T[3] * xa; hc = gtmc * xc;
+        gb = 0.f; hb = 0.f;
+      } else if (GM_ABLATE & 4) { ga = xa + gx; gb = xb + txa; gcc = xc + A[0]; ha = txb + T[0]; hb = v2 + gy + t0; hc = tv2 + v1 + t1 + t2 + gz + txc + v0 + tv0 + tv1; }
       else {
         const float gmb = A[0] * v0 + A[1] * v1 + A[2] * v2 + (T[0] * tv0 + T[1] * tv1 + T[2] * tv2);
         const float gtmb = T[0] * v0 + T[1] * v1 + T[2] * v2;
@@ -316,7 +325,7 @@
         ga = gma * xa + gtma * txa; gb = gmb * xb + gtmb * txb; gcc = gmc * xc + gtmc * txc;
         ha = gtma * xa; hb = gtmb * xb; hc = gtmc * xc;
       }
-      ba = gm_pair_sum<false>(ga, ha); bb = gm_pair_sum<false>(gb, hb); bc = gm_pair_sum<true>(gcc, hc);
+      ba = gm_pair_sum<false>(ga, ha); bb = LZ ? 0.f : gm_pair_sum<false>(gb, hb); bc = gm_pair_sum<true>(gcc, hc);
       gc = gn;
     };
     if (!(GM_ABLATE & 1)) {
@@ -327,7 +336,7 @@
         step(2 * j, L0, L1, a0_, b0_, c0_);
         step(2 * j + 1, L1, L0, a1_, b1_, c1_);
         gm_split2(a0_, a1_, bh[0][j], bl[0][j]);
-        gm_split2(b0_, b1_, bh[1][j], bl[1][j]);
+        if (!LZ) gm_split2(b0_, b1_, bh[1][j], bl[1][j]);
         gm_split2(c0_, c1_, bh[2][j], bl[2][j]);
       }
     }
@@ -337,13 +346,13 @@
       const gm_bf8 h1 = __builtin_bit_cast(gm_bf8, (u4{bh[1][0], bh[1][1], bh[1][2], bh[1][3]})), l1 = __builtin_bit_cast(gm_bf8, (u4{bl[1][0], bl[1][1], bl[1][2], bl[1][3]}));
       const gm_bf8 h2 = __builtin_bit_cast(gm_bf8, (u4{bh[2][0], bh[2][1], bh[2][2], bh[2][3]})), l2 = __builtin_bit_cast(gm_bf8, (u4{bl[2][0], bl[2][1], bl[2][2], bl[2][3]}));
       acc0 = __builtin_amdgcn_mfma_f32_32x32x16_bf16(al, h0, acc0, 0, 0, 0);
-      acc1 = __builtin_amdgcn_mfma_f32_32x32x16_bf16(al, h1, acc1, 0, 0, 0);
+      if (!LZ) acc1 = __builtin_amdgcn_mfma_f32_32x32x16_bf16(al, h1, acc1, 0, 0, 0);
       acc2 = __builtin_amdgcn_mfma_f32_32x32x16_bf16(al, h2, acc2, 0, 0, 0);
       acc0 = __builtin_amdgcn_mfma_f32_32x32x16_bf16(ah, l0, acc0, 0, 0, 0);
-      acc1 = __builtin_amdgcn_mfma_f32_32x32x16_bf16(ah, l1, acc1, 0, 0, 0);
+      if (!LZ) acc1 = __builtin_amdgcn_mfma_f32_32x32x16_bf16(ah, l1, acc1, 0, 0, 0);
       acc2 = __builtin_amdgcn_mfma_f32_32x32x16_bf16(ah, l2, acc2, 0, 0, 0);
       acc0 = __builtin_amdgcn_mfma_f32_32x32x16_bf16(ah, h0, acc0, 0, 0, 0);
-      acc1 = __builtin_amdgcn_mfma_f32_32x32x16_bf16(ah, h1, acc1, 0, 0, 0);
+      if (!LZ) acc1 = __builtin_amdgcn_mfma_f32_32x32x16_bf16(ah, h1, acc1, 0, 0, 0);
       acc2 = __builtin_amdgcn_mfma_f32_32x32x16_bf16(ah, h2, acc2, 0, 0, 0);
     } else { acc0[0] += __uint_as_float(bh[0][0] ^ bl[1][1] ^ bh[2][2] ^ bl[0][3] ^ bh[1][0] ^ bl[2][1] ^ bh[0][1] ^ bl[0][0] ^ bh[1][2] ^ bl[1][3] ^ bh[2][0] ^ bl[2][3] ^ rc.hi[0] ^ rc.lo[1]); }
   };
@@ -361,7 +370,7 @@
   if (m < q.g.B && stager) {
     const int a0 = __builtin_amdgcn_readfirstlane(q.g.mol_ptr[m]), na = __builtin_amdgcn_readfirstlane(q.g.mol_ptr[m + 1]) - a0;
 #pragma unroll
-    for (int blk = 0; blk < 5; ++blk) { f4 r[4]; blk_load(blk, a0, na, r); blk_store(blk, na, r); }
+    for (int blk = 0; blk < 5; ++blk) { if (LZ && (blk == 1 || blk == 2)) continue; f4 r[4]; blk_load(blk, a0, na, r); blk_store(blk, na, r); }
   }
   GmRec RX, RY;
   unsigned gq0 = 0, gq1 = 0;
@@ -408,13 +417,14 @@
     f4 stg[5][4];
     if (GM_STAGE_EARLY && mn < q.g.B && stager) {
 #pragma unroll
-      for (int blk = 0; blk < 5; ++blk) blk_load(blk, a0n, nan, stg[blk]);
+      for (int blk = 0; blk < 5; ++blk) { if (LZ && (blk == 1 || blk == 2)) continue; blk_load(blk, a0n, nan, stg[blk]); }
     }
     if (mn < q.g.B) { rec_load(RX, sgn_.x); gq0 = geo_load(sgn_.x); gq1 = geo_load(sgn_.x + 1); }
     if (!(GM_ABLATE & 128)) __syncthreads();
     if (mn < q.g.B && stager) {
 #pragma unroll
       for (int blk = 0; blk < 5; ++blk) {
+        if (LZ && (blk == 1 || blk == 2)) continue;
         if (!GM_STAGE_EARLY) blk_load(blk, a0n, nan, stg[blk]);
         blk_store(blk, nan, stg[blk]);
       }
@@ -561,8 +571,8 @@
 
 int nq_gwr_mol(hipStream_t st, const NqGraphView& g, int F, int R, int max_mol_atoms, const float* XH, const float* V, const float* TXH, const float* TV,
                const float* GX, const float* GV, const float* GTX, const float* GTV, const int* sched_ints, const float* recs, float* part, float* gWr,
-               float* gbr, bool accumulate) {
-  NQ_PROF(st, "gwr_mol");
+               float* gbr, bool accumulate, bool layer0) {
+  NQ_PROF(st, layer0 ? "gwr_mol_l0" : "gwr_mol");
   const MolGwBufs b = molgw_bufs(const_cast<int*>(sched_ints), g.E, g.B);
   GwrMolArgs q;
   q.g = g; q.F = F; q.nslices = F / GM_CH; q.groups = molgw_groups(g.B, q.nslices);
@@ -572,8 +582,13 @@
   const u4* PA = reinterpret_cast<const u4*>(recs);
   const unsigned* PG = reinterpret_cast<const unsigned*>(recs + gm_max_batches(g.E, g.B) * GM_PA_DWORDS);
   const size_t lds = (size_t)q.max_atoms * GM_ATOM_BYTES + GM_NW * GM_RING_BYTES;
-  NQ_DYN_LDS(k_gwr_mol, lds);
-  hipLaunchKernelGGL(k_gwr_mol, dim3(q.groups * q.nslices), dim3(GM_THREADS), lds, st, q, PA, PG);
+  if (layer0) {
+    NQ_DYN_LDS(k_gwr_mol<true>, lds);
+    hipLaunchKernelGGL(k_gwr_mol<true>, dim3(q.groups * q.nslices), dim3(GM_THREADS), lds, st, q, PA, PG);
+  } else {
+    NQ_DYN_LDS(k_gwr_mol<false>, lds);
+    hipLaunchKernelGGL(k_gwr_mol<false>, dim3(q.groups * q.nslices), dim3(GM_THREADS), lds, st, q, PA, PG);
+  }
   NQ_LAUNCH_CHECK();
   hipLaunchKernelGGL(k_gwr_mol_reduce, dim3(nq_cdiv((long)(R + 1) * 3 * F, 256 / GMR_Q)), dim3(256), 0, st, part, b.wlo, q.groups, q.nslices, R, F, gWr, gbr, accumulate ? 1 : 0);
   NQ_LAUNCH_CHECK();
```
